# montyhall/bot7

Hardware: AMD Instinct MI355X
Metric: EI candidates scored/sec at N=2048,d=32 (higher is better)
Workload: dtype f64

## Files before the change

bot7_amd/build.py:

```python
import concurrent.futures
import os
import subprocess
import sys

HERE = os.path.dirname(os.path.abspath(__file__))
ROOT = os.path.dirname(HERE)
CSRC = os.path.join(HERE, "csrc")
BUILD = os.path.join(HERE, "_build")
OUT = os.path.join(HERE, "libbot7hip.so")
SOURCES = ["context.hip", "grid_api.hip", "gp_api.hip", "nominate.hip", "blr_api.hip", "sobol.hip", "covar.hip", "potrf.hip", "potrf_persist.hip", "posterior.hip", "score.hip", "extras.hip", "comm.hip", "group.hip", "blr_small.hip", "gp_small.hip", "kpost_small.hip", "batch.hip", "mes.hip", "rff.hip", "slice.hip", "refine.hip", "kg.hip", "ehvi.hip", "trust_region.hip"]
DIAG_ONLY_SOURCES = ["nll_small.hip"]
DIAG_OUT = os.path.join(ROOT, "tools", "_build", "libbot7hip_diag.so")
HEADERS = [os.path.join(CSRC, "b7_internal.h"), os.path.join(CSRC, "gemm_f64.h"), os.path.join(CSRC, "potrf_diag.h"), os.path.join(CSRC, "comm_rccl.h"), os.path.join(CSRC, "ksx_exp.h"), os.path.join(CSRC, "ksx_walk.h"), os.path.join(CSRC, "exp_table.h"), os.path.join(CSRC, "mes_math.h"), os.path.join(CSRC, "counter_rng.h"), os.path.join(CSRC, "gp_small_body.h"), os.path.join(CSRC, "post_ring_layout.h"),
           os.path.join(ROOT, "include", "bot7hip.h")]
HIPCC = os.environ.get("HIPCC", "/opt/rocm/bin/hipcc")
FLAGS = ["-O3", "-std=c++17", "-fPIC", "--offload-arch=gfx950", "-fno-fast-math", "-Wall",
         "-I" + os.path.join(ROOT, "include"), "-I" + CSRC, "-I/opt/rocm/include"]


def _stale(target, deps):
    if not os.path.exists(target):
        return True
    t = os.path.getmtime(target)
    return any(os.path.getmtime(d) > t for d in deps)


EXTRA_FLAGS = {"covar.hip": ["-mllvm", "-amdgpu-mfma-vgpr-form"], "batch.hip": ["-mllvm", "-amdgpu-mfma-vgpr-form"],
               "rff.hip": ["-mllvm", "-amdgpu-mfma-vgpr-form"],
               "kg.hip": ["-mllvm", "-amdgpu-mfma-vgpr-form"],
               "slice.hip": ["-mllvm", "-disable-machine-licm"]}


def _compile(src, diag=False):
    obj = os.path.join(BUILD, ("diag_" if diag else "") + src.replace(".hip", ".o"))
    path = os.path.join(CSRC, src)
    if _stale(obj, [path] + HEADERS + [os.path.abspath(__file__)]):
        subprocess.check_call([HIPCC] + FLAGS + EXTRA_FLAGS.get(src, []) + (["-DB7_DIAG"] if diag else []) + ["-c", path, "-o", obj])
        return obj, True
    return obj, False


def _mentions_diag(src):
    return "B7_DIAG" in open(os.path.join(CSRC, src)).read()


def build_diag(verbose=False):
    build()
    os.makedirs(os.path.dirname(DIAG_OUT), exist_ok=True)
    todo = [s for s in SOURCES if _mentions_diag(s)] + DIAG_ONLY_SOURCES
    with concurrent.futures.ThreadPoolExecutor(max_workers=min(8, len(todo))) as ex:
        res = dict(zip(todo, ex.map(lambda s: _compile(s, True), todo)))
    objs = [res[s][0] if s in res else os.path.join(BUILD, s.replace(".hip", ".o")) for s in SOURCES + DIAG_ONLY_SOURCES]
    if any(ch for _, ch in res.values()) or _stale(DIAG_OUT, objs):
        subprocess.check_call([HIPCC, "-shared", "-fPIC", "--offload-arch=gfx950", "-o", DIAG_OUT] + objs +
                              ["-ldl", "-Wl,-rpath,/opt/rocm/lib", "-Wl,--no-undefined", "-Wl,-Bsymbolic"])
        if verbose:
            print("built", DIAG_OUT)
    return DIAG_OUT


def posterior_isa():
    out = os.path.join(BUILD, "posterior.s")
    path = os.path.join(CSRC, "posterior.hip")
    if _stale(out, [path] + HEADERS + [os.path.abspath(__file__)]):
        subprocess.check_call([HIPCC] + [f for f in FLAGS if f != "-fPIC"] + ["-S", "--cuda-device-only", "-Wno-unused-command-line-argument",
                                                                            path, "-o", out])
    return out


def check_agpr_discipline():
    import re
    text = open(posterior_isa()).read()
    found = {}
    for m in re.finditer(r"^(_ZN\S*post_kernel_w4(?:ILi(\d)E|tILi\d+ELi\d+E)\S*):[^\n]*\n(.*?)\n\s*s_endpgm", text, flags=re.S | re.M):
        nj = int(m.group(2)) if m.group(2) else 16
        ntiles = 32 if nj == 16 else 8 * nj
        in_asm, stats, bad = False, {"mfma": 0, "mfma_from_zero": 0, "acc_reads": 0, "scratch": 0}, []
        for line in m.group(3).split("\n"):
            code = line.split(";")[0]
            if "ASMSTART" in line:
                in_asm = True
                continue
            if "ASMEND" in line:
                in_asm = False
                continue
            if in_asm:
                stats["mfma"] += "v_mfma_f64_16x16x4_f64" in code
                stats["mfma_from_zero"] += bool(re.search(r"v_mfma_f64_16x16x4_f64 a\[[^\]]*\], v\[[^\]]*\], v\[[^\]]*\], 0\s*$", code))
                stats["acc_reads"] += "v_accvgpr_read_b32" in code
            else:
                if re.search(r"(?<![A-Za-z0-9_.])a(\[|\d)", code):
                    bad.append(line.strip())
                if nj == 16 and re.search(r"\bm0\b", code):
                    bad.append(line.strip())
                stats["scratch"] += "scratch_" in code
        if bad or stats["scratch"] or stats["mfma_from_zero"] != ntiles or stats["acc_reads"] != 8 * ntiles:
            raise RuntimeError("post_kernel_w4<%d>: AGPR discipline broken: %r, compiler-generated AGPR uses: %r"
                               % (nj, stats, bad[:5]))
        found[nj] = stats
    if not {2, 4} <= set(found):
        raise RuntimeError("post_kernel_w4<2> and <4> expected in the ISA of posterior.hip, found %r" % sorted(found))
    return found


def build_post_probe():
    src = os.path.join(ROOT, "tools", "post_probe.hip")
    out = os.path.join(ROOT, "tools", "_build", "post_probe")
    os.makedirs(os.path.dirname(out), exist_ok=True)
    if _stale(out, [src, os.path.join(ROOT, "tools", "post_kernel_w8.h"), os.path.join(CSRC, "posterior.hip")] + HEADERS):
        subprocess.check_call([HIPCC, "--offload-arch=gfx950", "-O3", "-std=c++17", "-fno-fast-math", "-Wno-unused-value",
                               "-DB7_POST_NO_LAUNCHERS", "-I" + os.path.join(ROOT, "include"), "-I" + CSRC,
                               "-I/opt/rocm/include", "-o", out, src, "-Wl,-rpath,/opt/rocm/lib"])
    return out


def build(force=False, verbose=False):
    os.makedirs(BUILD, exist_ok=True)
    if force:
        for f in os.listdir(BUILD):
            os.remove(os.path.join(BUILD, f))
    with concurrent.futures.ThreadPoolExecutor(max_workers=min(8, len(SOURCES) + 2)) as ex:
        isa = ex.submit(check_agpr_discipline)
        probe = ex.submit(build_post_probe)
        results = list(ex.map(_compile, SOURCES))
        isa.result()
        probe.result()
    objs = [o for o, _ in results]
    if any(changed for _, changed in results) or _stale(OUT, objs):
        subprocess.check_call([HIPCC, "-shared", "-fPIC", "--offload-arch=gfx950", "-o", OUT] + objs +
                              ["-ldl", "-Wl,-rpath,/opt/rocm/lib", "-Wl,--no-undefined", "-Wl,-Bsymbolic"])
        if verbose:
            print("built", OUT)
    return OUT


if __name__ == "__main__":
    build(force="--force" in sys.argv, verbose=True)
    if "--diag" in sys.argv:
        build_diag(verbose=True)
```

bot7_amd/csrc/b7_internal.h:

```cpp
#pragma once
#include <hip/hip_runtime.h>
#include <stddef.h>
#include <stdint.h>

#include <map>
#include <string>
#include <vector>

#include "bot7hip.h"

constexpr int B7_NPAD = 128;
constexpr int B7_PANEL = 64;
constexpr int B7_PERSIST_NMAX = 4096;
constexpr int B7_MROWS = 256;
constexpr int B7_MAX_D = 96;

constexpr int B7_TAB_VAL = 0;
constexpr int B7_TAB_IDX = 1;
constexpr int B7_TAB_STATUS = 2;
constexpr int B7_TAB_ROWS = 3;
constexpr int B7_TAB_ROW0 = 4;
constexpr int B7_TAB_W = B7_TAB_ROW0 + B7_MAX_D;
constexpr int B7_MAX_WORLD = 64;

// ... 160 lines not shown
  DevBuf part;
  DevBuf ystar, mes_ticket;
  DevBuf mes_user;
  int mes_levels = 8;
  int mes_S = 0, mes_K = 0, mes_nb = 0;
  int64_t mes_M = 0;
  int mes_slot = 0;
  bool mes_valid = false;
  DevBuf ticket;
  DevBuf feas;
  DevBuf feas_stage;
  bool feas_valid = false;
  hipEvent_t ev_feas[2] = {nullptr, nullptr};
  DevBuf scratch;
  DevBuf tmpgrid;
  DevBuf tmpmu, tmpvar;
  DevBuf fant;
  DevBuf bel;
  DevBuf belvec;
  PinBuf pin_bel;
  DevBuf ts_paths;
  DevBuf ts_draw;
  DevBuf ts_work, ts_user;
  bool ts_valid = false;
  int64_t ts_M = 0;
  int ts_q = 0, ts_S = 0, ts_F = 0, ts_N = 0, ts_d = 0;
  DevBuf refine_ws, refine_trace;
  DevBuf refine_user;
  bool refine_trace_on = false, refine_valid = false;
  int refine_P = 0, refine_d = 0, refine_iters = 0, refine_trace_P = 0, refine_trace_iters = 0;
  RefState refine_last;
  DevBuf kg;
  DevBuf kgvec;
  DevBuf kg_slopes;
  DevBuf kg_user;
  PinBuf pin_kg;
  bool kg_trace_on = false, kg_valid = false, kg_traced = false;
  int kg_S = 0, kg_n = 0;
  int64_t kg_M = 0;
  size_t kg_al_off = 0;
  DevBuf post;
  bool post_valid = false;
  int post_S = 0;
  int64_t post_M = 0;
  DevBuf ehvi_front;
  DevBuf ehvi_user;
  hipEvent_t ev_ehvi[2] = {nullptr, nullptr};
  DevBuf feat;
  size_t feat_zeroed_bytes = 0;
  int feat_z = -1;
  int64_t Mfeat = 0;
  int zdim = 0;
  uint64_t feat_version = 0, grid_version = 0;
  DevBuf netbuf;

  void *comm = nullptr;
  int comm_rank = 0, comm_world = 1;
  DevBuf slots;
  uint64_t *tab_host = nullptr;
  uint64_t *tab_host_dev = nullptr;
  struct b7_group *group = nullptr;
  bool group_busy = false;
  bool win_valid = false;
  int64_t win_idx1 = 0;
  int win_rank = -1, win_d = 0;
  double win_row[B7_MAX_D];
  int64_t shard_rows[B7_MAX_WORLD];
  int shard_world = 0;

  hipEvent_t tev[B7_MAX_TIMERS][2];
  bool tev_init = false;
  bool profile = false;
  std::map<std::string, PhaseStat> phases;
  struct PendingPhase { const char *name; hipEvent_t e0, e1; };
  std::vector<PendingPhase> pending;
  std::vector<hipEvent_t> free_events;
  hipEvent_t phase_e0 = nullptr;
};

int b7_fail(b7_ctx *c, int code, const char *fmt, ...);
#define B7_HIP(c, expr)                                                                          \
  do {                                                                                           \
    hipError_t e__ = (expr);                                                                     \
    if (e__ != hipSuccess)                                                                       \
      return b7_fail((c), e__ == hipErrorOutOfMemory ? B7_ERR_NOMEM : B7_ERR_HIP, "%s:%d: %s", \
                     __FILE_NAME__, __LINE__, hipGetErrorString(e__));                           \
  } while (0)
#define B7_TRY(expr)          \
  do {                        \
    int rc__ = (expr);        \
    if (rc__ != B7_OK) return rc__; \
  } while (0)

int b7_ensure(b7_ctx *c, DevBuf &b, size_t bytes);
void b7_release(DevBuf &b);
int b7_pin_ensure(b7_ctx *c, PinBuf &b, size_t bytes, bool mapped);
static inline ScratchBlock *b7_scratch(const b7_ctx *c) { return static_cast<ScratchBlock *>(c->scratch.p); }

struct PhaseScope {
  b7_ctx *c;
  const char *name;
  PhaseScope(b7_ctx *c, const char *name);
  ~PhaseScope();
};

static inline int64_t round_up(int64_t x, int64_t m) { return (x + m - 1) / m * m; }
int npad_of(const b7_ctx *c, int64_t n);

struct FitSet {
  const double *w = nullptr, *zsc = nullptr, *zss = nullptr, *Linv = nullptr, *alpha = nullptr;
  int S = 1, Npad = 0, dpad = 0;
  double amp = 0.0, noise = 0.0, mean = 0.0;
  const double *amp_dev = nullptr, *noise_dev = nullptr, *mean_dev = nullptr;
  static int64_t s_w(int, int dpad) { return dpad; }
  static int64_t s_zsc(int Npad, int dpad) { return (int64_t)Npad * dpad; }
  static int64_t s_zss(int Npad, int) { return Npad; }
  static int64_t s_Linv(int Npad, int) { return (int64_t)Npad * Npad; }
  static int64_t s_alpha(int Npad, int) { return Npad; }
};
static inline FitSet ctx_fit(const b7_ctx *c) {
  FitSet f;
  f.w = (const double *)c->w.p, f.zsc = (const double *)c->zsc.p, f.zss = (const double *)c->zss.p;
  f.Linv = (const double *)c->Linv.p, f.alpha = (const double *)c->alpha.p;
  f.Npad = c->Npad, f.dpad = c->dpad;
  f.amp = c->amp, f.noise = c->noise, f.mean = c->mean;
  return f;
}

int launch_sobol(b7_ctx *c, double *out, int64_t size, int dims, int64_t skip, const double *mins,
                 const double *maxes);
int launch_random_grid(b7_ctx *c, double *out, int64_t size, int dims, uint64_t seed, int64_t row_offset,
                       const double *mins, const double *maxes);
int launch_remove_row(b7_ctx *c, const double *src, double *dst, int64_t M, int d, int64_t idx0);
int launch_remove_rows(b7_ctx *c, const double *src, double *dst, int64_t M, int d, const int64_t *cuts_dev, int ncut);
int launch_colrange(b7_ctx *c, const double *grid, int64_t M, int d, double *out_dev);
int launch_col_affine(b7_ctx *c, double *grid, int64_t M, int d, const double *v_dev, bool mul);
int launch_gather_rows(b7_ctx *c, const double *src, double *out, const int64_t *idx0_dev, int64_t n, int d);
int launch_trust_region(b7_ctx *c, double *grid, int64_t M, int d, const double *vec_dev, bool rotate, double prob, uint64_t seed,
                        int64_t row_offset);

struct KBatchDesc {
  int64_t s_w = 0, s_zsc = 0, s_zsh = 0, s_out = 0;
  const double *amp = nullptr;
  int64_t s_alpha = 0, s_mu = 0;
  const double *mean = nullptr;
};
struct ObsSet {
  const double *zsc;
  const double *zsh;
  int npad;
  const double *w = nullptr;
  KBatchDesc batch;
};
int launch_prep_obs_aux(b7_ctx *c, const double *xobs, const double *ls_dev, int N, int npad, double *zsc,
                        double *zsh);
int launch_k_generic(b7_ctx *c, const double *xq, int64_t rows, int64_t Mtotal, const ObsSet &o, double *out);
int launch_prep_obs(b7_ctx *c, const double *xobs, const double *lenscale_sq_dev, int N, int d);
int launch_kxx(b7_ctx *c, double diag_add);
int launch_ksx_batch(b7_ctx *c, const FitSet &f, const double *xq, int64_t rows, int64_t Mtotal, double *ks, int64_t s_out,
                     double *mu, int64_t s_mu);
int launch_kxx_batch(b7_ctx *c, int B, const double *ls_dev, const double *amp_dev, const double *noise_dev, double *w,
                     double *zsc, double *zss, double *K);
int launch_ksx(b7_ctx *c, const FitSet &f, const double *xq, int64_t row0, int64_t rows, int64_t Mtotal, int d, double *ks,
               double *mu, int ycols);

struct FactorNote {
  bool alpha_done = false;
  int *report_written = nullptr;
};
int launch_potrf(b7_ctx *c, double extra, bool with_inverse, int *report_hint = nullptr, FactorNote *note = nullptr);
int launch_trtri(b7_ctx *c);
int launch_potrf_persist(b7_ctx *c, double extra, bool with_inverse);
int launch_nll_batch(b7_ctx *c, int B, const double *K, double *L, double *dinv, unsigned *flags, int *info,
                     const double *resid, double *terms);
int launch_nll_one(b7_ctx *c, const double *K, double *L, double *dinv, unsigned *flags, int *info, const double *resid,
                   double *terms, double extra);
size_t persist_flag_words_host(int nb);
int launch_potrf_small(b7_ctx *c, int B, const double *K, double *L, double *Linv, double *dinv, const double *resid, double *alpha,
                       double extra, int *info, int *report_dev, int64_t sK, int64_t sL, int64_t sdinv, int64_t svec, int sinfo);
int launch_blr_head_small(b7_ctx *c, const double *Z, int N, int z, int ldz, const double *yv, double alpha_prec, double beta,
                          int *report_dev);
int launch_blr_heads_small(b7_ctx *c, int S, const double *Z, int N, int z, int ldz, const double *yraw_dev, const double *hyp3_dev,
                           double *L, double *Linv, double *m, double *b, int *info, int *report_dev, double *terms);
int launch_post_heads(b7_ctx *c, int S, const double *Linv, const double *feat, int64_t rows, int64_t Mtotal, double *var, int64_t svar,
                      const double *zero_dev, const double *invbeta_dev);
int launch_gemv_rows_batch(b7_ctx *c, int S, const double *A, int lda, const double *x, int64_t sx, int n, const double *base_dev,
                           int64_t rows, double *y, int64_t sy);
int launch_nll_small(b7_ctx *c, int B, const double *hyp_dev, const double *hyp_host, double *terms_dev, int *info_dev,
                     unsigned *done_dev);
bool kpost_small_applies(const b7_ctx *c);
int launch_kpost_small(b7_ctx *c, const FitSet &f, const double *xq, int64_t M, double *mu, double *var, int64_t sout);
bool gp_small_applies(const b7_ctx *c);
static inline bool fit_small_applies(const b7_ctx *c) {
  return c->fit_small && c->potrf_sched == 3 && c->inverse_inline && gp_small_applies(c);
}
int launch_nll_small8(b7_ctx *c, int B, const double *hyp_dev, const double *hyp_host, double *terms_dev, int *info_dev,
                      unsigned *done_dev);
int launch_fit_small(b7_ctx *c, int B, const double *hyp_dev, const double *hyp_host, double *hyp_out, double *w, double *zsc,
                     double *zss, double *L, double *Linv, double *dinv, double *alpha, double *resid, int *info_dev,
                     int *report_dev);
int launch_alpha(b7_ctx *c, int *report_dev = nullptr, int report_words = 0, const FactorNote &note = FactorNote());
int launch_alpha_batch(b7_ctx *c, int B, const double *Linv, const double *resid, double *alpha, const int *report_src = nullptr,
                       int *report_dev = nullptr, int report_words = 0);
int launch_fit_batch(b7_ctx *c, int B, const double *K, double *L, double *Linv, double *dinv, unsigned *flags, int *info);
int launch_nll_terms(b7_ctx *c, double *out_dev);
int launch_fro_norm_sq(b7_ctx *c, const double *A, int n, int ld, double *out_dev);
int launch_set_identity(b7_ctx *c);

int launch_post(b7_ctx *c, const FitSet &f, const double *ks, int64_t row0, int64_t rows, int64_t Mtotal, double *var);
int launch_post_batch(b7_ctx *c, const FitSet &f, const double *ks, int64_t sks, int64_t rows, int64_t Mtotal, double *var,
                      int64_t svar);

int launch_mean_multi(b7_ctx *c, const FitSet &f, const double *ks, int64_t row0, int64_t rows, int64_t Mtotal, double *mu);
int launch_gemm_nt(b7_ctx *c, const double *A, int lda, const double *B, int ldb, double *C, int ldc, int m, int n,
                   int k);
int launch_fantasy_cov(b7_ctx *c, const double *kpp, const double *g, double *S, int P, double diag_add);
int launch_fantasy_factor(b7_ctx *c, double *S, double *dinv_tmp, int *info_dev);
int launch_fantasy_sample(b7_ctx *c, const double *Lp, const double *mu, int P, int n, uint64_t seed, double *out);
int launch_add_diag(b7_ctx *c, double *S, int ld, int n, double v);

int launch_append_finalize(b7_ctx *c, const double *krow, const double *lvec, const double *uvec, const double *evec,
                           int *status_dev);
int launch_append_vectors(b7_ctx *c, const double *krow, double *lvec, double *uvec, double *part, double *evec);
int launch_mlp_forward(b7_ctx *c, const double *X, int64_t M, int d, const double *net_dev, const int *dims,
                       int n_layers, int activation, double *out, int ld_out);
int launch_mlp_forward_mean(b7_ctx *c, const double *X, int64_t M, int d, const double *net_dev, const int *dims,
                            int n_layers, int activation, double *out, int ld_out, const double *mvec, double mean0,
                            double *mu, bool *mean_done);
int launch_gemv_rows(b7_ctx *c, const double *A, int lda, const double *x, int n, double base, int64_t row0,
                     int64_t rows, int64_t Mtotal, double *y);
int launch_transpose_pad(b7_ctx *c, const double *Z, int n, int ldz, int z, double *Zt, int zpad, int nk);
int launch_blr_assemble(b7_ctx *c, const double *G, double *K, int z, int zpad, double alpha_prec, double beta);

int launch_score(b7_ctx *c, ScoreParams p, const double *mu, const double *var, int64_t M, int ycols, double *out, bool accumulate);
int launch_score_batch(b7_ctx *c, const ScoreParams &p, double *acc, int64_t M);
int launch_finish(b7_ctx *c, double *acc, int64_t M, double divisor, double *best_val, int64_t *best_idx1, bool logacc = false);
int launch_fill(b7_ctx *c, double *p, int64_t n, double v);
int launch_finish_slot(b7_ctx *c, double *acc, int64_t M, double divisor, uint64_t *tab_dev, int rank, int world,
                       int64_t offset, const double *grid, int d, bool all_slots, uint64_t *host_rec = nullptr,
                       unsigned *host_done = nullptr, bool logacc = false, const double *feas = nullptr);

struct ExclRows {
  int n = 0;
  long long row[B7_BATCH_MAX];
};
int launch_score_finish_slot(b7_ctx *c, const ScoreParams &p, double *acc, int64_t M, double divisor, uint64_t *tab_dev,
                             int rank, int world, int64_t offset, const double *grid, int d, bool all_slots, uint64_t *host_rec = nullptr,
                             unsigned *host_done = nullptr, const ExclRows *excl = nullptr, const double *feas = nullptr);
void acc_declare_zeros(b7_ctx *c, int score_kind);
int acc_write_zeros(b7_ctx *c);
void acc_forget(b7_ctx *c);
int acc_materialize(b7_ctx *c);
void feas_forget(b7_ctx *c);
static inline void post_forget(b7_ctx *c) { c->post_valid = false; }
int feas_write_zeros(b7_ctx *c);
int launch_feas_add(b7_ctx *c, const double *src);
int launch_feas_best(b7_ctx *c, double *best_val, int64_t *best_idx1);
int launch_keep_record(b7_ctx *c, uint64_t *tab_dev, int rank, int world);
int launch_score_grad(b7_ctx *c, const ScoreParams &p, const double *mu, const double *var, const double *dmu, const double *dvar,
                      int64_t M1, int d, double *value, double *grad);
struct RefStep {
  const double *mu, *var, *dmu, *dvar;
  const double *xq;
  double *xq_next;
  RefState *st;
  double *trace;
  const double *lo, *hi;
  int d, P, iter, iters;
  double eta0;
};
int launch_refine_step(b7_ctx *c, const ScoreParams &p, const RefStep &r);
int launch_row_slot(b7_ctx *c, uint64_t *tab_dev, int rank, int world, int64_t idx1_global, int64_t local0, const double *grid,
                    int d);

int exch_table_ensure(b7_ctx *c, int world);
int exch_local(b7_ctx *c, double divisor, int64_t offset, int rank, int world, bool all_slots, bool mirror = false,
               const ScoreParams *pend = nullptr, const ExclRows *excl = nullptr, const double *feas = nullptr);
int exch_wait_mirror(b7_ctx *c);
int exch_fail_record(b7_ctx *c, int rank, int world, int code);
int exch_allreduce(b7_ctx *c);
int exch_collective(b7_ctx *c, int rc, int rank, int world, double *best_val, int64_t *best_idx1);
int exch_rewrite_record(b7_ctx *c, int rank, int world);
int exch_fetch(b7_ctx *c, int first_rank, int nranks);
bool exch_pick(const uint64_t *tab, int world, int stride, double *val, int64_t *idx1, int *rank);
int exch_conclude(b7_ctx *c, const uint64_t *tab, int world, double *best_val, int64_t *best_idx1);
void exch_forget(b7_ctx *c);

void persist_gave_up(b7_ctx *c);
int chol_with_jitter(b7_ctx *c, double *jitter_out, int *info_first_out, bool with_inverse, FactorNote *note = nullptr);
int check_hyp(b7_ctx *c, const b7_hyp *hyp, int d);
void launch_resid_batch(b7_ctx *c, int B, const double *mean_dev);
int fit_front(b7_ctx *c, const b7_hyp *hyp, const double *ls_dev);
int fit_hyp_core(b7_ctx *c, const b7_hyp *hyp, double *nll_out, double *jitter_used, int *info_out, bool then_predict);
int64_t predict_chunk(const b7_ctx *c, int64_t M);
int predict_into(b7_ctx *c, const FitSet &fit, const double *xq, int64_t M, double *mu, double *var);
int copy_out_mu_var(b7_ctx *c, const void *mu, const void *var, int64_t M, int cols, double *mean_host, double *var_host,
                    bool wait = false);

struct HypPack { double *ls, *amp, *noise, *mean; };
static inline HypPack hyp_pack(void *base, int B, int d) {
  double *amp = static_cast<double *>(base) + (size_t)B * d;
  return {static_cast<double *>(base), amp, amp + B, amp + 2 * (size_t)B};
}
constexpr int B7_SLOTS_OPERANDS = 1;
constexpr int B7_SLOTS_LINV = 2;
constexpr int B7_SLOTS_ALPHA = 4;
constexpr int B7_SLOTS_FACTOR = 8;
int batch_slots_ensure(b7_ctx *c, int B, int groups);
static inline FitSet batch_fits(const b7_ctx *c, int S) {
  const HypPack hd = hyp_pack(c->bhyp.p, S, c->dfit);
  FitSet f;
  f.w = (const double *)c->bw.p, f.zsc = (const double *)c->bzsc.p, f.zss = (const double *)c->bzss.p;
  f.Linv = (const double *)c->bLinv.p, f.alpha = (const double *)c->balpha.p;
  f.S = S, f.Npad = c->Npad, f.dpad = c->dpad;
  f.amp_dev = hd.amp, f.noise_dev = hd.noise, f.mean_dev = hd.mean;
  return f;
}
static inline FitSet fit_at(const FitSet &set, int s, const b7_hyp &hyp) {
  const int Npad = set.Npad, dpad = set.dpad;
  FitSet f;
  f.Npad = Npad, f.dpad = dpad;
  f.w = set.w + s * FitSet::s_w(Npad, dpad), f.zsc = set.zsc + s * FitSet::s_zsc(Npad, dpad), f.zss = set.zss + s * FitSet::s_zss(Npad, dpad);
  f.Linv = set.Linv + s * FitSet::s_Linv(Npad, dpad), f.alpha = set.alpha + s * FitSet::s_alpha(Npad, dpad);
  f.amp = hyp.amp, f.noise = hyp.noise, f.mean = hyp.mean;
  return f;
}

int nominate_args(b7_ctx *c, const char *who, const b7_score_spec *spec, int64_t offset);
int stage_fmin(b7_ctx *c, const double *fmin, double **fd_out);
static inline bool score_needs_fmin(int kind) { return kind == B7_SCORE_EI || kind == B7_SCORE_LOGEI || kind == B7_SCORE_LOGPI; }
constexpr int score_acc_kind(int kind) { return (kind == B7_SCORE_LOGEI || kind == B7_SCORE_LOGPI) ? B7_ACC_LOG : B7_ACC_LINEAR; }
static inline const char *score_kind_name(int kind) {
  return kind == B7_SCORE_EI ? "ei" : kind == B7_SCORE_LOGEI ? "logei" : kind == B7_SCORE_LOGPI ? "logpi" : kind == B7_SCORE_MES ? "mes" : "cb";
}
int mes_begin(b7_ctx *c, int S, int64_t M, int K);
int launch_mes_search(b7_ctx *c, const double *mu, const double *var, int64_t stride, int nS, int slot0);
const double *mes_ystar_dev(const b7_ctx *c, int slot);
int mes_refuse(b7_ctx *c, const char *who, const b7_score_spec *spec);
ScoreParams score_params(const b7_ctx *c, const b7_score_spec *spec, const double *fd);
int score_add(b7_ctx *c, const b7_score_spec *sp, const double *fd, bool accumulate = true);
int pending_score(b7_ctx *c, int S, const b7_score_spec *spec, const double *fd, ScoreParams *out);
int eval_validate(b7_ctx *c, int S, const b7_hyp *hyps, const b7_score_spec *spec, int64_t offset);
struct BelKeep {
  double *mu = nullptr, *var = nullptr;
  FitSet fits;
  bool want_alpha = false;
};
int eval_enqueue(b7_ctx *c, int S, const b7_hyp *hyps, const b7_score_spec *spec, ScoreParams *pend, BelKeep *keep = nullptr);
bool reports_clean(b7_ctx *c, const int *reports, int S, bool persist);
int eval_redo(b7_ctx *c, int S, const b7_hyp *hyps, const b7_score_spec *spec, double *jitter_out, int *info_out,
              BelKeep *keep = nullptr);
struct BelPass {
  const double *xq; int64_t rows;
  const double *xj;
  const double *w, *zsc, *zss;
  const double *wj;
  const double *par;
  double *scal;
  double *kcol;
  double *var, *u; int64_t sgrid;
  int64_t idx; int j;
};
int launch_believer(b7_ctx *c, int S, const BelPass &p, bool column);
// ... 31 lines not shown
```

bot7_amd/csrc/blr_api.hip:

```cpp
#include <math.h>
#include <string.h>

#include "b7_internal.h"

static int upload_net(b7_ctx *c, const b7_mlp *net, int *z_out) {
  if (!net || !net->dims || !net->W || !net->b || net->n_layers < 1 || net->n_layers > 4)
    return b7_fail(c, B7_ERR_INVALID, "mlp: 1..4 layers with dims, W and b required");
  size_t total = 0;
  for (int l = 0; l < net->n_layers; ++l) total += (size_t)net->dims[l + 1] * net->dims[l] + net->dims[l + 1];
  std::vector<double> pack(total);
  size_t off = 0;
  for (int l = 0; l < net->n_layers; ++l) {
    const size_t nw = (size_t)net->dims[l + 1] * net->dims[l];
    memcpy(&pack[off], net->W[l], nw * sizeof(double));
    off += nw;
    memcpy(&pack[off], net->b[l], (size_t)net->dims[l + 1] * sizeof(double));
    off += net->dims[l + 1];
  }
  *z_out = net->dims[net->n_layers];
  if (c->net_host.size() == total && c->netbuf.cap >= total * sizeof(double) &&
      memcmp(c->net_host.data(), pack.data(), total * sizeof(double)) == 0)
    return B7_OK;
  B7_TRY(b7_ensure(c, c->netbuf, total * sizeof(double)));
  B7_HIP(c, hipStreamSynchronize(c->stream));
  B7_HIP(c, hipMemcpy(c->netbuf.p, pack.data(), total * sizeof(double), hipMemcpyHostToDevice));
  c->net_host.swap(pack);
  return B7_OK;
}

static int feat_alloc(b7_ctx *c, int64_t M, int z) {
  const int zpad = npad_of(c, z);
  const size_t bytes = sizeof(double) * (size_t)round_up(M, B7_MROWS) * zpad;
  const bool grown = c->feat.cap < bytes;
  B7_TRY(b7_ensure(c, c->feat, bytes));
  if (grown || c->feat_z != z || c->feat_zeroed_bytes < bytes) {
    B7_HIP(c, hipMemsetAsync(c->feat.p, 0, c->feat.cap, c->stream));
    c->feat_zeroed_bytes = c->feat.cap;
    c->feat_z = z;
  }
  c->Mfeat = M;
  c->zdim = z;
  c->predicted = false;
  return B7_OK;
}

static int blr_head_setup(b7_ctx *c, int z, int nk, double mean, double noise, bool general = true) {
  const size_t np = (size_t)npad_of(c, z), nn = np * np * sizeof(double);
  if (general) {
    for (DevBuf *b : {&c->K, &c->L, &c->Linv, &c->W}) B7_TRY(b7_ensure(c, *b, nn));
    B7_TRY(b7_ensure(c, c->dinv, sizeof(double) * (np + B7_PANEL) * B7_PANEL));
    B7_TRY(b7_ensure(c, c->alpha, sizeof(double) * np));
    B7_TRY(b7_ensure(c, c->resid, sizeof(double) * np));
    B7_TRY(b7_ensure(c, c->tmpvar, sizeof(double) * (size_t)nk));
  }
  B7_TRY(b7_ensure(c, c->info, B7_INFO_BYTES));
  c->have_data = false, c->fitted = false, c->predicted = false;
  post_forget(c);
  c->N = z, c->Npad = (int)np, c->ycols = 1, c->yld = 1, c->model_kind = 1;
  c->mean = mean, c->noise = noise, c->amp = 0.0;
  return B7_OK;
}

static int blr_predict_enqueue(b7_ctx *c, int64_t M, bool mean_done = false) {
  B7_TRY(b7_ensure(c, c->mu, sizeof(double) * (size_t)M));
  B7_TRY(b7_ensure(c, c->var, sizeof(double) * (size_t)M));
  if (!mean_done)
    B7_TRY(launch_gemv_rows(c, (const double *)c->feat.p, c->Npad, (const double *)c->alpha.p, c->Npad, c->mean, 0, M, M,
                            (double *)c->mu.p));
  B7_TRY(launch_post(c, ctx_fit(c), (const double *)c->feat.p, 0, round_up(M, B7_MROWS), M, (double *)c->var.p));
  c->predicted = true;
  c->Mpred = M;
  return B7_OK;
}

static int blr_fit_core(b7_ctx *c, const double *Y0, int N, int z, double alpha_prec, double beta, double mean,
                        double *nll_out) {
  const int zpad = npad_of(c, z), nk = (int)round_up(N, 16);
  const size_t np = (size_t)zpad;
  B7_TRY(blr_head_setup(c, z, nk, mean, 1.0 / beta));
  std::vector<double> rb((size_t)nk, 0.0);
  for (int i = 0; i < N; ++i) rb[i] = beta * (Y0[i] - mean);
  B7_HIP(c, hipMemcpyAsync(c->tmpvar.p, rb.data(), sizeof(double) * nk, hipMemcpyHostToDevice, c->stream));
  B7_TRY(launch_gemm_nt(c, (const double *)c->tmpgrid.p, nk, (const double *)c->tmpgrid.p, nk, (double *)c->W.p, zpad,
                        zpad, zpad, nk));
  B7_TRY(launch_blr_assemble(c, (const double *)c->W.p, (double *)c->K.p, z, zpad, alpha_prec, beta));
  B7_TRY(launch_gemv_rows(c, (const double *)c->tmpgrid.p, nk, (const double *)c->tmpvar.p, nk, 0.0, 0, zpad, zpad,
                          (double *)c->resid.p));
  int info_first = 0;
  double jitter = 0.0;
  FactorNote note;
  B7_TRY(chol_with_jitter(c, &jitter, &info_first, true, &note));
  B7_TRY(launch_trtri(c));
  B7_TRY(launch_alpha(c, nullptr, 0, note));
  B7_HIP(c, hipStreamSynchronize(c->stream));
  if (nll_out) {
    std::vector<double> diag(z), m(z), bq(z);
    B7_HIP(c, hipMemcpy2D(diag.data(), sizeof(double), c->L.p, sizeof(double) * (np + 1), sizeof(double), z,
                          hipMemcpyDeviceToHost));
    B7_HIP(c, hipMemcpy(m.data(), c->alpha.p, sizeof(double) * z, hipMemcpyDeviceToHost));
    B7_HIP(c, hipMemcpy(bq.data(), c->resid.p, sizeof(double) * z, hipMemcpyDeviceToHost));
    double logdet = 0.0, rr = 0.0, qm = 0.0;
    for (int k = 0; k < z; ++k) {
      logdet += 2.0 * log(diag[k]);
      qm += bq[k] * m[k];
    }
    for (int i = 0; i < N; ++i) rr += (Y0[i] - mean) * (Y0[i] - mean);
    const double Em = 0.5 * beta * rr - 0.5 * qm;
    *nll_out = -(0.5 * z * log(alpha_prec) + 0.5 * N * log(beta) - Em - 0.5 * logdet - 0.5 * N * log(2.0 * M_PI));
  }
  c->fitted = true;
  return B7_OK;
}

static int blr_enqueue_fit(b7_ctx *c, const b7_mlp *net, const double *X0, const double *Y0, int N, int z, double alpha_prec,
                           double beta, double mean) {
  const int d = net->dims[0], zpad = npad_of(c, z), nk = (int)round_up(N, 16);
  B7_TRY(b7_ensure(c, c->tmpgrid, sizeof(double) * (size_t)zpad * nk));
  B7_TRY(blr_head_setup(c, z, nk, mean, 1.0 / beta));
  const size_t up_doubles = (size_t)N * d + (size_t)nk;
  B7_TRY(b7_ensure(c, c->tmpmu, sizeof(double) * (up_doubles + (size_t)N * z)));
  B7_TRY(b7_pin_ensure(c, c->pin_blr, sizeof(double) * up_doubles, false));
  double *stage = static_cast<double *>(c->pin_blr.host);
  memcpy(stage, X0, sizeof(double) * (size_t)N * d);
  for (int i = 0; i < nk; ++i) stage[(size_t)N * d + i] = i < N ? beta * (Y0[i] - mean) : 0.0;
  double *xdev = (double *)c->tmpmu.p, *yvdev = xdev + (size_t)N * d, *zdev = yvdev + nk;
  B7_HIP(c, hipMemcpyAsync(xdev, stage, sizeof(double) * up_doubles, hipMemcpyHostToDevice, c->stream));
  B7_TRY(launch_mlp_forward(c, xdev, N, d, (const double *)c->netbuf.p, net->dims, net->n_layers, net->activation, zdev, z));
  if (zpad == 64 && c->blr_small) {
    B7_TRY(launch_blr_head_small(c, zdev, N, z, z, yvdev, alpha_prec, beta, nullptr));
    B7_HIP(c, hipMemcpyAsync(c->pinned->fit.info, c->info.p, 16, hipMemcpyDeviceToHost, c->stream));
    c->fitted = true;
    return B7_OK;
  }
  B7_TRY(launch_transpose_pad(c, zdev, N, z, z, (double *)c->tmpgrid.p, zpad, nk));
  B7_TRY(launch_gemm_nt(c, (const double *)c->tmpgrid.p, nk, (const double *)c->tmpgrid.p, nk, (double *)c->W.p, zpad, zpad,
                        zpad, nk));
  B7_TRY(launch_blr_assemble(c, (const double *)c->W.p, (double *)c->K.p, z, zpad, alpha_prec, beta));
  B7_TRY(launch_gemv_rows(c, (const double *)c->tmpgrid.p, nk, (const double *)yvdev, nk, 0.0, 0, zpad, zpad,
                          (double *)c->resid.p));
  FactorNote note;
  B7_TRY(launch_potrf(c, 0.0, true, nullptr, &note));
  if (!c->linv_done) B7_TRY(launch_trtri(c));
  B7_TRY(launch_alpha(c, nullptr, 0, note));
  B7_HIP(c, hipMemcpyAsync(c->pinned->fit.info, c->info.p, 16, hipMemcpyDeviceToHost, c->stream));
  c->fitted = true;
  return B7_OK;
}

static int blr_enqueue_score(b7_ctx *c, const b7_mlp *net, int z, const b7_score_spec *spec, bool fused_mean = true) {
  const int zpad = npad_of(c, z);
  B7_TRY(feat_alloc(c, c->M, z));
  B7_TRY(b7_ensure(c, c->mu, sizeof(double) * (size_t)c->M));
  B7_TRY(b7_ensure(c, c->var, sizeof(double) * (size_t)c->M));
  B7_TRY(b7_ensure(c, c->acc, sizeof(double) * (size_t)c->M));
  bool mean_done = false;
  B7_TRY(launch_mlp_forward_mean(c, (const double *)c->grid[c->grid_cur].p, c->M, c->d, (const double *)c->netbuf.p, net->dims,
                                 net->n_layers, net->activation, (double *)c->feat.p, zpad,
                                 fused_mean ? (const double *)c->alpha.p : nullptr, c->mean, (double *)c->mu.p, &mean_done));
  B7_TRY(blr_predict_enqueue(c, c->M, mean_done));
  double *fd = nullptr;
  if (score_needs_fmin(spec->kind)) B7_TRY(stage_fmin(c, spec->fmin, &fd));
  return score_add(c, spec, fd, false);
}

static int blr_marg_slow(b7_ctx *c, const b7_mlp *net, const double *X0, const double *Y0, int N, int S, const double *ap,
                         const double *bt, const double *mn, int z, const b7_score_spec *spec, double *nll_out) {
  const int zpad = npad_of(c, z);
  B7_TRY(b7_ensure(c, c->acc, sizeof(double) * (size_t)c->M));
  B7_TRY(acc_write_zeros(c));
  for (int s = 0; s < S; ++s) {
    B7_TRY(b7_blr_fit_x(c, net, X0, Y0, N, ap[s], bt[s], mn[s], nll_out ? nll_out + s : nullptr));
    if (s == 0) {
      B7_TRY(feat_alloc(c, c->M, z));
      B7_TRY(launch_mlp_forward(c, (const double *)c->grid[c->grid_cur].p, c->M, c->d, (const double *)c->netbuf.p, net->dims,
                                net->n_layers, net->activation, (double *)c->feat.p, zpad));
    }
    c->Mfeat = c->M;
    B7_TRY(blr_predict_enqueue(c, c->M));
    double *fd = nullptr;
    if (score_needs_fmin(spec->kind)) B7_TRY(stage_fmin(c, spec->fmin, &fd));
    B7_TRY(score_add(c, spec, fd));
  }
  return B7_OK;
}

static int blr_marg_fast(b7_ctx *c, const b7_mlp *net, const double *X0, const double *Y0, int N, int S, const double *ap,
                         const double *bt, const double *mn, int z, const b7_score_spec *spec, bool want_terms, ScoreParams *pend) {
  const int d = net->dims[0];
  const size_t up_doubles = (size_t)N * d + (size_t)N + 5 * (size_t)S;
  B7_TRY(b7_ensure(c, c->tmpmu, sizeof(double) * (up_doubles + (size_t)N * z)));
  B7_TRY(b7_ensure(c, c->bL, sizeof(double) * (size_t)S * 64 * 64));
  B7_TRY(b7_ensure(c, c->bLinv, sizeof(double) * (size_t)S * 64 * 64));
  B7_TRY(b7_ensure(c, c->balpha, sizeof(double) * (size_t)S * 64));
  B7_TRY(b7_ensure(c, c->bresid, sizeof(double) * (size_t)S * 64));
  B7_TRY(b7_ensure(c, c->binfo, sizeof(int) * 4 * (size_t)S));
  B7_TRY(b7_ensure(c, c->bterms, sizeof(double) * 3 * (size_t)S + 64));
  B7_TRY(b7_ensure(c, c->bmu, sizeof(double) * (size_t)S * c->M));
  B7_TRY(b7_ensure(c, c->bvar, sizeof(double) * (size_t)S * c->M));
  B7_TRY(b7_ensure(c, c->acc, sizeof(double) * (size_t)c->M));
  const size_t rep_bytes = 16 * (size_t)S, term_bytes = sizeof(double) * 3 * (size_t)S;
  B7_TRY(b7_pin_ensure(c, c->pin_eval, rep_bytes + term_bytes, true));
  B7_TRY(b7_pin_ensure(c, c->pin_blr, sizeof(double) * up_doubles, false));
  B7_TRY(blr_head_setup(c, z, 0, c->mean, c->noise, false));
  double *stage = static_cast<double *>(c->pin_blr.host);
  memcpy(stage, X0, sizeof(double) * (size_t)N * d);
  memcpy(stage + (size_t)N * d, Y0, sizeof(double) * N);
  double *hs = stage + (size_t)N * d + N;
  for (int s = 0; s < S; ++s) hs[s] = ap[s], hs[S + s] = bt[s], hs[2 * S + s] = mn[s], hs[3 * S + s] = 0.0, hs[4 * S + s] = 1.0 / bt[s];
  double *xdev = (double *)c->tmpmu.p, *ydev = xdev + (size_t)N * d, *hdev = ydev + N, *zdev = hdev + 5 * (size_t)S;
  B7_HIP(c, hipMemcpyAsync(xdev, stage, sizeof(double) * up_doubles, hipMemcpyHostToDevice, c->stream));
  B7_TRY(launch_mlp_forward(c, xdev, N, d, (const double *)c->netbuf.p, net->dims, net->n_layers, net->activation, zdev, z));
  int *reports = static_cast<int *>(c->pin_eval.host);
  memset(reports, 0xff, rep_bytes);
  B7_TRY(launch_blr_heads_small(c, S, zdev, N, z, z, ydev, hdev, (double *)c->bL.p, (double *)c->bLinv.p, (double *)c->balpha.p,
                                (double *)c->bresid.p, (int *)c->binfo.p, static_cast<int *>(c->pin_eval.dev), (double *)c->bterms.p));
  if (want_terms)
    B7_HIP(c, hipMemcpyAsync(static_cast<char *>(c->pin_eval.host) + rep_bytes, c->bterms.p, term_bytes, hipMemcpyDeviceToHost, c->stream));
  B7_TRY(feat_alloc(c, c->M, z));
  B7_TRY(launch_mlp_forward(c, (const double *)c->grid[c->grid_cur].p, c->M, c->d, (const double *)c->netbuf.p, net->dims,
                            net->n_layers, net->activation, (double *)c->feat.p, 64));
  B7_TRY(launch_gemv_rows_batch(c, S, (const double *)c->feat.p, 64, (const double *)c->balpha.p, 64, 64, hdev + 2 * (size_t)S, c->M,
                                (double *)c->bmu.p, c->M));
// ... 194 lines not shown
```

bot7_amd/csrc/covar.hip:

```cpp
#include "b7_internal.h"
#include "gemm_f64.h"
#include "ksx_exp.h"
#include "ksx_walk.h"

namespace {

__global__ void __launch_bounds__(64) prep_obs_kernel(const double *__restrict__ xobs, const double *ls, double *w,
                                                      double *zsc, double *zsh, int N, int Npad, int d, int dpad) {
  extern __shared__ __align__(16) double psm[];
  {
    const int64_t b = blockIdx.y;
    ls += b * d;
    w += b * dpad;
    zsc += b * (int64_t)Npad * dpad;
    zsh += b * Npad;
  }
  const int tld = dpad + 1, lane = threadIdx.x, row0 = blockIdx.x * 64;
  double *tile = psm, *wl = psm + 64 * tld;
  for (int k = lane; k < dpad; k += 64) {
    const double wk = (k < d) ? 1.0 / ls[k] : 0.0;
    wl[k] = wk;
    if (blockIdx.x == 0) w[k] = wk;
  }
  int nrows = N - row0;
  nrows = nrows < 0 ? 0 : (nrows > 64 ? 64 : nrows);
  const double *src = xobs + (int64_t)row0 * d;
#pragma unroll 8
  for (int e = lane; e < nrows * d; e += 64) {
    const int r = e / d, k = e - r * d;
    tile[r * tld + k] = src[e];
  }
  __syncthreads();
  double s = 0.0;
#pragma unroll 8
  for (int k = 0; k < dpad; ++k) {
    const double z = (lane < nrows && k < d) ? tile[lane * tld + k] : 0.0;
    const double wk = wl[k];
    tile[lane * tld + k] = z * wk;
    s += (z * z) * wk;
  }
  if (row0 + lane < Npad) zsh[row0 + lane] = (lane < nrows) ? 0.5 * s : 1e300;
  __syncthreads();
  double *dst = zsc + (int64_t)row0 * dpad;
#pragma unroll 8
  for (int e = lane; e < 64 * dpad; e += 64) {
    const int r = e / dpad, k = e - r * dpad;
    if (row0 + r < Npad) dst[e] = tile[r * tld + k];
  }
}

__device__ __forceinline__ void pair_pack(double a, double b, d2_t &out) {
  const int alo = __double2loint(a), ahi = __double2hiint(a), blo = __double2loint(b), bhi = __double2hiint(b);
  int o0l, o0h, o1l, o1h;
  asm volatile(
      "s_mov_b32 vcc_lo, 0x55555555\n\t"
      "s_mov_b32 vcc_hi, 0x55555555\n\t"
      "s_nop 0\n\t"
      "v_cndmask_b32_dpp %0, %6, %4, vcc quad_perm:[1,0,3,2] row_mask:0xf bank_mask:0xf\n\t"
      "v_cndmask_b32_dpp %1, %7, %5, vcc quad_perm:[1,0,3,2] row_mask:0xf bank_mask:0xf\n\t"
      "s_not_b64 vcc, vcc\n\t"
      "v_cndmask_b32_dpp %2, %4, %6, vcc quad_perm:[1,0,3,2] row_mask:0xf bank_mask:0xf\n\t"
      "v_cndmask_b32_dpp %3, %5, %7, vcc quad_perm:[1,0,3,2] row_mask:0xf bank_mask:0xf"
      : "=&v"(o0l), "=&v"(o0h), "=&v"(o1l), "=&v"(o1h)
      : "v"(alo), "v"(ahi), "v"(blo), "v"(bhi)
      : "vcc", "scc");
  out[0] = __hiloint2double(o0h, o0l);
  out[1] = __hiloint2double(o1h, o1l);
}

using KBatch = KBatchDesc;
template <int DPAD, int KERN>
__global__ void __launch_bounds__(256)
    ksx_kernel(const double *__restrict__ xq, int64_t row0, int64_t Mtotal, int d, int dpad_rt, const double *w,
               const double *zsc, const double *zsh, const double *__restrict__ alpha, double amp, double meanc, int Npad,
               double *out, double *__restrict__ mu, KBatch kb) {
  extern __shared__ __align__(16) double sm[];
  if (kb.amp) {
    const int64_t bz = blockIdx.z;
    w += bz * kb.s_w;
    zsc += bz * kb.s_zsc;
    zsh += bz * kb.s_zsh;
    out += bz * kb.s_out;
    amp = kb.amp[bz];
    if (kb.mean) {
      alpha += bz * kb.s_alpha;
      mu += bz * kb.s_mu;
      meanc = kb.mean[bz];
    }
  }
  (void)dpad_rt;
  using T = KsxTile<DPAD, 1>;
  constexpr int KO = T::KO;
  KsxWalk<DPAD, 1> wk(sm, zsc, zsh);
  const int tid = wk.tid, lane = wk.lane, wave = wk.wave, lr = wk.lr, lq = wk.lq;
  const int64_t qbase = row0 + (int64_t)blockIdx.x * KSX_Q;
  const int nslab_total = Npad / KO;
  const int nslab = nslab_total / gridDim.y;
  const int slab0 = blockIdx.y * nslab;
  __builtin_assume(nslab > 0);

  const double *sh = wk.zs();
  double *sal = wk.rider();
  double pre_a = 0.0;
  auto rider_load = [&](int s) { pre_a = alpha ? alpha[s * KO + tid] : 0.0; };
  auto rider_store = [&](int buf) { sal[buf * KO + tid] = pre_a; };
  wk.begin(xq, qbase, Mtotal, d, w, amp, slab0, nslab, [] {}, rider_load, rider_store);

  double hq[4], macc[4] = {0.0, 0.0, 0.0, 0.0};
#pragma unroll
  for (int r = 0; r < 4; ++r) hq[r] = wk.xs()[wave * 16 + lq + 4 * r];
  const bool odd = lane & 1;
  double *orow = out + ((int64_t)blockIdx.x * KSX_Q + wave * 16 + lq + (odd ? 4 : 0)) * Npad + (lr & ~1);

  wk.run(slab0, nslab, rider_load, rider_store, [&](int s, int cur, int t, const double (&bf)[T::KSTEPS]) {
    const int o0 = s * KO;
#if B7_KSX_ABLATE & 8
    const d4_t c = mfma_f64(wk.qf[0], bf[0], d4_t{0.0, 0.0, 0.0, 0.0});
#else
    const d4_t c = wk.dist(bf);
#endif
    const double hk = sh[cur * KO + t * 16 + lr];
    const double al = sal[cur * KO + t * 16 + lr];
    double kv[4];
#if B7_KSX_ABLATE & 4
    wk.arg4(c, hq, hk, kv);
#else
    wk.template cov<KERN>(c, hq, hk, kv);
#endif
#pragma unroll
    for (int r = 0; r < 4; ++r) macc[r] = __builtin_fma(kv[r], al, macc[r]);
    d2_t v01, v23;
    pair_pack(kv[0], kv[1], v01);
    pair_pack(kv[2], kv[3], v23);
    {
      double *p = orow + o0 + t * 16;
#if B7_KSX_ABLATE & 1
      if (v01[0] == 1.2345e-300) {
#endif
#if B7_KSX_ABLATE & 16
      double *pi = out + ((int64_t)blockIdx.x * KSX_Q + wave * 16 + 4 * t + (lane >> 5)) * Npad + o0 + (lane & 31) * 2;
      *reinterpret_cast<d2_t *>(pi) = v01;
      *reinterpret_cast<d2_t *>(pi + (int64_t)2 * Npad) = v23;
#elif B7_KSX_ABLATE & 32
      __builtin_nontemporal_store(v01, reinterpret_cast<d2_t *>(p));
      __builtin_nontemporal_store(v23, reinterpret_cast<d2_t *>(p + (int64_t)8 * Npad));
#else
      *reinterpret_cast<d2_t *>(p) = v01;
      *reinterpret_cast<d2_t *>(p + (int64_t)8 * Npad) = v23;
#endif
#if B7_KSX_ABLATE & 1
      }
#endif
    }
  });

  if (mu) {
#pragma unroll
    for (int r = 0; r < 4; ++r) {
      double v = macc[r];
      v += __shfl_xor(v, 1);
      v += __shfl_xor(v, 2);
      v += __shfl_xor(v, 4);
      v += __shfl_xor(v, 8);
      const int64_t g = qbase + wave * 16 + lq + 4 * r;
      if (lr == 0 && g < Mtotal) mu[g] = meanc + v;
    }
  }
}

__global__ void __launch_bounds__(256)
    kxx_fix_kernel(double *K, int N, int Npad, double diag_add, const double *diag_arr, int64_t sK) {
  if (diag_arr) {
    K += (int64_t)blockIdx.y * sK;
    diag_add = diag_arr[blockIdx.y];
  }
  int64_t e = (int64_t)blockIdx.x * blockDim.x + threadIdx.x;
  if (e >= (int64_t)Npad * Npad) return;
  int i = (int)(e / Npad), j = (int)(e - (int64_t)i * Npad);
  if (i >= N || j >= N)
    K[e] = (i == j) ? 1.0 : 0.0;
  else if (i == j)
    K[e] += diag_add;
}

template <int DPAD>
size_t ksx_lds_bytes() {
  size_t bytes = KsxTile<DPAD, 1>::lds_bytes(0);
#if B7_KSX_ABLATE & 128
  const size_t per_cu = 160 * 1024, fit = per_cu / bytes;
  if (fit > 1) bytes = per_cu / (fit - 1) - 512;
#endif
  return bytes;
}

int ksx_launch(b7_ctx *c, dim3 grid, const double *xq, int64_t row0, int64_t Mtotal, int d, const ObsSet &o,
               const double *alpha, double amp, double meanc, double *out, double *mu) {
  return ksx_for_class(c, "covariance kernel", [&](auto cls) {
    using C = decltype(cls);
    const size_t lds = ksx_lds_bytes<C::DPAD>();
    auto kern = ksx_kernel<C::DPAD, C::KERN>;
    B7_HIP(c, hipFuncSetAttribute(reinterpret_cast<const void *>(kern), hipFuncAttributeMaxDynamicSharedMemorySize,
                                  (int)lds));
    hipLaunchKernelGGL(kern, grid, dim3(256), lds, c->stream, xq, row0, Mtotal, d, c->dpad, o.w ? o.w : (const double *)c->w.p,
                       o.zsc, o.zsh, alpha, amp, meanc, o.npad, out, mu, o.batch);
    B7_HIP(c, hipGetLastError());
    return B7_OK;
  });
}

}

int launch_prep_obs(b7_ctx *c, const double *xobs, const double *ls_dev, int N, int d) {
  PhaseScope ps(c, "prep");
  const size_t lds = sizeof(double) * (64 * (size_t)(c->dpad + 1) + c->dpad);
  hipLaunchKernelGGL(prep_obs_kernel, dim3((c->Npad + 63) / 64), dim3(64), lds, c->stream, xobs, ls_dev,
                     (double *)c->w.p, (double *)c->zsc.p, (double *)c->zss.p, N, c->Npad, d, c->dpad);
  B7_HIP(c, hipGetLastError());
  return B7_OK;
}

int launch_prep_obs_aux(b7_ctx *c, const double *xobs, const double *ls_dev, int N, int npad, double *zsc,
                        double *zsh) {
  const size_t lds = sizeof(double) * (64 * (size_t)(c->dpad + 1) + c->dpad);
  hipLaunchKernelGGL(prep_obs_kernel, dim3((npad + 63) / 64), dim3(64), lds, c->stream, xobs, ls_dev, (double *)c->w.p,
                     zsc, zsh, N, npad, c->dfit, c->dpad);
  B7_HIP(c, hipGetLastError());
  return B7_OK;
}

int launch_k_generic(b7_ctx *c, const double *xq, int64_t rows, int64_t Mtotal, const ObsSet &o, double *out) {
  if (rows % KSX_Q || o.npad % 64) return b7_fail(c, B7_ERR_INVALID, "k_generic: extents not multiples of 64");
  return ksx_launch(c, dim3((unsigned)(rows / KSX_Q), 1), xq, 0, Mtotal, c->dfit, o, nullptr, c->amp, 0.0, out, nullptr);
}

int launch_ksx(b7_ctx *c, const FitSet &f, const double *xq, int64_t row0, int64_t rows, int64_t Mtotal, int d, double *ks,
               double *mu, int ycols) {
  PhaseScope ps(c, "ksx");
  if (rows % KSX_Q) return b7_fail(c, B7_ERR_INVALID, "ksx: rows %lld not a multiple of %d", (long long)rows, KSX_Q);
  if (ycols != 1) mu = nullptr;
  ObsSet o{f.zsc, f.zss, c->Npad};
  o.w = f.w;
  return ksx_launch(c, dim3((unsigned)(rows / KSX_Q), 1), xq, row0, Mtotal, d, o, mu ? f.alpha : nullptr, f.amp, f.mean, ks, mu);
}

int launch_kxx(b7_ctx *c, double diag_add) {
  PhaseScope ps(c, "kxx");
  const int Npad = c->Npad;
  int ny = 1;
  while (ny < 16 && (Npad / 64) % (ny * 2) == 0 && (Npad / KSX_Q) * ny < 2 * c->cus) ny *= 2;
  const ObsSet o{(const double *)c->zsc.p, (const double *)c->zss.p, Npad};
  B7_TRY(ksx_launch(c, dim3(Npad / KSX_Q, ny), (const double *)c->xobs.p, 0, c->N, c->dfit, o, nullptr, c->amp, 0.0,
                      (double *)c->K.p, nullptr));
  int64_t total = (int64_t)Npad * Npad;
  hipLaunchKernelGGL(kxx_fix_kernel, dim3((unsigned)((total + 255) / 256)), dim3(256), 0, c->stream, (double *)c->K.p,
                     c->N, Npad, diag_add, (const double *)nullptr, (int64_t)0);
  B7_HIP(c, hipGetLastError());
  return B7_OK;
}

int launch_ksx_batch(b7_ctx *c, const FitSet &f, const double *xq, int64_t rows, int64_t Mtotal, double *ks, int64_t s_out,
                     double *mu, int64_t s_mu) {
  PhaseScope ps(c, "ksx");
  if (rows % KSX_Q) return b7_fail(c, B7_ERR_INVALID, "ksx: rows %lld not a multiple of %d", (long long)rows, KSX_Q);
  ObsSet o{f.zsc, f.zss, c->Npad};
  o.w = f.w;
  o.batch.s_w = FitSet::s_w(c->Npad, c->dpad);
  o.batch.s_zsc = FitSet::s_zsc(c->Npad, c->dpad);
  o.batch.s_zsh = FitSet::s_zss(c->Npad, c->dpad);
  o.batch.s_out = s_out;
  o.batch.amp = f.amp_dev;
  o.batch.s_alpha = FitSet::s_alpha(c->Npad, c->dpad);
  o.batch.s_mu = s_mu;
  o.batch.mean = f.mean_dev;
  return ksx_launch(c, dim3((unsigned)(rows / KSX_Q), 1, f.S), xq, 0, Mtotal, c->dfit, o, f.alpha, f.amp, 0.0, ks, mu);
}

int launch_kxx_batch(b7_ctx *c, int B, const double *ls_dev, const double *amp_dev, const double *noise_dev, double *w,
                     double *zsc, double *zss, double *K) {
  PhaseScope ps(c, "kxx");
  const int Npad = c->Npad, d = c->dfit, dpad = c->dpad;
  const size_t lds = sizeof(double) * (64 * (size_t)(dpad + 1) + dpad);
  hipLaunchKernelGGL(prep_obs_kernel, dim3((Npad + 63) / 64, B), dim3(64), lds, c->stream, (const double *)c->xobs.p, ls_dev,
                     w, zsc, zss, c->N, Npad, d, dpad);
  ObsSet o{zsc, zss, Npad};
  o.w = w;
  o.batch.s_w = FitSet::s_w(Npad, dpad);
  o.batch.s_zsc = FitSet::s_zsc(Npad, dpad);
  o.batch.s_zsh = FitSet::s_zss(Npad, dpad);
  o.batch.s_out = (int64_t)Npad * Npad;
  o.batch.amp = amp_dev;
  int ny = 1;
  while (ny < 16 && (Npad / 64) % (ny * 2) == 0 && (Npad / KSX_Q) * ny * B < 2 * c->cus) ny *= 2;
  B7_TRY(ksx_launch(c, dim3(Npad / KSX_Q, ny, B), (const double *)c->xobs.p, 0, c->N, d, o, nullptr, c->amp, 0.0, K, nullptr));
  const int64_t total = (int64_t)Npad * Npad;
  hipLaunchKernelGGL(kxx_fix_kernel, dim3((unsigned)((total + 255) / 256), B), dim3(256), 0, c->stream, K, c->N, Npad, 0.0,
                     noise_dev, total);
  B7_HIP(c, hipGetLastError());
  return B7_OK;
}
```

bot7_amd/csrc/gp_api.hip:

```cpp
#include <math.h>
#include <string.h>

#include <chrono>

#include "b7_internal.h"

extern "C" __global__ void __launch_bounds__(256) resid_kernel(const double *__restrict__ y, double *__restrict__ r, int64_t nreal,
                                                               int64_t ntotal, double mean) {
  const int64_t e = (int64_t)blockIdx.x * blockDim.x + threadIdx.x;
  if (e < ntotal) r[e] = e < nreal ? y[e] - mean : 0.0;
}

extern "C" __global__ void __launch_bounds__(256) resid_batch_kernel(const double *__restrict__ y, double *__restrict__ r, int N,
                                                                     int Npad, const double *__restrict__ mean) {
  const int i = blockIdx.x * blockDim.x + threadIdx.x, b = blockIdx.y;
  if (i < Npad) r[(int64_t)b * Npad + i] = i < N ? y[i] - mean[b] : 0.0;
}

void launch_resid_batch(b7_ctx *c, int B, const double *mean_dev) {
  hipLaunchKernelGGL(resid_batch_kernel, dim3((c->Npad + 255) / 256, B), dim3(256), 0, c->stream, (const double *)c->ybuf.p,
                     (double *)c->bresid.p, c->N, c->Npad, mean_dev);
}

void persist_gave_up(b7_ctx *c) {
  c->persist_aborts += 1;
  if (c->potrf_sched == 3) c->potrf_sched_saved = 3;
  c->potrf_sched = 1;
}
static void persist_restore(b7_ctx *c) {
  if (c->potrf_sched_saved == 3 && c->persist_aborts < 3) c->potrf_sched = 3;
}

static int try_factor(b7_ctx *c, double extra, int *info, bool with_inverse, FactorNote *note) {
  int two[2] = {0, 0};
  for (int attempt = 0; attempt < 2; ++attempt) {
    B7_TRY(launch_potrf(c, extra, with_inverse, nullptr, note));
    B7_HIP(c, hipMemcpyAsync(two, c->info.p, 2 * sizeof(int), hipMemcpyDeviceToHost, c->stream));
    B7_HIP(c, hipStreamSynchronize(c->stream));
    if (two[1] == 0) break;
    if (attempt == 1) return b7_fail(c, B7_ERR_HIP, "Cholesky: hand-off time-out (code %d) outside the persistent schedule", two[1]);
    persist_gave_up(c);
  }
  persist_restore(c);
  *info = two[0];
  return B7_OK;
}

static int jitter_retries(b7_ctx *c, double *jitter_out, bool with_inverse, FactorNote *note) {
  const int N = c->N;
  int info = 1;
  double jitter = 0.0;
  {
    double *fro_dev = reinterpret_cast<double *>(reinterpret_cast<char *>(c->info.p) + 16);
    B7_TRY(launch_fro_norm_sq(c, (const double *)c->K.p, N, c->Npad, fro_dev));
    double fro = 0.0;
    B7_HIP(c, hipMemcpyAsync(&fro, fro_dev, sizeof(double), hipMemcpyDeviceToHost, c->stream));
    B7_HIP(c, hipStreamSynchronize(c->stream));
    const double max_eps = sqrt(fro);
    if (max_eps != max_eps)
      return b7_fail(c, B7_ERR_INVALID, "chol: the matrix contains NaN (check X_obs and the hyper-parameters)");
    double eps = c->opts.jitter_eps;
    for (;;) {
      if (eps > max_eps) {
        jitter = -1.0;
        B7_TRY(launch_set_identity(c));
        c->linv_done = false;
        if (note) *note = FactorNote();
        break;
      }
      eps = eps * c->opts.jitter_growth;
      B7_TRY(try_factor(c, eps, &info, with_inverse, note));
      if (info == 0) {
        jitter = eps;
        break;
      }
    }
  }
  *jitter_out = jitter;
  return B7_OK;
}

int chol_with_jitter(b7_ctx *c, double *jitter_out, int *info_first_out, bool with_inverse, FactorNote *note) {
  int info = 0;
  B7_TRY(try_factor(c, 0.0, &info, with_inverse, note));
  *info_first_out = info;
  *jitter_out = 0.0;
  if (info != 0) B7_TRY(jitter_retries(c, jitter_out, with_inverse, note));
  return B7_OK;
}

int64_t predict_chunk(const b7_ctx *c, int64_t M) {
  int64_t chunk = (int64_t)(c->ks_bytes / (sizeof(double) * (size_t)c->Npad)) / B7_MROWS * B7_MROWS;
  if (chunk < B7_MROWS) chunk = B7_MROWS;
  const int64_t Mpad = round_up(M, B7_MROWS);
  return chunk > Mpad ? Mpad : chunk;
}

int predict_into(b7_ctx *c, const FitSet &fit, const double *xq, int64_t M, double *mu, double *var) {
  if (M == 0) return B7_OK;
  if (c->kpost_small && c->model_kind == 0 && kpost_small_applies(c))
    return launch_kpost_small(c, fit, xq, M, mu, var, M);
  const int64_t chunk = predict_chunk(c, M), Mpad = round_up(M, B7_MROWS);
  B7_TRY(b7_ensure(c, c->ks, sizeof(double) * (size_t)chunk * c->Npad));
  for (int64_t row0 = 0; row0 < M; row0 += chunk) {
    int64_t rows = Mpad - row0 < chunk ? Mpad - row0 : chunk;
    B7_TRY(launch_ksx(c, fit, xq, row0, rows, M, c->dfit, (double *)c->ks.p, mu, c->ycols));
    if (c->ycols > 1) B7_TRY(launch_mean_multi(c, fit, (const double *)c->ks.p, row0, rows, M, mu));
    B7_TRY(launch_post(c, fit, (const double *)c->ks.p, row0, rows, M, var));
  }
  return B7_OK;
}

int batch_slots_ensure(b7_ctx *c, int B, int groups) {
  const size_t n = (size_t)c->Npad, one = sizeof(double) * (size_t)B;
  if (groups & B7_SLOTS_OPERANDS) {
    B7_TRY(b7_ensure(c, c->bw, one * FitSet::s_w(c->Npad, c->dpad)));
    B7_TRY(b7_ensure(c, c->bzsc, one * FitSet::s_zsc(c->Npad, c->dpad)));
    B7_TRY(b7_ensure(c, c->bzss, one * FitSet::s_zss(c->Npad, c->dpad)));
  }
  if (groups & B7_SLOTS_LINV) B7_TRY(b7_ensure(c, c->bLinv, one * FitSet::s_Linv(c->Npad, c->dpad)));
  if (groups & B7_SLOTS_ALPHA) B7_TRY(b7_ensure(c, c->balpha, one * FitSet::s_alpha(c->Npad, c->dpad)));
  if (groups & B7_SLOTS_FACTOR) {
    B7_TRY(b7_ensure(c, c->bK, one * n * n));
    B7_TRY(b7_ensure(c, c->bL, one * n * n));
    B7_TRY(b7_ensure(c, c->bdinv, one * n * B7_PANEL));
    B7_TRY(b7_ensure(c, c->bresid, one * n));
  }
  return B7_OK;
}

int check_hyp(b7_ctx *c, const b7_hyp *hyp, int d) {
  if (!hyp || !hyp->lenscale_sq) return b7_fail(c, B7_ERR_INVALID, "gp_fit_hyp: NULL argument");
  for (int k = 0; k < d; ++k)
    if (!(hyp->lenscale_sq[k] > 0.0)) return b7_fail(c, B7_ERR_INVALID, "gp_fit: lenscale_sq[%d] must be > 0", k);
  if (!(hyp->amp > 0.0) || !(hyp->noise >= 0.0)) return b7_fail(c, B7_ERR_INVALID, "gp_fit: amp > 0, noise >= 0");
  return B7_OK;
}

int fit_front(b7_ctx *c, const b7_hyp *hyp, const double *ls_dev) {
  const int N = c->N, d = c->dfit, ycols = c->ycols;
  c->fitted = false;
  c->model_kind = 0;
  c->predicted = false;
  c->amp = hyp->amp;
  c->noise = hyp->noise;
  c->mean = hyp->mean;
  const int64_t ntotal = (int64_t)c->Npad * ycols;
  hipLaunchKernelGGL(resid_kernel, dim3((unsigned)((ntotal + 255) / 256)), dim3(256), 0, c->stream,
                     (const double *)c->ybuf.p, (double *)c->resid.p, (int64_t)N * ycols, ntotal, hyp->mean);
  B7_TRY(launch_prep_obs(c, (const double *)c->xobs.p, ls_dev, N, d));
  return launch_kxx(c, hyp->noise);
}

int fit_hyp_core(b7_ctx *c, const b7_hyp *hyp, double *nll_out, double *jitter_used, int *info_out,
                        bool then_predict) {
  if (!c) return B7_ERR_INVALID;
  if (!c->have_data) return b7_fail(c, B7_ERR_STATE, "gp_fit_hyp: call b7_gp_set_data first");
  const int N = c->N, d = c->dfit, ycols = c->ycols;
  B7_TRY(check_hyp(c, hyp, d));
  B7_HIP(c, hipSetDevice(c->device));

  double *ls_stage = c->pinned->vec, *ls_dev = b7_scratch(c)->lenscale;
  memcpy(ls_stage, hyp->lenscale_sq, sizeof(double) * d);
  const bool small = fit_small_applies(c);
  if (small) {
    ls_stage[d] = hyp->amp, ls_stage[d + 1] = hyp->noise, ls_stage[d + 2] = hyp->mean;
    c->fitted = false;
    c->model_kind = 0;
    c->predicted = false;
    c->amp = hyp->amp;
    c->noise = hyp->noise;
    c->mean = hyp->mean;
  } else {
    B7_HIP(c, hipMemcpyAsync(ls_dev, ls_stage, sizeof(double) * d, hipMemcpyHostToDevice, c->stream));
    B7_TRY(fit_front(c, hyp, ls_dev));
  }

  FitBlock &blk = c->pinned->fit;
  double *terms_dev = reinterpret_cast<double *>(reinterpret_cast<char *>(c->info.p) + 16);
  const size_t blk_bytes = 16 + sizeof(double) * (nll_out ? 1 + ycols : 0);
  bool tail_done = false;
  FactorNote note;
  for (int attempt = 0; attempt < 2; ++attempt) {
    if (small && attempt == 0) {
      B7_TRY(launch_fit_small(c, 1, nullptr, ls_stage, ls_dev, (double *)c->w.p, (double *)c->zsc.p, (double *)c->zss.p, (double *)c->L.p,
                              (double *)c->Linv.p, (double *)c->dinv.p, (double *)c->alpha.p, (double *)c->resid.p, (int *)c->info.p,
                              nullptr));
      c->linv_done = true;
      tail_done = true;
      if (nll_out) B7_TRY(launch_nll_terms(c, terms_dev));
    } else {
      B7_TRY(launch_potrf(c, 0.0, true, nullptr, &note));
      tail_done = c->linv_done;
      if (tail_done) {
        B7_TRY(launch_alpha(c, nullptr, 0, note));
        if (nll_out) B7_TRY(launch_nll_terms(c, terms_dev));
      }
    }
    B7_HIP(c, hipMemcpyAsync(&blk, c->info.p, tail_done ? blk_bytes : 16, hipMemcpyDeviceToHost, c->stream));
    if (then_predict && tail_done) {
      B7_HIP(c, hipEventRecord(c->ev_fit, c->stream));
      c->fitted = true;
      B7_TRY(predict_into(c, ctx_fit(c), (const double *)c->grid[c->grid_cur].p, c->M, (double *)c->mu.p, (double *)c->var.p));
      B7_HIP(c, hipEventSynchronize(c->ev_fit));
    } else {
      B7_HIP(c, hipStreamSynchronize(c->stream));
    }
    if (blk.info[1] == 0) break;
    c->fitted = false;
    if (attempt == 1) return b7_fail(c, B7_ERR_HIP, "Cholesky: hand-off time-out (code %d) outside the persistent schedule", blk.info[1]);
    persist_gave_up(c);
  }
  const int info_first = blk.info[0];
  double jitter = 0.0;
  bool predicted = then_predict && tail_done;
  if (info_first != 0) {
    c->fitted = false;
    if (small) B7_TRY(fit_front(c, hyp, ls_dev));
    B7_TRY(jitter_retries(c, &jitter, true, &note));
    tail_done = false;
    predicted = false;
  }
  if (!tail_done) {
    B7_TRY(launch_trtri(c));
    B7_TRY(launch_alpha(c, nullptr, 0, note));
    if (nll_out) B7_TRY(launch_nll_terms(c, terms_dev));
    B7_HIP(c, hipMemcpyAsync(&blk, c->info.p, blk_bytes, hipMemcpyDeviceToHost, c->stream));
    B7_HIP(c, hipStreamSynchronize(c->stream));
  }
  if (then_predict && !predicted) {
    c->fitted = true;
    B7_TRY(predict_into(c, ctx_fit(c), (const double *)c->grid[c->grid_cur].p, c->M, (double *)c->mu.p, (double *)c->var.p));
  }
  if (nll_out)
    for (int k = 0; k < ycols; ++k) nll_out[k] = 0.5 * blk.terms[1 + k] + blk.terms[0] + 0.5 * N * log(2.0 * M_PI);
  if (jitter_used) *jitter_used = jitter;
  if (info_out) *info_out = info_first;
  persist_restore(c);
  c->fitted = true;
  return B7_OK;
}

int copy_out_mu_var(b7_ctx *c, const void *mu, const void *var, int64_t M, int cols, double *mean_host, double *var_host, bool wait) {
  if (mean_host) B7_HIP(c, hipMemcpyAsync(mean_host, mu, sizeof(double) * (size_t)M * cols, hipMemcpyDeviceToHost, c->stream));
  if (var_host) B7_HIP(c, hipMemcpyAsync(var_host, var, sizeof(double) * (size_t)M, hipMemcpyDeviceToHost, c->stream));
  if (mean_host || var_host || wait) B7_HIP(c, hipStreamSynchronize(c->stream));
  return B7_OK;
}

extern "C" {

int b7_gp_default_opts(b7_gp_opts *o) {
  if (!o) return B7_ERR_INVALID;
  o->jitter_eps = 1e-8;
  o->jitter_growth = 1.1;
  o->var_with_noise = 0;
  o->var_clamp = 0;
  o->var_min = 0.0;
  return B7_OK;
}

// ... 146 lines not shown
      B7_HIP(c, hipMemcpyAsync(&terms[(size_t)b * 2], tb, 2 * sizeof(double), hipMemcpyDeviceToHost, c->stream));
      B7_HIP(c, hipStreamSynchronize(c->stream));
      bad = two[0];
      aborted = two[1];
      return B7_OK;
    };
    if (aborted) {
      c->persist_aborts += 1;
      B7_TRY(redo(0.0));
    }
    if (aborted) {
      b7_hyp h{lenscale_sq + (size_t)b * d, amp[b], noise[b], mean[b]};
      persist_gave_up(c);
      double nll1 = 0.0, jit1 = 0.0;
      int info1 = 0;
      const int rc1 = fit_hyp_core(c, &h, &nll1, &jit1, &info1, false);
      c->fitted = false;
      c->predicted = false;
      B7_TRY(rc1);
      nll_out[b] = nll1;
      if (jitter_out) jitter_out[b] = jit1;
      if (info_out) info_out[b] = info1;
      continue;
    }
    if (bad != 0) {
      double *fro_dev = (double *)c->bterms.p;
      B7_TRY(launch_fro_norm_sq(c, Kb, N, n, fro_dev));
      double fro = 0.0;
      B7_HIP(c, hipMemcpyAsync(&fro, fro_dev, sizeof(double), hipMemcpyDeviceToHost, c->stream));
      B7_HIP(c, hipStreamSynchronize(c->stream));
      const double max_eps = sqrt(fro);
      if (max_eps != max_eps) return b7_fail(c, B7_ERR_INVALID, "gp_nll_batch: K of fit %d contains NaN", b);
      double eps = c->opts.jitter_eps;
      while (bad != 0) {
        if (eps > max_eps) return b7_fail(c, B7_ERR_INVALID, "gp_nll_batch: fit %d cannot be factored", b);
        eps = eps * c->opts.jitter_growth;
        B7_TRY(redo(eps));
        if (aborted) return b7_fail(c, B7_ERR_HIP, "gp_nll_batch: hand-off time-out (code %d) in fit %d", aborted, b);
        jitter = eps;
      }
    }
    nll_out[b] = 0.5 * terms[(size_t)b * 2] + terms[(size_t)b * 2 + 1] + c0;
    if (jitter_out) jitter_out[b] = jitter;
    if (info_out) info_out[b] = info_first;
  }
  return B7_OK;
}

int b7_gp_fit_hyp(b7_ctx *c, const b7_hyp *hyp, double *nll_out, double *jitter_used, int *info_out) {
  return fit_hyp_core(c, hyp, nll_out, jitter_used, info_out, false);
}

int b7_gp_fit(b7_ctx *c, const double *X, const double *Y, int N, int d, int ycols, const b7_hyp *hyp,
              double *nll_out, double *jitter_used, int *info_out) {
  if (!c) return B7_ERR_INVALID;
  if (!hyp || !hyp->lenscale_sq) return b7_fail(c, B7_ERR_INVALID, "gp_fit: NULL argument");
  B7_TRY(b7_gp_set_data(c, X, Y, N, d, ycols));
  return b7_gp_fit_hyp(c, hyp, nll_out, jitter_used, info_out);
}

int b7_gp_predict_hyp(b7_ctx *c, const b7_hyp *hyp, double *mean_host, double *var_host, double *nll_out,
                      double *jitter_used, int *info_out) {
  if (!c) return B7_ERR_INVALID;
  if (!c->have_data) return b7_fail(c, B7_ERR_STATE, "gp_predict_hyp: call b7_gp_set_data first");
  if (c->M <= 0) return b7_fail(c, B7_ERR_STATE, "gp_predict_hyp: no candidate grid on this context");
  if (c->d != c->dfit) return b7_fail(c, B7_ERR_INVALID, "gp_predict_hyp: grid dims %d != data dims %d", c->d, c->dfit);
  B7_HIP(c, hipSetDevice(c->device));
  B7_TRY(b7_ensure(c, c->mu, sizeof(double) * (size_t)c->M * c->ycols));
  B7_TRY(b7_ensure(c, c->var, sizeof(double) * (size_t)c->M));
  B7_TRY(fit_hyp_core(c, hyp, nll_out, jitter_used, info_out, true));
  c->predicted = true;
  c->Mpred = c->M;
  return copy_out_mu_var(c, c->mu.p, c->var.p, c->M, c->ycols, mean_host, var_host);
}

int b7_chol(b7_ctx *c, const double *src, int n, double *res, double *jitter_used, int *info_out) {
  if (!c) return B7_ERR_INVALID;
  if (!src || !res || n < 1) return b7_fail(c, B7_ERR_INVALID, "chol: bad arguments");
  B7_HIP(c, hipSetDevice(c->device));
  c->fitted = false;
  c->have_data = false;
  c->predicted = false;
  post_forget(c);
  c->N = n;
  c->Npad = npad_of(c, n);
  const size_t np = (size_t)c->Npad, nn = np * np * sizeof(double);
  B7_TRY(b7_ensure(c, c->K, nn));
  B7_TRY(b7_ensure(c, c->L, nn));
  B7_TRY(b7_ensure(c, c->dinv, sizeof(double) * (np + B7_PANEL) * B7_PANEL));
  B7_TRY(b7_ensure(c, c->info, B7_INFO_BYTES));
  std::vector<double> Kp(np * np, 0.0);
  for (size_t i = 0; i < np; ++i) {
    if (i < (size_t)n)
      memcpy(&Kp[i * np], src + i * (size_t)n, sizeof(double) * n);
    else
      Kp[i * np + i] = 1.0;
  }
  B7_HIP(c, hipMemcpy(c->K.p, Kp.data(), nn, hipMemcpyHostToDevice));
  int info_first = 0;
  double jitter = 0.0;
  B7_TRY(chol_with_jitter(c, &jitter, &info_first, false));
  B7_HIP(c, hipStreamSynchronize(c->stream));
  B7_HIP(c, hipMemcpy2D(res, sizeof(double) * n, c->L.p, sizeof(double) * np, sizeof(double) * n, n,
                        hipMemcpyDeviceToHost));
  if (jitter_used) *jitter_used = jitter;
  if (info_out) *info_out = info_first;
  return B7_OK;
}

int b7_gp_predict(b7_ctx *c, double *mean_host, double *var_host) {
  if (!c) return B7_ERR_INVALID;
  if (!c->fitted || c->model_kind != 0) return b7_fail(c, B7_ERR_STATE, "gp_predict: no GP fit on this context");
  if (c->M <= 0) return b7_fail(c, B7_ERR_STATE, "gp_predict: no candidate grid on this context");
  if (c->d != c->dfit) return b7_fail(c, B7_ERR_INVALID, "gp_predict: grid dims %d != fit dims %d", c->d, c->dfit);
  B7_HIP(c, hipSetDevice(c->device));
  B7_TRY(b7_ensure(c, c->mu, sizeof(double) * (size_t)c->M * c->ycols));
  B7_TRY(b7_ensure(c, c->var, sizeof(double) * (size_t)c->M));
  B7_TRY(predict_into(c, ctx_fit(c), (const double *)c->grid[c->grid_cur].p, c->M, (double *)c->mu.p, (double *)c->var.p));
  c->predicted = true;
  c->Mpred = c->M;
  return copy_out_mu_var(c, c->mu.p, c->var.p, c->M, c->ycols, mean_host, var_host);
}

int b7_gp_predict_at(b7_ctx *c, const double *X1, int64_t M1, double *mean_host, double *var_host) {
  if (!c) return B7_ERR_INVALID;
  if (!c->fitted || c->model_kind != 0) return b7_fail(c, B7_ERR_STATE, "gp_predict_at: no GP fit on this context");
  if (M1 < 0 || (!X1 && M1 > 0)) return b7_fail(c, B7_ERR_INVALID, "gp_predict_at: bad X1/M1");
  if (M1 == 0) return B7_OK;
  B7_HIP(c, hipSetDevice(c->device));
  B7_TRY(b7_ensure(c, c->tmpgrid, sizeof(double) * (size_t)M1 * c->dfit));
  B7_TRY(b7_ensure(c, c->tmpmu, sizeof(double) * (size_t)M1 * c->ycols));
  B7_TRY(b7_ensure(c, c->tmpvar, sizeof(double) * (size_t)M1));
  B7_HIP(c, hipMemcpyAsync(c->tmpgrid.p, X1, sizeof(double) * (size_t)M1 * c->dfit, hipMemcpyHostToDevice, c->stream));
  B7_TRY(predict_into(c, ctx_fit(c), (const double *)c->tmpgrid.p, M1, (double *)c->tmpmu.p, (double *)c->tmpvar.p));
  return copy_out_mu_var(c, c->tmpmu.p, c->tmpvar.p, M1, c->ycols, mean_host, var_host, true);
}

int b7_gp_fantasize(b7_ctx *c, const double *X_pend, int P, int n, uint64_t seed, double *Y_out, double *mean_out,
                    double *cov_out) {
  if (!c) return B7_ERR_INVALID;
  if (!c->fitted || c->model_kind != 0) return b7_fail(c, B7_ERR_STATE, "gp_fantasize: no GP fit on this context");
  if (c->ycols != 1) return b7_fail(c, B7_ERR_UNSUPPORTED, "gp_fantasize: the fit must have one response column");
  if (!X_pend || P < 1 || n < 1 || !Y_out) return b7_fail(c, B7_ERR_INVALID, "gp_fantasize: bad arguments");
  if (P > 64) return b7_fail(c, B7_ERR_UNSUPPORTED, "gp_fantasize: %d pending points > 64", P);
  B7_HIP(c, hipSetDevice(c->device));
  const int np = c->Npad, d = c->dfit, dp = c->dpad;
  size_t need = (size_t)64 * d + (size_t)64 * dp + 64 + (size_t)2 * 64 * np + 4 * 4096 + 64 + (size_t)P * n + 16;
  B7_TRY(b7_ensure(c, c->fant, need * sizeof(double)));
  double *xp = (double *)c->fant.p, *zscp = xp + (size_t)64 * d, *zshp = zscp + (size_t)64 * dp, *kp = zshp + 64;
  double *vt = kp + (size_t)64 * np, *g = vt + (size_t)64 * np, *kpp = g + 4096, *S = kpp + 4096, *dv = S + 4096;
  double *mu = dv + 4096, *out = mu + 64;
  int *info_dev = (int *)(out + (size_t)P * n + 2);
  B7_HIP(c, hipMemcpyAsync(xp, X_pend, sizeof(double) * (size_t)P * d, hipMemcpyHostToDevice, c->stream));
  B7_TRY(launch_ksx(c, ctx_fit(c), xp, 0, 64, P, d, kp, mu, 1));
  B7_TRY(launch_gemm_nt(c, kp, np, (const double *)c->Linv.p, np, vt, np, 64, np, np));
  B7_TRY(launch_gemm_nt(c, vt, np, vt, np, g, 64, 64, 64, np));
  double *ls_dev = b7_scratch(c)->lenscale;
  B7_TRY(launch_prep_obs_aux(c, xp, ls_dev, P, 64, zscp, zshp));
  const ObsSet op{zscp, zshp, 64};
  B7_TRY(launch_k_generic(c, xp, 64, P, op, kpp));
  B7_TRY(launch_fantasy_cov(c, kpp, g, S, P, c->opts.var_with_noise ? c->noise : 0.0));
  if (cov_out) {
    B7_HIP(c, hipStreamSynchronize(c->stream));
    B7_HIP(c, hipMemcpy2D(cov_out, sizeof(double) * P, S, sizeof(double) * 64, sizeof(double) * P, P,
                          hipMemcpyDeviceToHost));
  }
  B7_HIP(c, hipMemcpyAsync(kpp, S, sizeof(double) * 4096, hipMemcpyDeviceToDevice, c->stream));
  double eps = c->opts.jitter_eps;
  int info = 0;
  for (int attempt = 0;; ++attempt) {
    B7_TRY(launch_fantasy_factor(c, S, dv, info_dev));
    B7_HIP(c, hipMemcpyAsync(&info, info_dev, sizeof(int), hipMemcpyDeviceToHost, c->stream));
    B7_HIP(c, hipStreamSynchronize(c->stream));
    if (info == 0) break;
    if (attempt > 4000) return b7_fail(c, B7_ERR_INVALID, "gp_fantasize: posterior covariance cannot be factored");
    eps = eps * c->opts.jitter_growth;
    B7_HIP(c, hipMemcpyAsync(S, kpp, sizeof(double) * 4096, hipMemcpyDeviceToDevice, c->stream));
    B7_TRY(launch_add_diag(c, S, 64, P, eps));
  }
  B7_TRY(launch_fantasy_sample(c, S, mu, P, n, seed, out));
  B7_HIP(c, hipMemcpyAsync(Y_out, out, sizeof(double) * (size_t)P * n, hipMemcpyDeviceToHost, c->stream));
  if (mean_out) B7_HIP(c, hipMemcpyAsync(mean_out, mu, sizeof(double) * P, hipMemcpyDeviceToHost, c->stream));
  B7_HIP(c, hipStreamSynchronize(c->stream));
  return B7_OK;
}

int b7_gp_append(b7_ctx *c, const double *x_new, const double *y_new) {
  if (!c) return B7_ERR_INVALID;
  if (!c->fitted || c->model_kind != 0) return b7_fail(c, B7_ERR_STATE, "gp_append: no GP fit on this context");
  if (!x_new || !y_new) return b7_fail(c, B7_ERR_INVALID, "gp_append: NULL argument");
  if (c->N + 1 > c->Npad)
    return b7_fail(c, B7_ERR_STATE, "gp_append: the padded factor is full (N = %d); refit with b7_gp_fit", c->N);
  B7_HIP(c, hipSetDevice(c->device));
  const int N = c->N, np = c->Npad, d = c->dfit, yc = c->ycols;
  c->predicted = false;
  post_forget(c);
  B7_HIP(c, hipMemcpyAsync((double *)c->xobs.p + (size_t)N * d, x_new, sizeof(double) * d, hipMemcpyHostToDevice,
                           c->stream));
  std::vector<double> r(yc);
  for (int k = 0; k < yc; ++k) r[k] = y_new[k] - c->mean;
  B7_HIP(c, hipMemcpyAsync((double *)c->resid.p + (size_t)N * yc, r.data(), sizeof(double) * yc, hipMemcpyHostToDevice,
                           c->stream));
  if (c->have_data)
    B7_HIP(c, hipMemcpyAsync((double *)c->ybuf.p + (size_t)N * yc, y_new, sizeof(double) * yc, hipMemcpyHostToDevice,
                             c->stream));
  double *ls_dev = b7_scratch(c)->lenscale;
  B7_TRY(launch_prep_obs(c, (const double *)c->xobs.p, ls_dev, N + 1, d));
  const size_t nslices = ((size_t)np + 255) / 256;
  B7_TRY(b7_ensure(c, c->fant, sizeof(double) * ((size_t)64 * np + 4 * (size_t)np + (size_t)np * nslices + 64)));
  double *krows = (double *)c->fant.p, *lvec = krows + (size_t)64 * np, *uvec = lvec + np, *evec = uvec + np;
  double *part = evec + np;
  int *status_dev = (int *)(part + (size_t)np * nslices);
  B7_TRY(launch_ksx(c, ctx_fit(c), (const double *)c->xobs.p + (size_t)N * d, 0, 64, 1, d, krows, nullptr, 1));
  B7_TRY(launch_append_vectors(c, krows, lvec, uvec, part, evec));
  B7_TRY(launch_append_finalize(c, krows, lvec, uvec, evec, status_dev));
  int status = 0;
  B7_HIP(c, hipMemcpyAsync(&status, status_dev, sizeof(int), hipMemcpyDeviceToHost, c->stream));
  B7_HIP(c, hipStreamSynchronize(c->stream));
  if (status != 0) {
    B7_TRY(launch_prep_obs(c, (const double *)c->xobs.p, ls_dev, N, d));
    B7_HIP(c, hipStreamSynchronize(c->stream));
    return b7_fail(c, B7_ERR_STATE, "gp_append: the extended matrix is not positive definite; refit with b7_gp_fit");
  }
  c->N = N + 1;
  B7_TRY(launch_alpha(c));
  B7_HIP(c, hipStreamSynchronize(c->stream));
  return B7_OK;
}

int b7_gp_download(b7_ctx *c, double *L_host, double *alpha_host, double *Linv_host) {
  if (!c) return B7_ERR_INVALID;
  if (!c->fitted) return b7_fail(c, B7_ERR_STATE, "gp_download: no fit on this context");
  const size_t N = c->N, np = c->Npad;
  B7_HIP(c, hipStreamSynchronize(c->stream));
  if (L_host)
    B7_HIP(c, hipMemcpy2D(L_host, sizeof(double) * N, c->L.p, sizeof(double) * np, sizeof(double) * N, N,
                          hipMemcpyDeviceToHost));
  if (Linv_host)
    B7_HIP(c, hipMemcpy2D(Linv_host, sizeof(double) * N, c->Linv.p, sizeof(double) * np, sizeof(double) * N, N,
                          hipMemcpyDeviceToHost));
  if (alpha_host)
    B7_HIP(c, hipMemcpy2D(alpha_host, sizeof(double) * c->ycols, c->alpha.p, sizeof(double) * c->yld,
                          sizeof(double) * c->ycols, N, hipMemcpyDeviceToHost));
  return B7_OK;
}

}
```

bot7_amd/csrc/nominate.hip:

```cpp
#include <string.h>

#include <algorithm>

#include "b7_internal.h"

int stage_fmin(b7_ctx *c, const double *fmin, double **fd_out) {
  if (c->ycols == 1) {
    c->fmin_scalar = fmin[0];
    *fd_out = nullptr;
    return B7_OK;
  }
  double *fh = c->pinned->fmin, *fd = b7_scratch(c)->fmin;
  if (!c->fmin_staged || memcmp(fh, fmin, sizeof(double) * c->ycols) != 0) {
    B7_HIP(c, hipStreamSynchronize(c->stream));
    memcpy(fh, fmin, sizeof(double) * c->ycols);
    c->fmin_staged = true;
  }
  B7_HIP(c, hipMemcpyAsync(fd, fh, sizeof(double) * c->ycols, hipMemcpyHostToDevice, c->stream));
  *fd_out = fd;
  return B7_OK;
}

ScoreParams score_params(const b7_ctx *c, const b7_score_spec *spec, const double *fd) {
  ScoreParams p;
// ... 11 lines not shown

int mes_refuse(b7_ctx *c, const char *who, const b7_score_spec *spec) {
  if (spec->kind != B7_SCORE_MES) return B7_OK;
  if (c->comm && c->comm_world > 1)
    return b7_fail(c, B7_ERR_UNSUPPORTED, "%s: max-value entropy search over a communicator of %d ranks is not built (y* over a sharded grid needs an all-reduce per round)", who, c->comm_world);
  if (c->ycols != 1)
    return b7_fail(c, B7_ERR_UNSUPPORTED, "%s: max-value entropy search over %d response columns (fantasies) is not built", who, c->ycols);
  return B7_OK;
}

int score_add(b7_ctx *c, const b7_score_spec *sp, const double *fd, bool accumulate) {
  ScoreParams p = score_params(c, sp, fd);
  if (sp->kind == B7_SCORE_MES)
    B7_TRY(mes_search_for(c, &p, (const double *)c->mu.p, (const double *)c->var.p, 0, 1, c->mes_slot));
  return launch_score(c, p, (const double *)c->mu.p, (const double *)c->var.p, c->M, c->ycols, (double *)c->acc.p, accumulate);
}

int nominate_args(b7_ctx *c, const char *who, const b7_score_spec *spec, int64_t offset) {
  if (spec->kind != B7_SCORE_EI && spec->kind != B7_SCORE_CB && spec->kind != B7_SCORE_LOGEI && spec->kind != B7_SCORE_MES &&
      spec->kind != B7_SCORE_LOGPI)
    return b7_fail(c, B7_ERR_INVALID, "%s: unknown score kind %d", who, spec->kind);
  if (score_needs_fmin(spec->kind) && !spec->fmin)
    return b7_fail(c, B7_ERR_INVALID, "%s: %s needs fmin", who, spec->kind == B7_SCORE_LOGPI ? "LogPI" : "EI");
  if (offset < 0) return b7_fail(c, B7_ERR_INVALID, "%s: negative row offset", who);
  if (c->M == 0 && !(c->comm && c->comm_world > 1) && !c->group)
    return b7_fail(c, B7_ERR_STATE, "%s: no candidate grid on this context", who);
  return B7_OK;
}

int eval_validate(b7_ctx *c, int S, const b7_hyp *hyps, const b7_score_spec *spec, int64_t offset) {
  if (S < 1 || !hyps || !spec) return b7_fail(c, B7_ERR_INVALID, "eval_nominate: S >= 1, hyps and spec required");
  B7_TRY(nominate_args(c, "eval_nominate", spec, offset));
  if (!c->have_data) return b7_fail(c, B7_ERR_STATE, "eval_nominate: call b7_gp_set_data first");
  if (c->M > 0 && c->d != c->dfit)
    return b7_fail(c, B7_ERR_INVALID, "eval_nominate: grid dims %d != data dims %d", c->d, c->dfit);
  for (int s = 0; s < S; ++s) B7_TRY(check_hyp(c, &hyps[s], c->dfit));
  return mes_refuse(c, "eval_nominate", spec);
}

int pending_score(b7_ctx *c, int S, const b7_score_spec *spec, const double *fd, ScoreParams *out) {
  ScoreParams p = score_params(c, spec, fd);
  p.S = S, p.mu = (const double *)c->bmu.p, p.var = (const double *)c->bvar.p, p.stride = c->M;
  if (spec->kind == B7_SCORE_MES) B7_TRY(mes_search_for(c, &p, p.mu, p.var, p.stride, S, 0));
  *out = p;
  return B7_OK;
}

static int keep_slots_ensure(b7_ctx *c, const BelKeep *keep, int S) {
  if (!keep || S == 1) return B7_OK;
  return batch_slots_ensure(c, S, B7_SLOTS_OPERANDS | B7_SLOTS_LINV | (keep->want_alpha ? B7_SLOTS_ALPHA : 0));
}
static int keep_sample(b7_ctx *c, BelKeep *keep, int S, int s, bool in_slot) {
  if (!keep) return B7_OK;
  const size_t mb = sizeof(double) * (size_t)c->M;
  if (keep->mu) {
    B7_HIP(c, hipMemcpyAsync(keep->mu + (size_t)s * c->M, c->mu.p, mb, hipMemcpyDeviceToDevice, c->stream));
    B7_HIP(c, hipMemcpyAsync(keep->var + (size_t)s * c->M, c->var.p, mb, hipMemcpyDeviceToDevice, c->stream));
  }
  if (S == 1 && !in_slot) {
    keep->fits = ctx_fit(c);
    return B7_OK;
  }
  keep->fits = batch_fits(c, S);
  if (in_slot) return B7_OK;
  const FitSet src = ctx_fit(c), dst = fit_at(keep->fits, s, b7_hyp{nullptr, c->amp, c->noise, c->mean});
  const int n = c->Npad, dp = c->dpad;
  auto put = [&](const double *to, const double *from, int64_t doubles) {
    return hipMemcpyAsync(const_cast<double *>(to), from, sizeof(double) * (size_t)doubles, hipMemcpyDeviceToDevice, c->stream);
  };
  if (keep->want_alpha) B7_HIP(c, put(dst.alpha, src.alpha, FitSet::s_alpha(n, dp)));
  B7_HIP(c, put(dst.w, src.w, FitSet::s_w(n, dp)));
  B7_HIP(c, put(dst.zsc, src.zsc, FitSet::s_zsc(n, dp)));
  B7_HIP(c, put(dst.zss, src.zss, FitSet::s_zss(n, dp)));
  B7_HIP(c, put(dst.Linv, src.Linv, FitSet::s_Linv(n, dp)));
  return B7_OK;
}
static int keep_batch(b7_ctx *c, BelKeep *keep, int S) {
  if (!keep) return B7_OK;
  const size_t bytes = sizeof(double) * (size_t)S * c->M;
  if (keep->mu) {
    B7_HIP(c, hipMemcpyAsync(keep->mu, c->bmu.p, bytes, hipMemcpyDeviceToDevice, c->stream));
    B7_HIP(c, hipMemcpyAsync(keep->var, c->bvar.p, bytes, hipMemcpyDeviceToDevice, c->stream));
  }
  keep->fits = batch_fits(c, S);
  return B7_OK;
}

struct EvalStage {
  int *reports, *reports_dev;
  double *hyp_host;
  const double *hyp_map;
  size_t hyp_bytes, rep_bytes;
};
static int eval_stage(b7_ctx *c, int S, const b7_hyp *hyps, EvalStage *st) {
  const int d = c->dfit;
  st->hyp_bytes = sizeof(double) * (size_t)S * (d + 3), st->rep_bytes = 16 * (size_t)S;
  B7_TRY(b7_pin_ensure(c, c->pin_eval, st->hyp_bytes + st->rep_bytes, true));
  B7_TRY(b7_ensure(c, c->bhyp, st->hyp_bytes));
  st->reports = static_cast<int *>(c->pin_eval.host), st->reports_dev = static_cast<int *>(c->pin_eval.dev);
  st->hyp_host = reinterpret_cast<double *>(static_cast<char *>(c->pin_eval.host) + st->rep_bytes);
  st->hyp_map = reinterpret_cast<const double *>(static_cast<const char *>(c->pin_eval.dev) + st->rep_bytes);
  const HypPack hp = hyp_pack(st->hyp_host, S, d);
  for (int s = 0; s < S; ++s) {
    memcpy(hp.ls + (size_t)s * d, hyps[s].lenscale_sq, sizeof(double) * d);
    hp.amp[s] = hyps[s].amp;
    hp.noise[s] = hyps[s].noise;
    hp.mean[s] = hyps[s].mean;
  }
  memset(st->reports, 0xff, st->rep_bytes);
  return B7_OK;
}

static int fits_side_by_side(b7_ctx *c, int S, bool small, const EvalStage &st) {
  double *bw = (double *)c->bw.p, *bzsc = (double *)c->bzsc.p, *bzss = (double *)c->bzss.p, *bLinv = (double *)c->bLinv.p;
  double *balpha = (double *)c->balpha.p;
  int *binfo = (int *)c->binfo.p;
  if (small)
    return launch_fit_small(c, S, st.hyp_map, st.hyp_host, (double *)c->bhyp.p, bw, bzsc, bzss, nullptr, bLinv, nullptr, balpha, nullptr,
                            binfo, st.reports_dev);
  const int n = c->Npad;
  const int64_t sq = FitSet::s_Linv(n, c->dpad);
  const HypPack hd = hyp_pack(c->bhyp.p, S, c->dfit);
  const double *bK = (const double *)c->bK.p, *bresid = (const double *)c->bresid.p;
  double *bL = (double *)c->bL.p, *bdinv = (double *)c->bdinv.p;
  launch_resid_batch(c, S, hd.mean);
  B7_TRY(launch_kxx_batch(c, S, hd.ls, hd.amp, hd.noise, bw, bzsc, bzss, (double *)c->bK.p));
  if (n == 64 && c->potrf_small)
    return launch_potrf_small(c, S, bK, bL, bLinv, bdinv, bresid, balpha, 0.0, binfo, st.reports_dev, sq, sq, (int64_t)n * B7_PANEL,
                              FitSet::s_alpha(n, c->dpad), 4);
  B7_TRY(launch_fit_batch(c, S, bK, bL, bLinv, bdinv, (unsigned *)c->bflags.p, binfo));
  if (4 * S <= 256)
    return launch_alpha_batch(c, S, bLinv, bresid, balpha, binfo, st.reports_dev, 4 * S);
  B7_TRY(launch_alpha_batch(c, S, bLinv, bresid, balpha));
  B7_HIP(c, hipMemcpyAsync(st.reports, binfo, st.rep_bytes, hipMemcpyDeviceToHost, c->stream));
  return B7_OK;
}

static int post_side_by_side_small(b7_ctx *c, int S, const b7_score_spec *spec, const double *fd, ScoreParams *pend, BelKeep *keep) {
  B7_TRY(b7_ensure(c, c->bmu, sizeof(double) * (size_t)S * c->M));
  B7_TRY(b7_ensure(c, c->bvar, sizeof(double) * (size_t)S * c->M));
  B7_TRY(launch_kpost_small(c, batch_fits(c, S), (const double *)c->grid[c->grid_cur].p, c->M, (double *)c->bmu.p, (double *)c->bvar.p, c->M));
  B7_TRY(keep_batch(c, keep, S));
  B7_TRY(pending_score(c, S, spec, fd, pend));
  c->fitted = false;
  c->predicted = false;
  return B7_OK;
}
static int post_side_by_side(b7_ctx *c, int S, const b7_score_spec *spec, const double *fd, BelKeep *keep) {
  const int64_t Mpad = round_up(c->M, B7_MROWS), sks = Mpad * c->Npad;
  const FitSet fits = batch_fits(c, S);
  B7_TRY(b7_ensure(c, c->ks, sizeof(double) * (size_t)sks * S));
  B7_TRY(b7_ensure(c, c->bmu, sizeof(double) * (size_t)S * c->M));
  B7_TRY(b7_ensure(c, c->bvar, sizeof(double) * (size_t)S * c->M));
  B7_TRY(launch_ksx_batch(c, fits, (const double *)c->grid[c->grid_cur].p, Mpad, c->M, (double *)c->ks.p, sks, (double *)c->bmu.p, c->M));
  B7_TRY(launch_post_batch(c, fits, (const double *)c->ks.p, sks, Mpad, c->M, (double *)c->bvar.p, c->M));
  B7_TRY(keep_batch(c, keep, S));
  ScoreParams all;
  B7_TRY(pending_score(c, S, spec, fd, &all));
  B7_TRY(launch_score_batch(c, all, (double *)c->acc.p, c->M));
  c->fitted = false;
  c->predicted = false;
  return B7_OK;
}
static int post_in_turn(b7_ctx *c, int S, const b7_hyp *hyps, const b7_score_spec *spec, const double *fd, BelKeep *keep) {
  const FitSet fits = batch_fits(c, S);
  c->model_kind = 0;
  int rc = B7_OK;
  for (int s = 0; s < S && rc == B7_OK; ++s) {
    c->amp = hyps[s].amp, c->noise = hyps[s].noise, c->mean = hyps[s].mean;
    rc = predict_into(c, fit_at(fits, s, hyps[s]), (const double *)c->grid[c->grid_cur].p, c->M, (double *)c->mu.p, (double *)c->var.p);
    c->mes_slot = s;
    if (rc == B7_OK) rc = score_add(c, spec, fd);
    if (rc == B7_OK) rc = keep_sample(c, keep, S, s, true);
  }
  c->fitted = false;
  c->predicted = true;
  c->Mpred = c->M;
  return rc;
}

static int fits_in_turn(b7_ctx *c, int S, const b7_hyp *hyps, const b7_score_spec *spec, const double *fd, BelKeep *keep) {
  B7_TRY(keep_slots_ensure(c, keep, S));
  for (int s = 0; s < S; ++s) {
    B7_TRY(fit_front(c, &hyps[s], (const double *)c->bhyp.p + (size_t)s * c->dfit));
    int *report = static_cast<int *>(c->pin_eval.dev) + 4 * s;
    FactorNote note;
    B7_TRY(launch_potrf(c, 0.0, true, report, &note));
    if (!c->linv_done) B7_TRY(launch_trtri(c));
    B7_TRY(launch_alpha(c, report, 4, note));
    c->fitted = true;
    B7_TRY(predict_into(c, ctx_fit(c), (const double *)c->grid[c->grid_cur].p, c->M, (double *)c->mu.p, (double *)c->var.p));
    c->predicted = true;
    c->Mpred = c->M;
    c->mes_slot = s;
    B7_TRY(score_add(c, spec, fd));
    B7_TRY(keep_sample(c, keep, S, s, false));
  }
  c->fitted = false;
  return B7_OK;
}

int eval_enqueue(b7_ctx *c, int S, const b7_hyp *hyps, const b7_score_spec *spec, ScoreParams *pend, BelKeep *keep) {
  B7_HIP(c, hipSetDevice(c->device));
  B7_TRY(b7_ensure(c, c->mu, sizeof(double) * (size_t)c->M * c->ycols));
  B7_TRY(b7_ensure(c, c->var, sizeof(double) * (size_t)c->M));
  B7_TRY(b7_ensure(c, c->acc, sizeof(double) * (size_t)c->M));
  B7_TRY(b7_ensure(c, c->ks, sizeof(double) * (size_t)predict_chunk(c, c->M) * c->Npad));
  if (spec->kind == B7_SCORE_MES) B7_TRY(mes_begin(c, S, c->M, c->mes_levels));
  EvalStage st;
  B7_TRY(eval_stage(c, S, hyps, &st));
  const bool small = fit_small_applies(c);
  const bool batch = small || (S > 1 && c->ycols == 1 && c->potrf_sched == 3 && c->Npad <= B7_PERSIST_NMAX && c->inverse_inline);
  if (batch) {
    B7_TRY(batch_slots_ensure(c, S, B7_SLOTS_OPERANDS | B7_SLOTS_LINV | B7_SLOTS_ALPHA | (small ? 0 : B7_SLOTS_FACTOR)));
    B7_TRY(b7_ensure(c, c->binfo, sizeof(int) * 4 * (size_t)S));
    if (!small) B7_TRY(b7_ensure(c, c->bflags, sizeof(unsigned) * S * persist_flag_words_host(c->Npad / B7_PANEL)));
  }
  if (!small) B7_HIP(c, hipMemcpyAsync(c->bhyp.p, st.hyp_host, st.hyp_bytes, hipMemcpyHostToDevice, c->stream));
  double *fd = nullptr;
  if (score_needs_fmin(spec->kind)) B7_TRY(stage_fmin(c, spec->fmin, &fd));
  acc_declare_zeros(c, spec->kind);
  if (!batch) return fits_in_turn(c, S, hyps, spec, fd, keep);
  B7_TRY(fits_side_by_side(c, S, small, st));
  if (c->kpost_small && kpost_small_applies(c)) return post_side_by_side_small(c, S, spec, fd, pend, keep);
  if ((size_t)round_up(c->M, B7_MROWS) * S * sizeof(double) * (size_t)c->Npad <= c->ks_bytes) return post_side_by_side(c, S, spec, fd, keep);
  return post_in_turn(c, S, hyps, spec, fd, keep);
}

bool reports_clean(b7_ctx *c, const int *reports, int S, bool persist) {
  bool clean = true, aborted = false;
  for (int s = 0; s < S; ++s) {
    clean = clean && reports[4 * s] == 0 && reports[4 * s + 1] == 0;
    aborted = aborted || reports[4 * s + 1] != 0;
  }
  if (aborted && persist) persist_gave_up(c);
  return clean;
}

int eval_redo(b7_ctx *c, int S, const b7_hyp *hyps, const b7_score_spec *spec, double *jitter_out, int *info_out, BelKeep *keep) {
  B7_HIP(c, hipSetDevice(c->device));
  B7_TRY(keep_slots_ensure(c, keep, S));
  B7_TRY(acc_write_zeros(c));
  if (spec->kind == B7_SCORE_MES) B7_TRY(mes_begin(c, S, c->M, c->mes_levels));
  double *fd = nullptr;
  for (int s = 0; s < S; ++s) {
    B7_TRY(fit_hyp_core(c, &hyps[s], nullptr, jitter_out ? jitter_out + s : nullptr, info_out ? info_out + s : nullptr, true));
    c->predicted = true;
    c->Mpred = c->M;
    if (score_needs_fmin(spec->kind)) B7_TRY(stage_fmin(c, spec->fmin, &fd));
    c->mes_slot = s;
    B7_TRY(score_add(c, spec, fd));
    B7_TRY(keep_sample(c, keep, S, s, false));
  }
  return B7_OK;
}

static int score_ready(b7_ctx *c, const char *who) {
  if (!c->predicted || c->Mpred != c->M) return b7_fail(c, B7_ERR_STATE, "%s: call b7_gp_predict first", who);
  if (!c->acc_valid) return b7_fail(c, B7_ERR_STATE, "%s: call b7_score_reset first", who);
  return B7_OK;
}

static int upload_mv(b7_ctx *c, const double *mean, const double *var, int64_t M, int cc) {
  B7_TRY(b7_ensure(c, c->tmpmu, sizeof(double) * (size_t)M * cc));
  B7_TRY(b7_ensure(c, c->tmpvar, sizeof(double) * (size_t)M));
  B7_TRY(b7_ensure(c, c->tmpgrid, sizeof(double) * (size_t)M));
  B7_HIP(c, hipMemcpyAsync(c->tmpmu.p, mean, sizeof(double) * (size_t)M * cc, hipMemcpyHostToDevice, c->stream));
  B7_HIP(c, hipMemcpyAsync(c->tmpvar.p, var, sizeof(double) * (size_t)M, hipMemcpyHostToDevice, c->stream));
  return B7_OK;
}

static int score_compute(b7_ctx *c, const b7_score_spec &spec, const double *mean, const double *var, int64_t M, int cc, double *out) {
  if (M == 0) return B7_OK;
  B7_HIP(c, hipSetDevice(c->device));
  B7_TRY(upload_mv(c, mean, var, M, cc));
  double *fd = nullptr;
  if (score_needs_fmin(spec.kind)) {
    fd = b7_scratch(c)->fmin;
    B7_HIP(c, hipMemcpyAsync(fd, spec.fmin, sizeof(double) * cc, hipMemcpyHostToDevice, c->stream));
  }
  B7_TRY(launch_score(c, score_params(c, &spec, fd), (const double *)c->tmpmu.p, (const double *)c->tmpvar.p, M, cc,
                      (double *)c->tmpgrid.p, false));
  B7_HIP(c, hipMemcpyAsync(out, c->tmpgrid.p, sizeof(double) * (size_t)M, hipMemcpyDeviceToHost, c->stream));
  B7_HIP(c, hipStreamSynchronize(c->stream));
  return B7_OK;
}

extern "C" {

int b7_eval_nominate(b7_ctx *c, int S, const b7_hyp *hyps, const b7_score_spec *spec, int64_t global_row_offset,
                     double *best_val, int64_t *best_idx1, double *jitter_out, int *info_out) {
  if (!c) return B7_ERR_INVALID;
  if (c->group) return b7_fail(c, B7_ERR_STATE, "eval_nominate: this context belongs to a group (b7_group_eval_nominate)");
  if (jitter_out && S > 0) std::fill(jitter_out, jitter_out + S, 0.0);
  if (info_out && S > 0) std::fill(info_out, info_out + S, 0);
  if (spec && spec->kind == B7_SCORE_MES && c->comm && c->comm_world > 1) return mes_refuse(c, "eval_nominate", spec);
  return nominate_run(
      c, "eval_nominate", eval_validate(c, S, hyps, spec, global_row_offset), global_row_offset, (double)S,
      [&](ScoreParams *pend) { return eval_enqueue(c, S, hyps, spec, pend); },
      [&]() { return reports_clean(c, static_cast<const int *>(c->pin_eval.host), S, true); },
      [&]() { return eval_redo(c, S, hyps, spec, jitter_out, info_out); }, best_val, best_idx1);
}

int b7_eval_nominate_feasible(b7_ctx *c, int S, const b7_hyp *hyps, const b7_score_spec *spec, double *best_val, int64_t *best_idx1,
                              double *jitter_out, int *info_out) {
  if (!c) return B7_ERR_INVALID;
  if (c->group) return b7_fail(c, B7_ERR_STATE, "eval_nominate_feasible: this context belongs to a group (constrained nomination over a sharded grid is not built)");
  if (jitter_out && S > 0) std::fill(jitter_out, jitter_out + S, 0.0);
// ... 182 lines not shown
```

bot7_amd/csrc/posterior.hip:

```cpp
#include "b7_internal.h"
#include "post_ring_layout.h"
#include <utility>

#ifdef B7_POST_STAMPS
__device__ unsigned long long b7_post_stamps[4 * 4096];
extern "C" int b7dbg_post_stamps(unsigned long long *out, int nblocks) {
  return (int)hipMemcpyFromSymbol(out, HIP_SYMBOL(b7_post_stamps), sizeof(unsigned long long) * 4 * nblocks);
}
#endif

typedef double d2_t __attribute__((ext_vector_type(2)));

struct PostBatch {
  int64_t sLinv = 0, sks = 0, svar = 0;
  const double *base = nullptr, *var_add = nullptr;
};

namespace w4 {
constexpr int BM = 128, BK = 16, LD = BK + 1, A_DBL = BM * LD;

#define B7_W4_ACC_REGS \
  "a0", "a1", "a2", "a3", "a4", "a5", "a6", "a7", "a8", "a9", "a10", "a11", "a12", "a13", "a14", "a15", \
  "a16", "a17", "a18", "a19", "a20", "a21", "a22", "a23", "a24", "a25", "a26", "a27", "a28", "a29", "a30", \
  "a31", "a32", "a33", "a34", "a35", "a36", "a37", "a38", "a39", "a40", "a41", "a42", "a43", "a44", "a45", \
  "a46", "a47", "a48", "a49", "a50", "a51", "a52", "a53", "a54", "a55", "a56", "a57", "a58", "a59", "a60", \
  "a61", "a62", "a63", "a64", "a65", "a66", "a67", "a68", "a69", "a70", "a71", "a72", "a73", "a74", "a75", \
  "a76", "a77", "a78", "a79", "a80", "a81", "a82", "a83", "a84", "a85", "a86", "a87", "a88", "a89", "a90", \
  "a91", "a92", "a93", "a94", "a95", "a96", "a97", "a98", "a99", "a100", "a101", "a102", "a103", "a104", \
  "a105", "a106", "a107", "a108", "a109", "a110", "a111", "a112", "a113", "a114", "a115", "a116", "a117", \
  "a118", "a119", "a120", "a121", "a122", "a123", "a124", "a125", "a126", "a127", "a128", "a129", "a130", \
  "a131", "a132", "a133", "a134", "a135", "a136", "a137", "a138", "a139", "a140", "a141", "a142", "a143", \
  "a144", "a145", "a146", "a147", "a148", "a149", "a150", "a151", "a152", "a153", "a154", "a155", "a156", \
  "a157", "a158", "a159", "a160", "a161", "a162", "a163", "a164", "a165", "a166", "a167", "a168", "a169", \
  "a170", "a171", "a172", "a173", "a174", "a175", "a176", "a177", "a178", "a179", "a180", "a181", "a182", \
  "a183", "a184", "a185", "a186", "a187", "a188", "a189", "a190", "a191", "a192", "a193", "a194", "a195", \
  "a196", "a197", "a198", "a199", "a200", "a201", "a202", "a203", "a204", "a205", "a206", "a207", "a208", \
  "a209", "a210", "a211", "a212", "a213", "a214", "a215", "a216", "a217", "a218", "a219", "a220", "a221", \
  "a222", "a223", "a224", "a225", "a226", "a227", "a228", "a229", "a230", "a231", "a232", "a233", "a234", \
  "a235", "a236", "a237", "a238", "a239", "a240", "a241", "a242", "a243", "a244", "a245", "a246", "a247", \
  "a248", "a249", "a250", "a251", "a252", "a253", "a254", "a255"

template <int NJ, int I, int J, bool ZERO>
__device__ __forceinline__ void mfma_tile(double a, double b) {
  constexpr int lo = 8 * (NJ * I + J);
  if constexpr (ZERO)
    asm volatile("v_mfma_f64_16x16x4_f64 a[%2:%3], %0, %1, 0" ::"v"(a), "v"(b), "n"(lo), "n"(lo + 7) : B7_W4_ACC_REGS);
  else
    asm volatile("v_mfma_f64_16x16x4_f64 a[%2:%3], %0, %1, a[%2:%3]" ::"v"(a), "v"(b), "n"(lo), "n"(lo + 7)
                 : B7_W4_ACC_REGS);
}

template <int NJ, int I, int J>
__device__ __forceinline__ void read_tile(double (&v)[4]) {
  constexpr int lo = 8 * (NJ * I + J);
  unsigned w[8];
  asm volatile(
      "v_accvgpr_read_b32 %0, a[%8]\n\tv_accvgpr_read_b32 %1, a[%9]\n\tv_accvgpr_read_b32 %2, a[%10]\n\t"
      "v_accvgpr_read_b32 %3, a[%11]\n\tv_accvgpr_read_b32 %4, a[%12]\n\tv_accvgpr_read_b32 %5, a[%13]\n\t"
      "v_accvgpr_read_b32 %6, a[%14]\n\tv_accvgpr_read_b32 %7, a[%15]"
      : "=v"(w[0]), "=v"(w[1]), "=v"(w[2]), "=v"(w[3]), "=v"(w[4]), "=v"(w[5]), "=v"(w[6]), "=v"(w[7])
      : "n"(lo), "n"(lo + 1), "n"(lo + 2), "n"(lo + 3), "n"(lo + 4), "n"(lo + 5), "n"(lo + 6), "n"(lo + 7));
#pragma unroll
  for (int r = 0; r < 4; ++r) v[r] = __hiloint2double((int)w[2 * r + 1], (int)w[2 * r]);
}

template <int NJ>
struct Frags {
  double a[2][8], b[2][NJ];
};
template <int NJ>
struct Stage {
  d2_t c[4 + 2 * NJ];
};
struct Cursor {
  int t, kb, ntiles;
  __device__ __forceinline__ void advance() {
    if (kb + 1 < (t + 1) * (BM / BK)) {
      ++kb;
    } else if (t + 1 < ntiles) {
      ++t;
      kb = 0;
    }
  }
};

template <int N, class F, int... Is>
__device__ __forceinline__ void static_for_impl(F &&f, std::integer_sequence<int, Is...>) {
  (f(std::integral_constant<int, Is>{}), ...);
}
template <int N, class F>
__device__ __forceinline__ void static_for(F &&f) {
  static_for_impl<N>(f, std::make_integer_sequence<int, N>{});
}

template <int NJ, int P, int S0>
__device__ __forceinline__ void read_pair(Frags<NJ> &f, const double *__restrict__ sa, const double *__restrict__ sb) {
  if constexpr (P < NJ) {
    f.b[0][P] = sb[P * 16 * LD + 4 * S0];
    f.b[1][P] = sb[P * 16 * LD + 4 * S0 + 4];
  } else {
    f.a[0][P - NJ] = sa[(P - NJ) * 16 * LD + 4 * S0];
    f.a[1][P - NJ] = sa[(P - NJ) * 16 * LD + 4 * S0 + 4];
  }
}

template <int NJ, int C>
__device__ __forceinline__ void load_chunk(Stage<NJ> &g, const double *__restrict__ qa, const double *__restrict__ qb,
                                           int64_t lda) {
  if constexpr (C < 4)
    g.c[C] = *reinterpret_cast<const d2_t *>(qa + (int64_t)(32 * C) * lda);
  else
    g.c[C] = *reinterpret_cast<const d2_t *>(qb + (int64_t)(32 * (C - 4)) * lda);
}
template <int NJ, int C>
__device__ __forceinline__ void store_chunk(const Stage<NJ> &g, double *__restrict__ w) {
  constexpr int o = C < 4 ? 32 * C * LD : A_DBL + 32 * (C - 4) * LD;
  w[o] = g.c[C][0];
  w[o + 1] = g.c[C][1];
}

template <int NJ, int FIRST, bool ZERO>
__device__ __forceinline__ void stage(Frags<NJ> &f0, Frags<NJ> &f1, Stage<NJ> &g, double *__restrict__ cur,
                                      double *__restrict__ nxt, int fa, int fb, int wofs, const double *__restrict__ pa,
                                      const double *__restrict__ pb, int64_t lda, Cursor &ld) {
  constexpr int NI = 8 - FIRST, NM = 2 * NJ * NI, NP = 8 + NJ, NC = 4 + 2 * NJ, NS = NP + 2 * NC;
  const double *qa = pa + ((int64_t)ld.t * BM) * lda + ld.kb * BK, *qb = pb + ld.kb * BK;
  ld.advance();
  constexpr int K1 = (NS + NM - 1) / NM + 1, K2 = (NP + NM - 1) / NM + 1;
  static_for<NM>([&](auto m_) {
    constexpr int m = decltype(m_)::value, ks = m / (NJ * NI), i = FIRST + (m % (NJ * NI)) / NJ, j = m % NJ;
    mfma_tile<NJ, i, j, ZERO && ks == 0>(f0.a[ks][i], f0.b[ks][j]);
    static_for<K1>([&](auto k_) {
      constexpr int sidx = m * NS / NM + decltype(k_)::value;
      if constexpr (sidx < (m + 1) * NS / NM) {
        if constexpr (sidx < NP) {
          if constexpr (sidx < NJ || sidx - NJ >= FIRST) read_pair<NJ, sidx, 2>(f1, cur + fa, cur + fb);
        } else if constexpr (sidx < NP + NC) {
          store_chunk<NJ, sidx - NP>(g, nxt + wofs);
        } else {
          load_chunk<NJ, sidx - NP - NC>(g, qa, qb, lda);
        }
      }
    });
  });
  __builtin_amdgcn_s_waitcnt(0xC07F);
  __builtin_amdgcn_s_barrier();
  static_for<NM>([&](auto m_) {
    constexpr int m = decltype(m_)::value, ks = m / (NJ * NI), i = FIRST + (m % (NJ * NI)) / NJ, j = m % NJ;
    mfma_tile<NJ, i, j, false>(f1.a[ks][i], f1.b[ks][j]);
    static_for<K2>([&](auto k_) {
      constexpr int sidx = m * NP / NM + decltype(k_)::value;
      if constexpr (sidx < (m + 1) * NP / NM) read_pair<NJ, sidx, 0>(f0, nxt + fa, nxt + fb);
    });
  });
}

template <int NJ>
__global__ void __launch_bounds__(256)
    post_kernel_w4(const double *__restrict__ Linv, const double *__restrict__ ks, int Npad, int64_t row0, int64_t Mtotal,
                   double base, double sgn, double var_add, int clamp, double var_min, double *__restrict__ var,
                   PostBatch bat) {
  constexpr int BN = 64 * NJ, STAGE_DBL = (BM + BN) * LD, NC = 4 + 2 * NJ, NP = 8 + NJ;
  extern __shared__ __align__(16) double sm[];
  if (bat.base) {
    const int64_t y = blockIdx.y;
    Linv += y * bat.sLinv;
    ks += y * bat.sks;
    var += y * bat.svar;
    base = bat.base[y];
    if (bat.var_add) var_add = bat.var_add[y];
  }
  const int lane = threadIdx.x & 63, wave = __builtin_amdgcn_readfirstlane(threadIdx.x >> 6);
#ifdef B7_POST_STAMPS
  const unsigned long long st0 = __builtin_amdgcn_s_memtime(), sr0 = __builtin_amdgcn_s_memrealtime();
  __builtin_amdgcn_s_waitcnt(0xC07F);
#endif
  const int64_t lda = Npad;
  const int r0 = threadIdx.x >> 3, kc = threadIdx.x & 7;
  const double *pa = Linv + (int64_t)r0 * lda + 2 * kc;
  const double *pb = ks + ((int64_t)blockIdx.x * BN + r0) * lda + 2 * kc;
  const int wofs = r0 * LD + 2 * kc;
  const int fa = (lane & 15) * LD + (lane >> 4);
  const int fb = A_DBL + (wave * 16 * NJ + (lane & 15)) * LD + (lane >> 4);

  const int ntiles = Npad / BM;
  Cursor ld{0, 0, ntiles};
  Stage<NJ> g;
  Frags<NJ> f0, f1;
  double *const b0 = sm, *const b1 = sm + STAGE_DBL;
  static_for<NC>([&](auto c_) { load_chunk<NJ, decltype(c_)::value>(g, pa, pb, lda); });
  ld.advance();
  static_for<NC>([&](auto c_) { store_chunk<NJ, decltype(c_)::value>(g, b0 + wofs); });
  {
    const double *qa = pa + ((int64_t)ld.t * BM) * lda + ld.kb * BK, *qb = pb + ld.kb * BK;
    static_for<NC>([&](auto c_) { load_chunk<NJ, decltype(c_)::value>(g, qa, qb, lda); });
    ld.advance();
  }
  __builtin_amdgcn_s_waitcnt(0xC07F);
  __builtin_amdgcn_s_barrier();
  static_for<NP>([&](auto p_) { read_pair<NJ, decltype(p_)::value, 0>(f0, b0 + fa, b0 + fb); });

  double colss[2][NJ] = {};
#define B7_STAGE(F, Z, CUR, NXT) stage<NJ, F, Z>(f0, f1, g, CUR, NXT, fa, fb, wofs, pa, pb, lda, ld)
  for (int t = 0; t < ntiles; ++t) {
    B7_STAGE(0, true, b0, b1);
    if (t > 0) {
      for (int p = 0; p < 4 * t - 1; ++p) {
        B7_STAGE(0, false, b1, b0);
        B7_STAGE(0, false, b0, b1);
      }
      B7_STAGE(0, false, b1, b0);
      B7_STAGE(0, false, b0, b1);
    }
    B7_STAGE(1, false, b1, b0);
    B7_STAGE(2, false, b0, b1);
    B7_STAGE(3, false, b1, b0);
    B7_STAGE(4, false, b0, b1);
    B7_STAGE(5, false, b1, b0);
    B7_STAGE(6, false, b0, b1);
    B7_STAGE(7, false, b1, b0);
    asm volatile("s_nop 15\n\ts_nop 15\n\ts_nop 15" ::: "memory");
    static_for<2 * NJ>([&](auto hj_) {
      constexpr int h = decltype(hj_)::value / NJ, j = decltype(hj_)::value % NJ;
      double s = 0.0;
      static_for<4>([&](auto i_) {
        double v[4];
        read_tile<NJ, 4 * h + decltype(i_)::value, j>(v);
#pragma unroll
        for (int r = 0; r < 4; ++r) s = __builtin_fma(v[r], v[r], s);
      });
      colss[h][j] += s;
    });
  }
#undef B7_STAGE

#pragma unroll
  for (int j = 0; j < NJ; ++j) {
    double v0 = colss[0][j], v1 = colss[1][j];
    v0 += __shfl_xor(v0, 16);
    v0 += __shfl_xor(v0, 32);
    v1 += __shfl_xor(v1, 16);
    v1 += __shfl_xor(v1, 32);
    const int64_t gidx = row0 + (int64_t)blockIdx.x * BN + wave * 16 * NJ + j * 16 + lane;
    if (lane < 16 && gidx < Mtotal) {
      double ss = v0;
      ss += v1;
      double v = (base + sgn * ss) + var_add;
      if (clamp) v = (v < var_min) ? var_min : v;
      var[gidx] = v;
    }
  }
#ifdef B7_POST_STAMPS
  if (threadIdx.x == 0 && blockIdx.x < 4096) {
    const unsigned long long st1 = __builtin_amdgcn_s_memtime(), sr1 = __builtin_amdgcn_s_memrealtime();
    __builtin_amdgcn_s_waitcnt(0xC07F);
    unsigned long long *o = b7_post_stamps + 4 * blockIdx.x;
    o[0] = st0, o[1] = sr0, o[2] = st1, o[3] = sr1;
  }
#endif
}

template <int NJ>
constexpr int lds_bytes() { return 2 * (BM + 64 * NJ) * LD * 8; }

template <int NJ, int NR>
struct Tall {
  static constexpr int BMT = 16 * NR, BN = 64 * NJ, ROWS = BMT + BN;
  static constexpr int STAGE_BYTES = ROWS * post_ring::ROW_BYTES, NBUF = 3;
  static constexpr int ND = ROWS / post_ring::PIECE_ROWS / post_ring::WAVES;
  static constexpr int NDA = BMT / post_ring::PIECE_ROWS / post_ring::WAVES;
  static constexpr int NP = NR + NJ;
  static constexpr int LDS_BYTES = NBUF * STAGE_BYTES;
  static_assert(NJ * NR == 32, "32 accumulator tiles per wave");
  static_assert(ND == 12 && ND % 3 == 0, "vmcnt(12) below is ND; a third of the pieces per k-step");
  static_assert(LDS_BYTES <= 160 * 1024, "three stage images in 160 KiB");

  struct Set {
    double a[NR], b[NJ];
  };
  typedef __attribute__((address_space(3))) double lds_double;
  struct Lane {
    int fa[NBUF][4], fb[NBUF][4];
    unsigned src, dst[NBUF];
    __device__ __forceinline__ void rotate1() {
#pragma unroll
      for (int s = 0; s < 4; ++s) {
        const int a = fa[0][s], b = fb[0][s];
        fa[0][s] = fa[1][s], fa[1][s] = fa[2][s], fa[2][s] = a;
        fb[0][s] = fb[1][s], fb[1][s] = fb[2][s], fb[2][s] = b;
      }
      const unsigned d = dst[0];
      dst[0] = dst[1], dst[1] = dst[2], dst[2] = d;
    }
    __device__ __forceinline__ void rotate(int k) {
      if (k >= 1) rotate1();
      if (k >= 2) rotate1();
    }
  };
  struct Cursor {
    int t, kb, ntiles;
    __device__ __forceinline__ void advance() {
      if (kb + 1 < (t + 1) * (BMT / BK)) {
        ++kb;
      } else if (t + 1 < ntiles) {
        ++t;
        kb = 0;
      }
    }
  };

  template <int P, int S, int B>
  static __device__ __forceinline__ void read_one(Set &f, const Lane &ln) {
    constexpr int strip = (P < NJ ? P : P - NJ) * 16 * post_ring::ROW_BYTES;
    if constexpr (P < NJ)
      f.b[P] = *reinterpret_cast<const lds_double *>((uintptr_t)(unsigned)(ln.fb[B][S] + strip));
    else
      f.a[P - NJ] = *reinterpret_cast<const lds_double *>((uintptr_t)(unsigned)(ln.fa[B][S] + strip));
  }
  template <int C>
  static __device__ __forceinline__ void dma_piece(const char *__restrict__ ga, const char *__restrict__ gb, int64_t step,
                                                   unsigned src, unsigned dst) {
    const char *g = C < NDA ? ga + C * step : gb + (C - NDA) * step;
    const unsigned m0 = dst + C * post_ring::WAVES * post_ring::PIECE_BYTES;
    asm volatile("s_mov_b32 m0, %0\n\ts_nop 0\n\tglobal_load_lds_dwordx4 %1, %2" ::"s"(m0), "v"(src), "s"(g) : "memory");
  }

  template <int FIRST, bool ZERO, int NSIDE, int TAIL, class Side>
  static __device__ __forceinline__ void kstep(const Set &use, Side &&side) {
    constexpr int NI = NR - FIRST, NM = NJ * NI, NMS = NM > 2 * TAIL ? NM - TAIL : NM;
    constexpr int KMAX = (NSIDE + NMS - 1) / NMS + 1;
    static_for<NM>([&](auto m_) {
      constexpr int m = decltype(m_)::value, i = FIRST + m / NJ, j = m % NJ;
      mfma_tile<NJ, i, j, ZERO>(use.a[i], use.b[j]);
      if constexpr (m < NMS)
        static_for<KMAX>([&](auto k_) {
          constexpr int sidx = m * NSIDE / NMS + decltype(k_)::value;
          if constexpr (sidx < (m + 1) * NSIDE / NMS) side(std::integral_constant<int, sidx>{});
        });
    });
  }
  static constexpr int H = ND / 3, NS = NP + H;
  static constexpr int dma_before(int x) {
    int n = 0;
    for (int d = 0; d < H; ++d) n += (d + 1) * NS / (H + 1) < x;
    return n;
  }
  static constexpr bool is_dma(int x) { return dma_before(x + 1) > dma_before(x); }

  template <int FIRST, int NEXT_FIRST, bool ZERO, int POS>
  static __device__ __forceinline__ void stage(Set &s0, Set &s1, const Lane &ln,
                                               const char *__restrict__ pa, const char *__restrict__ pb, int64_t lda, Cursor &ld) {
    constexpr int CUR = POS % NBUF, NXT = (POS + 1) % NBUF, DST = (POS + 2) % NBUF;
    const int64_t step = 32 * lda * 8;
    const char *ga = pa + (((int64_t)ld.t * BMT) * lda + ld.kb * BK) * 8, *gb = pb + (int64_t)(ld.kb * BK) * 8;
    ld.advance();
    auto sides = [&](auto ks_, Set &into, auto x_) {
      constexpr int ks = decltype(ks_)::value, x = decltype(x_)::value, r = x - dma_before(x);
      if constexpr (is_dma(x))
        dma_piece<H * ks + dma_before(x)>(ga, gb, step, ln.src, ln.dst[DST]);
      else if constexpr (r < NJ || r - NJ >= FIRST)
        read_one<r, ks + 1, CUR>(into, ln);
    };
    kstep<FIRST, ZERO, NS, 0>(s0, [&](auto x_) { sides(std::integral_constant<int, 0>{}, s1, x_); });
    kstep<FIRST, false, NS, 0>(s1, [&](auto x_) { sides(std::integral_constant<int, 1>{}, s0, x_); });
    kstep<FIRST, false, NS, 3>(s0, [&](auto x_) { sides(std::integral_constant<int, 2>{}, s1, x_); });
    asm volatile("s_waitcnt vmcnt(12) lgkmcnt(0)" ::: "memory");
    __builtin_amdgcn_s_barrier();
    kstep<FIRST, false, NP, 0>(s1, [&](auto s_) {
      constexpr int x = decltype(s_)::value;
      if constexpr (x < NJ || x - NJ >= NEXT_FIRST) read_one<x, 0, NXT>(s0, ln);
    });
  }
};

template <int NJ, int NR>
__global__ void __launch_bounds__(256)
    post_kernel_w4t(const double *__restrict__ Linv, const double *__restrict__ ks, int Npad, int64_t row0, int64_t Mtotal,
                    double base, double sgn, double var_add, int clamp, double var_min, double *__restrict__ var,
                    PostBatch bat) {
  using T = Tall<NJ, NR>;
  constexpr int BMT = T::BMT, BN = T::BN, NP = T::NP;
  extern __shared__ __align__(16) double sm[];
  if (bat.base) {
    const int64_t y = blockIdx.y;
    Linv += y * bat.sLinv;
    ks += y * bat.sks;
    var += y * bat.svar;
    base = bat.base[y];
    if (bat.var_add) var_add = bat.var_add[y];
  }
  const int lane = threadIdx.x & 63, wave = __builtin_amdgcn_readfirstlane(threadIdx.x >> 6);
#ifdef B7_POST_STAMPS
  const unsigned long long st0 = __builtin_amdgcn_s_memtime(), sr0 = __builtin_amdgcn_s_memrealtime();
  __builtin_amdgcn_s_waitcnt(0xC07F);
#endif
  const int64_t lda = Npad;
  const char *pa = reinterpret_cast<const char *>(Linv + (int64_t)(post_ring::PIECE_ROWS * wave) * lda);
  const char *pb = reinterpret_cast<const char *>(ks + ((int64_t)blockIdx.x * BN + post_ring::PIECE_ROWS * wave) * lda);
  typename T::Lane ln;
  {
    const post_ring::Chunk c = post_ring::dma_src(wave, lane);
    ln.src = (unsigned)(((c.row - post_ring::PIECE_ROWS * wave) * Npad + 2 * c.chunk) * 8);
  }
  const unsigned lds0 = (unsigned)(uintptr_t)(__attribute__((address_space(3))) void *)sm;
#pragma unroll
  for (int b = 0; b < T::NBUF; ++b) {
#pragma unroll
    for (int s = 0; s < 4; ++s) {
      ln.fa[b][s] = lds0 + b * T::STAGE_BYTES + post_ring::frag_byte(lane & 15, 4 * s + (lane >> 4));
      ln.fb[b][s] = ln.fa[b][s] + (BMT + wave * 16 * NJ) * post_ring::ROW_BYTES;
      asm volatile("" : "+v"(ln.fa[b][s]), "+v"(ln.fb[b][s]));
    }
    ln.dst[b] = lds0 + b * T::STAGE_BYTES + wave * post_ring::PIECE_BYTES;
  }

  const int ntiles = Npad / BMT;
  typename T::Cursor ld{0, 0, ntiles};
  typename T::Set s0, s1;
  {
    const int64_t step = 32 * lda * 8;
    static_for<T::ND>([&](auto c_) { T::template dma_piece<decltype(c_)::value>(pa, pb, step, ln.src, ln.dst[0]); });
    ld.advance();
    const char *ga = pa + (((int64_t)ld.t * BMT) * lda + ld.kb * BK) * 8, *gb = pb + (int64_t)(ld.kb * BK) * 8;
    static_for<T::ND>([&](auto c_) { T::template dma_piece<decltype(c_)::value>(ga, gb, step, ln.src, ln.dst[1]); });
    ld.advance();
  }
  asm volatile("s_waitcnt vmcnt(12)" ::: "memory");
  __builtin_amdgcn_s_barrier();
  static_for<NP>([&](auto p_) { T::template read_one<decltype(p_)::value, 0, 0>(s0, ln); });

  double colss[2][NJ] = {};
#define B7_STAGE(F, NF, Z, POS) T::template stage<F, NF, Z, POS>(s0, s1, ln, pa, pb, lda, ld)
  for (int t = 0; t < ntiles; ++t) {
    B7_STAGE(0, 0, true, 0);
    if (t > 0) {
      const int n = NR * t - 1;
      for (int p = 0; p < n / 3; ++p) {
        B7_STAGE(0, 0, false, 1);
        B7_STAGE(0, 0, false, 2);
        B7_STAGE(0, 0, false, 0);
      }
      if (n % 3 >= 1) B7_STAGE(0, 0, false, 1);
      if (n % 3 == 2) B7_STAGE(0, 0, false, 2);
      ln.rotate((n + 1) % 3);
      B7_STAGE(0, 1, false, 0);
    }
    static_for<NR - 1>([&](auto q_) {
      constexpr int Q = decltype(q_)::value + 1;
      B7_STAGE(Q, (Q + 1) % NR, false, Q % 3);
    });
    ln.rotate(NR % 3);
    asm volatile("s_nop 15\n\ts_nop 15\n\ts_nop 15" ::: "memory");
    static_for<(NR / 4) * NJ>([&](auto qj_) {
      constexpr int q = decltype(qj_)::value / NJ, j = decltype(qj_)::value % NJ;
      double s = 0.0;
      static_for<4>([&](auto i_) {
        double v[4];
        read_tile<NJ, 4 * q + decltype(i_)::value, j>(v);
#pragma unroll
        for (int r = 0; r < 4; ++r) s = __builtin_fma(v[r], v[r], s);
      });
      colss[q & 1][j] += s;
    });
  }
#undef B7_STAGE
  asm volatile("s_waitcnt vmcnt(0)" ::: "memory");

#pragma unroll
  for (int j = 0; j < NJ; ++j) {
    double v0 = colss[0][j], v1 = colss[1][j];
    v0 += __shfl_xor(v0, 16);
    v0 += __shfl_xor(v0, 32);
    v1 += __shfl_xor(v1, 16);
    v1 += __shfl_xor(v1, 32);
    const int64_t gidx = row0 + (int64_t)blockIdx.x * BN + wave * 16 * NJ + j * 16 + lane;
    if (lane < 16 && gidx < Mtotal) {
      double ss = v0;
      ss += v1;
      double v = (base + sgn * ss) + var_add;
      if (clamp) v = (v < var_min) ? var_min : v;
      var[gidx] = v;
    }
  }
#ifdef B7_POST_STAMPS
  if (threadIdx.x == 0 && blockIdx.x < 4096) {
    const unsigned long long st1 = __builtin_amdgcn_s_memtime(), sr1 = __builtin_amdgcn_s_memrealtime();
    __builtin_amdgcn_s_waitcnt(0xC07F);
    unsigned long long *o = b7_post_stamps + 4 * blockIdx.x;
    o[0] = st0, o[1] = sr0, o[2] = st1, o[3] = sr1;
  }
#endif
}
}

namespace small64 {
typedef double d4_t __attribute__((ext_vector_type(4)));
constexpr int NB = 64, LLD = NB + 2, BN = 64;
constexpr int LDS_BYTES = BN * LLD * 8;

__global__ void __launch_bounds__(256)
    post_small_kernel(const double *__restrict__ Linv, const double *__restrict__ ks, int64_t row0, int64_t Mtotal, int ntiles,
                      double base, double sgn, double var_add, int clamp, double var_min, double *__restrict__ var, PostBatch bat) {
  extern __shared__ __align__(16) double sm[];
  if (bat.base) {
    const int64_t y = blockIdx.y;
    Linv += y * bat.sLinv;
    ks += y * bat.sks;
    var += y * bat.svar;
    base = bat.base[y];
    if (bat.var_add) var_add = bat.var_add[y];
  }
  double *Ks = sm;
  const int tid = threadIdx.x, lane = tid & 63, wave = tid >> 6, lr = lane & 15, lq = lane >> 4;
  d2_t pv[BN / 8];
  auto fetch = [&](int tile) {
    const double *kt = ks + ((int64_t)tile * BN) * NB;
#pragma unroll
    for (int i = 0; i < BN / 8; ++i) {
      const int e = tid + 256 * i;
      pv[i] = *reinterpret_cast<const d2_t *>(kt + (int64_t)(e >> 5) * NB + 2 * (e & 31));
    }
  };
  int tile = blockIdx.x;
  if (tile < ntiles) fetch(tile);
  double af[40];
#pragma unroll
  for (int I = 0; I < 4; ++I)
#pragma unroll
    for (int k4 = 0; k4 < 4 * (I + 1); ++k4) af[2 * I * (I + 1) + k4] = Linv[(int64_t)(I * 16 + lr) * NB + 4 * k4 + lq];
#pragma unroll
  for (int g = 0; g < 4; ++g)
    asm volatile("" : "+v"(af[10 * g]), "+v"(af[10 * g + 1]), "+v"(af[10 * g + 2]), "+v"(af[10 * g + 3]), "+v"(af[10 * g + 4]),
                      "+v"(af[10 * g + 5]), "+v"(af[10 * g + 6]), "+v"(af[10 * g + 7]), "+v"(af[10 * g + 8]), "+v"(af[10 * g + 9]));
  for (; tile < ntiles; tile += gridDim.x) {
#pragma unroll
    for (int i = 0; i < BN / 8; ++i) {
      const int e = tid + 256 * i, r = e >> 5, c2 = 2 * (e & 31);
      Ks[r * LLD + c2] = pv[i][0];
      Ks[r * LLD + c2 + 1] = pv[i][1];
    }
    __syncthreads();
    if (tile + (int)gridDim.x < ntiles) fetch(tile + gridDim.x);
    __builtin_amdgcn_sched_barrier(0);
    constexpr int NJ = BN / 64;
    double ss[NJ];
#pragma unroll
    for (int j = 0; j < NJ; ++j) {
      const double *bp = Ks + (wave * 16 * NJ + j * 16 + lr) * LLD + lq;
      double bf[16];
#pragma unroll
      for (int k4 = 0; k4 < 16; ++k4) bf[k4] = bp[4 * k4];
      double s = 0.0;
#pragma unroll
      for (int I = 0; I < 4; ++I) {
        d4_t c = {0.0, 0.0, 0.0, 0.0};
#ifdef B7_PS_ABLATE
        c = __builtin_amdgcn_mfma_f64_16x16x4f64(af[2 * I * (I + 1)], bf[I], c, 0, 0, 0);
#else
#pragma unroll
        for (int k4 = 0; k4 < 4 * (I + 1); ++k4) c = __builtin_amdgcn_mfma_f64_16x16x4f64(af[2 * I * (I + 1) + k4], bf[k4], c, 0, 0, 0);
#endif
#pragma unroll
        for (int r = 0; r < 4; ++r) s = __builtin_fma(c[r], c[r], s);
      }
      ss[j] = s;
    }
#pragma unroll
    for (int j = 0; j < NJ; ++j) {
      double v = ss[j];
      v += __shfl_xor(v, 16);
      v += __shfl_xor(v, 32);
      const int64_t gidx = row0 + (int64_t)tile * BN + wave * 16 * NJ + j * 16 + lr;
      if (lane < 16 && gidx < Mtotal) {
        double o = (base + sgn * v) + var_add;
        if (clamp) o = (o < var_min) ? var_min : o;
        var[gidx] = o;
      }
    }
    __syncthreads();
  }
}
}

#ifndef B7_POST_NO_LAUNCHERS
namespace {
struct PostArgs {
  const double *Linv, *ks;
  double *var;
  double base, sgn, var_add;
  int S;
  PostBatch pb;
};

template <int NJ>
int launch_post_w4(b7_ctx *c, const PostArgs &a, int64_t row0, int64_t rows, int64_t Mtotal) {
  constexpr int lds = w4::lds_bytes<NJ>();
  B7_HIP(c, hipFuncSetAttribute(reinterpret_cast<const void *>(w4::post_kernel_w4<NJ>),
                                hipFuncAttributeMaxDynamicSharedMemorySize, lds));
  hipLaunchKernelGGL(w4::post_kernel_w4<NJ>, dim3((unsigned)(rows / (64 * NJ)), a.S), dim3(256), lds, c->stream, a.Linv, a.ks,
                     c->Npad, row0, Mtotal, a.base, a.sgn, a.var_add, c->opts.var_clamp, c->opts.var_min, a.var, a.pb);
  B7_HIP(c, hipGetLastError());
  return B7_OK;
}

template <int NJ, int NR>
int launch_post_tall(b7_ctx *c, const PostArgs &a, int64_t row0, int64_t rows, int64_t Mtotal) {
  using T = w4::Tall<NJ, NR>;
  auto kern = w4::post_kernel_w4t<NJ, NR>;
  B7_HIP(c, hipFuncSetAttribute(reinterpret_cast<const void *>(kern), hipFuncAttributeMaxDynamicSharedMemorySize,
                                T::LDS_BYTES));
  hipLaunchKernelGGL(kern, dim3((unsigned)(rows / T::BN), a.S), dim3(256), T::LDS_BYTES, c->stream, a.Linv, a.ks, c->Npad, row0,
                     Mtotal, a.base, a.sgn, a.var_add, c->opts.var_clamp, c->opts.var_min, a.var, a.pb);
  B7_HIP(c, hipGetLastError());
  return B7_OK;
}

int launch_post_small(b7_ctx *c, const PostArgs &a, int64_t row0, int64_t rows, int64_t Mtotal) {
  B7_HIP(c, hipFuncSetAttribute(reinterpret_cast<const void *>(small64::post_small_kernel), hipFuncAttributeMaxDynamicSharedMemorySize,
                                small64::LDS_BYTES));
  const int ntiles = (int)(rows / small64::BN), S = a.S > 0 ? a.S : 1;
  int gx = (2 * c->cus + S - 1) / S;
  if (gx > ntiles) gx = ntiles;
  if (gx < 1) gx = 1;
  hipLaunchKernelGGL(small64::post_small_kernel, dim3((unsigned)gx, S), dim3(256), small64::LDS_BYTES, c->stream, a.Linv, a.ks, row0,
                     Mtotal, ntiles, a.base, a.sgn, a.var_add, c->opts.var_clamp, c->opts.var_min, a.var, a.pb);
  B7_HIP(c, hipGetLastError());
  return B7_OK;
}

int dispatch_post(b7_ctx *c, const PostArgs &a, int64_t row0, int64_t rows, int64_t Mtotal) {
  if (rows % B7_MROWS) return b7_fail(c, B7_ERR_INVALID, "post: rows %lld not a multiple of %d", (long long)rows, B7_MROWS);
  if (c->Npad == 64) return launch_post_small(c, a, row0, rows, Mtotal);
  const bool large = rows / 256 * a.S >= c->cus;
  if (c->Npad % 256 == 0 && large) return launch_post_tall<2, 16>(c, a, row0, rows, Mtotal);
  if (!large) return launch_post_w4<2>(c, a, row0, rows, Mtotal);
  return launch_post_w4<4>(c, a, row0, rows, Mtotal);
}
}

int launch_post(b7_ctx *c, const FitSet &f, const double *ks, int64_t row0, int64_t rows, int64_t Mtotal, double *var) {
  PhaseScope ps(c, "post");
  const bool blr = c->model_kind == 1;
  PostArgs a{f.Linv, ks, var, blr ? 0.0 : f.amp, blr ? 1.0 : -1.0, blr ? f.noise : (c->opts.var_with_noise ? f.noise : 0.0), 1,
             PostBatch{}};
  return dispatch_post(c, a, row0, rows, Mtotal);
}

int launch_post_batch(b7_ctx *c, const FitSet &f, const double *ks, int64_t sks, int64_t rows, int64_t Mtotal, double *var,
                      int64_t svar) {
  PhaseScope ps(c, "post");
  PostArgs a{f.Linv, ks, var, 0.0, -1.0, 0.0, f.S, PostBatch{}};
  a.pb.sLinv = FitSet::s_Linv(c->Npad, c->dpad);
  a.pb.sks = sks;
  a.pb.svar = svar;
  a.pb.base = f.amp_dev;
  a.pb.var_add = c->opts.var_with_noise ? f.noise_dev : nullptr;
  return dispatch_post(c, a, 0, rows, Mtotal);
}

int launch_post_heads(b7_ctx *c, int S, const double *Linv, const double *feat, int64_t rows, int64_t Mtotal, double *var, int64_t svar,
                      const double *zero_dev, const double *invbeta_dev) {
  PhaseScope ps(c, "post");
  PostArgs a{Linv, feat, var, 0.0, 1.0, 0.0, S, PostBatch{}};
  a.pb.sLinv = FitSet::s_Linv(c->Npad, c->dpad);
  a.pb.sks = 0;
  a.pb.svar = svar;
  a.pb.base = zero_dev;
  a.pb.var_add = invbeta_dev;
  return dispatch_post(c, a, 0, rows, Mtotal);
}
#endif
```

bot7_amd/csrc/rff.hip:

```cpp
#include <math.h>
#include <string.h>

#include <vector>

#include "b7_internal.h"
#include "counter_rng.h"
#include "gemm_f64.h"

namespace {

constexpr int RT = 2;
constexpr int RROWS = 4 * 16 * RT;

__host__ __device__ constexpr int rff_dpad(int d) { return d <= 8 ? 8 : d <= 16 ? 16 : d <= 32 ? 32 : d <= 64 ? 64 : 96; }

__device__ __forceinline__ double rff_cos(double x) {
  const double n = __builtin_rint(x * 6.36619772367581382433e-01);
  double r = __builtin_fma(-n, 1.57079632679489655800e+00, x);
  r = __builtin_fma(-n, 6.12323399573676603587e-17, r);
  const double z = r * r;
  double ps = 1.58969099521155010221e-10;
  ps = __builtin_fma(ps, z, -2.50507602534068634195e-08);
  ps = __builtin_fma(ps, z, 2.75573137070700676789e-06);
  ps = __builtin_fma(ps, z, -1.98412698298579493134e-04);
// ... 92 lines not shown
    }
  }
#pragma unroll
  for (int t = 0; t < RT; ++t) {
    const int64_t g = row0 + 16 * t + lr;
    if (g >= M) continue;
#pragma unroll
    for (int r = 0; r < 4; ++r) {
      const int p = lq + 4 * r;
      if (p < qn) out[g * ldo + ocol0 + (int64_t)p * ostride] = (base ? base[g * ldb + p] : 0.0) + acc[t][r];
    }
  }
}

__global__ void __launch_bounds__(256) ts_basis_kernel(uint64_t key, int F, int d, int matern, const double *__restrict__ inv_ls,
                                                       double *__restrict__ omega, double *__restrict__ phase) {
  const int64_t e = (int64_t)blockIdx.x * blockDim.x + threadIdx.x;
  if (e >= (int64_t)F * d) return;
  const int f = (int)(e / d), k = (int)(e - (int64_t)f * d);
  double v = counter_normal(key, (uint64_t)f * 128 + (uint64_t)k);
  if (matern) {
    double u = 0.0;
    for (int i = 0; i < 5; ++i) {
      const double g = counter_normal(key, (uint64_t)f * 128 + 96 + (uint64_t)i);
      u += g * g;
    }
    v = v * sqrt(5.0 / u);
  }
  omega[e] = v * inv_ls[k];
  if (phase && k == 0) phase[f] = 6.283185307179586476925 * counter_uniform(key, (uint64_t)f * 128 + 101);
}

__global__ void __launch_bounds__(256) ts_path_draws_kernel(uint64_t seed, int q, int F, int N, double *__restrict__ weight,
                                                            double *__restrict__ zeps) {
  const int64_t e = (int64_t)blockIdx.x * blockDim.x + threadIdx.x;
  const int64_t per = (int64_t)F + N;
  if (e >= per * q) return;
  const int j = (int)(e / per);
  const int64_t i = e - (int64_t)j * per;
  const uint64_t key = counter_key(seed, 1 + (uint64_t)j);
  if (i < F)
    weight[(int64_t)j * F + i] = counter_normal(key, (uint64_t)i);
  else
    zeps[(int64_t)j * N + (i - F)] = counter_normal(key, 4096 + (uint64_t)(i - F));
}

__global__ void __launch_bounds__(256) ts_pseudo_kernel(const double *__restrict__ y, const double *__restrict__ phiw, double *__restrict__ eps,
                                                        int N, int qs, int s, int S, double sd_noise, double *__restrict__ ycols) {
  const int e = blockIdx.x * blockDim.x + threadIdx.x;
  if (e >= N * qs) return;
  const int i = e / qs, p = e - i * qs;
  double *ej = eps + (int64_t)(s + S * p) * N + i;
  const double ev = sd_noise * *ej;
  *ej = ev;
  ycols[e] = (y[i] - phiw[e]) - ev;
}

struct TsBest { double v; long long i; };
__device__ __forceinline__ bool ts_better(double av, long long ai, double bv, long long bi) {
  if (ai < 0) return false;
  if (bi < 0) return true;
  const bool an = av != av, bn = bv != bv;
  if (an != bn) return bn;
  if (!an && av != bv) return av < bv;
  return ai < bi;
}
__device__ __forceinline__ void ts_block_reduce(double &v, long long &i, TsBest *sm) {
  const int t = threadIdx.x;
  sm[t].v = v, sm[t].i = i;
  __syncthreads();
  for (int s = 128; s > 0; s >>= 1) {
    if (t < s && ts_better(sm[t + s].v, sm[t + s].i, sm[t].v, sm[t].i)) sm[t] = sm[t + s];
    __syncthreads();
  }
  v = sm[0].v, i = sm[0].i;
}
__global__ void __launch_bounds__(256) ts_argmin_part_kernel(const double *__restrict__ paths, int64_t M, int q, int j,
                                                             const long long *__restrict__ taken, TsBest *__restrict__ part) {
  __shared__ TsBest sm[256];
  long long tk[B7_BATCH_MAX];
  for (int i = 0; i < j; ++i) tk[i] = taken[i];
  double bv = 0.0;
  long long bi = -1;
  for (int64_t g = (int64_t)blockIdx.x * 256 + threadIdx.x; g < M; g += (int64_t)gridDim.x * 256) {
    bool skip = false;
    for (int i = 0; i < j; ++i) skip = skip || tk[i] == g;
    if (skip) continue;
    const double v = paths[g * q + j];
    if (ts_better(v, g, bv, bi)) bv = v, bi = g;
  }
  ts_block_reduce(bv, bi, sm);
  if (threadIdx.x == 0) part[blockIdx.x].v = bv, part[blockIdx.x].i = bi;
}
__global__ void __launch_bounds__(256) ts_argmin_final_kernel(const TsBest *__restrict__ part, int nblk, int j, long long *__restrict__ taken,
                                                              double *__restrict__ pmin) {
  __shared__ TsBest sm[256];
  double bv = 0.0;
  long long bi = -1;
  for (int b = threadIdx.x; b < nblk; b += 256)
    if (ts_better(part[b].v, part[b].i, bv, bi)) bv = part[b].v, bi = part[b].i;
  ts_block_reduce(bv, bi, sm);
  if (threadIdx.x == 0) taken[j] = bi, pmin[j] = bv;
}

template <int DPAD>
void rff_launch_class(b7_ctx *c, const double *X, int64_t M, int d, const double *omf, const double *phase, const double *wf, int F,
                      const double *base, int ldb, double *out, int ldo, int ocol0, int ostride, int qn) {
  hipLaunchKernelGGL(rff_kernel<DPAD>, dim3((unsigned)((M + RROWS - 1) / RROWS)), dim3(256), 0, c->stream, X, M, d, omf, phase, wf, F / 16,
                     base, ldb, out, ldo, ocol0, ostride, qn);
}

int launch_rff(b7_ctx *c, const double *X, int64_t M, int d, const double *omf, const double *phase, const double *wf, int F,
               const double *base, int ldb, double *out, int ldo, int ocol0, int ostride, int qn) {
  PhaseScope ps(c, "rff");
  if (M <= 0) return B7_OK;
  switch (rff_dpad(d)) {
    case 8: rff_launch_class<8>(c, X, M, d, omf, phase, wf, F, base, ldb, out, ldo, ocol0, ostride, qn); break;
    case 16: rff_launch_class<16>(c, X, M, d, omf, phase, wf, F, base, ldb, out, ldo, ocol0, ostride, qn); break;
    case 32: rff_launch_class<32>(c, X, M, d, omf, phase, wf, F, base, ldb, out, ldo, ocol0, ostride, qn); break;
    case 64: rff_launch_class<64>(c, X, M, d, omf, phase, wf, F, base, ldb, out, ldo, ocol0, ostride, qn); break;
    default: rff_launch_class<96>(c, X, M, d, omf, phase, wf, F, base, ldb, out, ldo, ocol0, ostride, qn); break;
  }
  B7_HIP(c, hipGetLastError());
  return B7_OK;
}

int launch_rff_pack(b7_ctx *c, const double *omega, int F, int d, const double *W, int64_t ldw, int64_t col0, int64_t cstride, int qn,
                    double scale, double *omf, double *wf) {
  const int dpad = rff_dpad(d);
  const int64_t total = (int64_t)F * (dpad + 16);
  hipLaunchKernelGGL(rff_pack_kernel, dim3((unsigned)((total + 255) / 256)), dim3(256), 0, c->stream, omega, F, d, dpad, W, ldw, col0,
                     cstride, qn, scale, omf, wf);
  B7_HIP(c, hipGetLastError());
  return B7_OK;
}

struct TsDraws { double *omega, *phase, *weight, *eps; };
TsDraws ts_draws(const b7_ctx *c, int ns, int q, int F, int d, int N) {
  TsDraws t;
  t.omega = (double *)c->ts_draw.p;
  t.phase = t.omega + (size_t)ns * F * d;
  t.weight = t.phase + F;
  t.eps = t.weight + (size_t)q * F;
  (void)N;
  return t;
}

int ts_mean_over_grid(b7_ctx *c) {
  const int64_t M = c->M, chunk = predict_chunk(c, M), Mpad = round_up(M, B7_MROWS);
  B7_TRY(b7_ensure(c, c->ks, sizeof(double) * (size_t)chunk * c->Npad));
  const double *grid = (const double *)c->grid[c->grid_cur].p;
  for (int64_t row0 = 0; row0 < M; row0 += chunk) {
    const int64_t rows = Mpad - row0 < chunk ? Mpad - row0 : chunk;
    B7_TRY(launch_ksx(c, ctx_fit(c), grid, row0, rows, M, c->dfit, (double *)c->ks.p, (double *)c->mu.p, c->ycols));
    if (c->ycols > 1) B7_TRY(launch_mean_multi(c, ctx_fit(c), (const double *)c->ks.p, row0, rows, M, (double *)c->mu.p));
  }
  return B7_OK;
}

struct YSwap {
  b7_ctx *c;
  DevBuf ybuf, alpha, resid;
  int ycols, yld;
  explicit YSwap(b7_ctx *c) : c(c), ybuf(c->ybuf), alpha(c->alpha), resid(c->resid), ycols(c->ycols), yld(c->yld) {}
  ~YSwap() {
    c->ybuf = ybuf, c->alpha = alpha, c->resid = resid, c->ycols = ycols, c->yld = yld;
    c->fitted = false;
    c->predicted = false;
  }
};

}

extern "C" {

int b7_ts_nominate(b7_ctx *c, int S, const b7_hyp *hyps, int q, int F, uint64_t seed, double *path_min, int64_t *best_idx1,
                   double *jitter_out, int *info_out) {
  if (!c) return B7_ERR_INVALID;
  if (c->group) return b7_fail(c, B7_ERR_STATE, "ts_nominate: this context belongs to a group (sharded Thompson sampling is not built)");
  if (q < 1 || q > B7_BATCH_MAX) return b7_fail(c, B7_ERR_INVALID, "ts_nominate: q = %d not in [1, %d]", q, B7_BATCH_MAX);
  if (F < 16 || F > B7_TS_MAX_FEATURES || F % 16)
    return b7_fail(c, B7_ERR_INVALID, "ts_nominate: F = %d features: a multiple of 16 in [16, %d]", F, B7_TS_MAX_FEATURES);
  if (S < 1) return b7_fail(c, B7_ERR_INVALID, "ts_nominate: S = %d hyper samples (at least one)", S);
  if (!hyps || !path_min || !best_idx1) return b7_fail(c, B7_ERR_INVALID, "ts_nominate: NULL argument (hyps, path_min and best_idx1 are needed)");
  if (c->comm && c->comm_world > 1)
    return b7_fail(c, B7_ERR_UNSUPPORTED, "ts_nominate: a communicator of %d ranks (sharded Thompson sampling is not built)", c->comm_world);
  if (!c->have_data) return b7_fail(c, B7_ERR_STATE, "ts_nominate: no resident data (call b7_gp_set_data first)");
  if (c->M <= 0) return b7_fail(c, B7_ERR_STATE, "ts_nominate: no candidate grid on this context");
  if (c->ycols != 1) return b7_fail(c, B7_ERR_UNSUPPORTED, "ts_nominate: %d response columns (one is built)", c->ycols);
  if (c->d != c->dfit) return b7_fail(c, B7_ERR_INVALID, "ts_nominate: grid dims %d != data dims %d", c->d, c->dfit);
  if (q > c->M) return b7_fail(c, B7_ERR_INVALID, "ts_nominate: q = %d exceeds the grid's %lld rows", q, (long long)c->M);
  const int ns = S < q ? S : q, N = c->N, d = c->dfit, dpad = rff_dpad(d), np = c->Npad;
  for (int s = 0; s < ns; ++s) B7_TRY(check_hyp(c, &hyps[s], d));
  B7_HIP(c, hipSetDevice(c->device));
  const int64_t M = c->M;
  if (jitter_out) std::fill(jitter_out, jitter_out + S, 0.0);
  if (info_out) std::fill(info_out, info_out + S, 0);
  c->ts_valid = false;

  const int qmax = (q + ns - 1) / ns, yldmax = qmax == 1 ? 1 : (int)round_up(qmax, 64);
  const int nblk = (int)std::min<int64_t>(1024, (M + 255) / 256);
  B7_TRY(b7_ensure(c, c->ts_paths, sizeof(double) * (size_t)M * q));
  B7_TRY(b7_ensure(c, c->ts_draw, sizeof(double) * ((size_t)ns * F * d + F + (size_t)q * F + (size_t)q * N)));
  const size_t pieces[10] = {(size_t)F * dpad, 16 * (size_t)F, (size_t)N * qmax, (size_t)np * qmax, (size_t)np * yldmax, (size_t)np * qmax,
                             (size_t)d,        (size_t)q,      (size_t)q,        2 * (size_t)nblk};
  size_t off[11] = {0};
  for (int i = 0; i < 10; ++i) off[i + 1] = off[i] + (size_t)round_up((int64_t)pieces[i], 32);
  B7_TRY(b7_ensure(c, c->ts_work, sizeof(double) * off[10]));
  const TsDraws dr = ts_draws(c, ns, q, F, d, N);
  double *wk = (double *)c->ts_work.p;
  double *omf = wk + off[0], *wf = wk + off[1], *phiw = wk + off[2], *ycols = wk + off[3], *alpha = wk + off[4], *resid = wk + off[5];
  double *inv_ls = wk + off[6], *pmin = wk + off[7];
  long long *taken = reinterpret_cast<long long *>(wk + off[8]);
  TsBest *part = reinterpret_cast<TsBest *>(wk + off[9]);
  double *paths = (double *)c->ts_paths.p;
  const double *grid = (const double *)c->grid[c->grid_cur].p;

  {
    const int64_t total = ((int64_t)F + N) * q;
    hipLaunchKernelGGL(ts_path_draws_kernel, dim3((unsigned)((total + 255) / 256)), dim3(256), 0, c->stream, seed, q, F, N, dr.weight, dr.eps);
    B7_HIP(c, hipGetLastError());
  }
  const uint64_t key0 = counter_key(seed, 0);
  std::vector<double> ils(d);
  {
    YSwap swap(c);
    for (int s = 0; s < ns; ++s) {
      const int qs = (q - s + S - 1) / S;
      const b7_hyp &h = hyps[s];
      for (int k = 0; k < d; ++k) ils[k] = 1.0 / sqrt(h.lenscale_sq[k]);
      B7_HIP(c, hipMemcpyAsync(inv_ls, ils.data(), sizeof(double) * d, hipMemcpyHostToDevice, c->stream));
      B7_HIP(c, hipStreamSynchronize(c->stream));
      double *omega = dr.omega + (size_t)s * F * d;
      {
        PhaseScope ps(c, "ts_draws");
        hipLaunchKernelGGL(ts_basis_kernel, dim3((unsigned)(((int64_t)F * d + 255) / 256)), dim3(256), 0, c->stream, key0, F, d,
                           c->kernel == B7_KERNEL_MATERN52 ? 1 : 0, (const double *)inv_ls, omega, s == 0 ? dr.phase : (double *)nullptr);
        B7_HIP(c, hipGetLastError());
        B7_TRY(launch_rff_pack(c, omega, F, d, dr.weight + (size_t)s * F, 1, 0, (int64_t)S * F, qs, sqrt(2.0 * h.amp / F), omf, wf));
      }
      B7_TRY(launch_rff(c, (const double *)c->xobs.p, N, d, omf, dr.phase, wf, F, nullptr, 0, phiw, qs, 0, 1, qs));
      hipLaunchKernelGGL(ts_pseudo_kernel, dim3((unsigned)((N * qs + 255) / 256)), dim3(256), 0, c->stream, (const double *)swap.ybuf.p,
                         (const double *)phiw, dr.eps, N, qs, s, S, sqrt(h.noise), ycols);
      B7_HIP(c, hipGetLastError());
      c->ybuf.p = ycols, c->alpha.p = alpha, c->resid.p = resid;
      c->ycols = qs;
      c->yld = qs == 1 ? 1 : (int)round_up(qs, 64);
      double jit = 0.0;
      int info = 0;
      B7_TRY(fit_hyp_core(c, &h, nullptr, &jit, &info, false));
      if (jitter_out) jitter_out[s] = jit;
      if (info_out) info_out[s] = info;
      B7_TRY(b7_ensure(c, c->mu, sizeof(double) * (size_t)M * qs));
      B7_TRY(ts_mean_over_grid(c));
      B7_TRY(launch_rff(c, grid, M, d, omf, dr.phase, wf, F, (const double *)c->mu.p, qs, paths, q, s, S, qs));
    }
  }
  {
    PhaseScope ps(c, "ts_argmin");
    for (int j = 0; j < q; ++j) {
      hipLaunchKernelGGL(ts_argmin_part_kernel, dim3(nblk), dim3(256), 0, c->stream, (const double *)paths, M, q, j, (const long long *)taken, part);
      hipLaunchKernelGGL(ts_argmin_final_kernel, dim3(1), dim3(256), 0, c->stream, (const TsBest *)part, nblk, j, taken, pmin);
    }
    B7_HIP(c, hipGetLastError());
  }
  long long tk[B7_BATCH_MAX];
  B7_HIP(c, hipMemcpyAsync(path_min, pmin, sizeof(double) * q, hipMemcpyDeviceToHost, c->stream));
  B7_HIP(c, hipMemcpyAsync(tk, taken, sizeof(long long) * q, hipMemcpyDeviceToHost, c->stream));
  B7_HIP(c, hipStreamSynchronize(c->stream));
  for (int j = 0; j < q; ++j) best_idx1[j] = tk[j] + 1;
  c->ts_valid = true;
  c->ts_M = M, c->ts_q = q, c->ts_S = S, c->ts_F = F, c->ts_N = N, c->ts_d = d;
  return B7_OK;
}

int b7_ts_last_paths(b7_ctx *c, double *paths_host) {
  if (!c) return B7_ERR_INVALID;
  if (!paths_host) return b7_fail(c, B7_ERR_INVALID, "ts_last_paths: NULL argument");
  if (!c->ts_valid) return b7_fail(c, B7_ERR_STATE, "ts_last_paths: no successful b7_ts_nominate on this context");
  B7_HIP(c, hipSetDevice(c->device));
  B7_HIP(c, hipMemcpyAsync(paths_host, c->ts_paths.p, sizeof(double) * (size_t)c->ts_M * c->ts_q, hipMemcpyDeviceToHost, c->stream));
  B7_HIP(c, hipStreamSynchronize(c->stream));
  return B7_OK;
}

int b7_ts_last_draws(b7_ctx *c, int path, double *omega, double *phase, double *weight, double *eps) {
  if (!c) return B7_ERR_INVALID;
  if (!c->ts_valid) return b7_fail(c, B7_ERR_STATE, "ts_last_draws: no successful b7_ts_nominate on this context");
  if (path < 0 || path >= c->ts_q) return b7_fail(c, B7_ERR_INVALID, "ts_last_draws: path %d not in [0, %d)", path, c->ts_q);
  B7_HIP(c, hipSetDevice(c->device));
  const int F = c->ts_F, d = c->ts_d, N = c->ts_N, ns = c->ts_S < c->ts_q ? c->ts_S : c->ts_q;
  const TsDraws dr = ts_draws(c, ns, c->ts_q, F, d, N);
  if (omega) B7_HIP(c, hipMemcpyAsync(omega, dr.omega + (size_t)(path % c->ts_S) * F * d, sizeof(double) * (size_t)F * d, hipMemcpyDeviceToHost, c->stream));
  if (phase) B7_HIP(c, hipMemcpyAsync(phase, dr.phase, sizeof(double) * F, hipMemcpyDeviceToHost, c->stream));
  if (weight) B7_HIP(c, hipMemcpyAsync(weight, dr.weight + (size_t)path * F, sizeof(double) * F, hipMemcpyDeviceToHost, c->stream));
  if (eps) B7_HIP(c, hipMemcpyAsync(eps, dr.eps + (size_t)path * N, sizeof(double) * N, hipMemcpyDeviceToHost, c->stream));
  B7_HIP(c, hipStreamSynchronize(c->stream));
  return B7_OK;
}

int b7_rff_compute(b7_ctx *c, const double *X, int64_t M1, int d, const double *omega, const double *phase, const double *W, int F, int q,
                   double *out) {
  if (!c) return B7_ERR_INVALID;
  if (!X || !omega || !phase || !W || !out) return b7_fail(c, B7_ERR_INVALID, "rff_compute: NULL argument");
  if (M1 < 1 || d < 1 || d > B7_MAX_D) return b7_fail(c, B7_ERR_INVALID, "rff_compute: M1 = %lld rows, d = %d (1..%d)", (long long)M1, d, B7_MAX_D);
  if (q < 1 || q > B7_BATCH_MAX) return b7_fail(c, B7_ERR_INVALID, "rff_compute: q = %d not in [1, %d]", q, B7_BATCH_MAX);
  if (F < 16 || F > B7_TS_MAX_FEATURES || F % 16)
// ... 20 lines not shown
```

Before: 16.48 million.

## Store K* in tiled piece order so the tall posterior kernel DMAs contiguous tiles

Adds a tiled K* layout in which the covariance kernel writes each 16x16 tile contiguously, in the order the tall posterior kernel's DMA ring consumes it. The posterior kernel gains a TILED variant that reads pieces from tile offsets and uses a matching LDS fragment mapping. The aim is to replace strided row-major global loads with contiguous ones and to simplify the ksx store. Selection runs through ks_buf_for for single-output GP predict and batch nominate. The change adds layout coupling between two kernels plus new validity checks that can reject some shapes.

```diff
diff --git a/bot7_amd/build.py b/bot7_amd/build.py
--- a/bot7_amd/build.py
+++ b/bot7_amd/build.py
@@ -11,7 +11,7 @@
 SOURCES = ["context.hip", "grid_api.hip", "gp_api.hip", "nominate.hip", "blr_api.hip", "sobol.hip", "covar.hip", "potrf.hip", "potrf_persist.hip", "posterior.hip", "score.hip", "extras.hip", "comm.hip", "group.hip", "blr_small.hip", "gp_small.hip", "kpost_small.hip", "batch.hip", "mes.hip", "rff.hip", "slice.hip", "refine.hip", "kg.hip", "ehvi.hip", "trust_region.hip"]
 DIAG_ONLY_SOURCES = ["nll_small.hip"]
 DIAG_OUT = os.path.join(ROOT, "tools", "_build", "libbot7hip_diag.so")
-HEADERS = [os.path.join(CSRC, "b7_internal.h"), os.path.join(CSRC, "gemm_f64.h"), os.path.join(CSRC, "potrf_diag.h"), os.path.join(CSRC, "comm_rccl.h"), os.path.join(CSRC, "ksx_exp.h"), os.path.join(CSRC, "ksx_walk.h"), os.path.join(CSRC, "exp_table.h"), os.path.join(CSRC, "mes_math.h"), os.path.join(CSRC, "counter_rng.h"), os.path.join(CSRC, "gp_small_body.h"), os.path.join(CSRC, "post_ring_layout.h"),
+HEADERS = [os.path.join(CSRC, "b7_internal.h"), os.path.join(CSRC, "gemm_f64.h"), os.path.join(CSRC, "potrf_diag.h"), os.path.join(CSRC, "comm_rccl.h"), os.path.join(CSRC, "ksx_exp.h"), os.path.join(CSRC, "ksx_walk.h"), os.path.join(CSRC, "exp_table.h"), os.path.join(CSRC, "mes_math.h"), os.path.join(CSRC, "counter_rng.h"), os.path.join(CSRC, "gp_small_body.h"), os.path.join(CSRC, "post_ring_layout.h"), os.path.join(CSRC, "ks_tile_layout.h"),
            os.path.join(ROOT, "include", "bot7hip.h")]
 HIPCC = os.environ.get("HIPCC", "/opt/rocm/bin/hipcc")
 FLAGS = ["-O3", "-std=c++17", "-fPIC", "--offload-arch=gfx950", "-fno-fast-math", "-Wall",
diff --git a/bot7_amd/csrc/b7_internal.h b/bot7_amd/csrc/b7_internal.h
--- a/bot7_amd/csrc/b7_internal.h
+++ b/bot7_amd/csrc/b7_internal.h
@@ -336,16 +336,27 @@
   const double *w = nullptr;
   KBatchDesc batch;
 };
+enum class KsLayout { RowMajor, Tiles };
+struct KsBuf {
+  double *p;
+  KsLayout layout;
+};
+static inline bool post_takes_tall(const b7_ctx *c, int64_t rows, int S) { return c->Npad % 256 == 0 && rows / 256 * S >= c->cus; }
+static inline KsBuf ks_row_major(const void *p) { return KsBuf{(double *)p, KsLayout::RowMajor}; }
+static inline KsBuf ks_buf_for(const b7_ctx *c, void *p, int64_t rows, int S) {
+  const bool tiles = c->model_kind == 0 && c->ycols == 1 && post_takes_tall(c, rows, S);
+  return KsBuf{(double *)p, tiles ? KsLayout::Tiles : KsLayout::RowMajor};
+}
 int launch_prep_obs_aux(b7_ctx *c, const double *xobs, const double *ls_dev, int N, int npad, double *zsc,
                         double *zsh);
 int launch_k_generic(b7_ctx *c, const double *xq, int64_t rows, int64_t Mtotal, const ObsSet &o, double *out);
 int launch_prep_obs(b7_ctx *c, const double *xobs, const double *lenscale_sq_dev, int N, int d);
 int launch_kxx(b7_ctx *c, double diag_add);
-int launch_ksx_batch(b7_ctx *c, const FitSet &f, const double *xq, int64_t rows, int64_t Mtotal, double *ks, int64_t s_out,
+int launch_ksx_batch(b7_ctx *c, const FitSet &f, const double *xq, int64_t rows, int64_t Mtotal, const KsBuf &ks, int64_t s_out,
                      double *mu, int64_t s_mu);
 int launch_kxx_batch(b7_ctx *c, int B, const double *ls_dev, const double *amp_dev, const double *noise_dev, double *w,
                      double *zsc, double *zss, double *K);
-int launch_ksx(b7_ctx *c, const FitSet &f, const double *xq, int64_t row0, int64_t rows, int64_t Mtotal, int d, double *ks,
+int launch_ksx(b7_ctx *c, const FitSet &f, const double *xq, int64_t row0, int64_t rows, int64_t Mtotal, int d, const KsBuf &ks,
                double *mu, int ycols);
 
 struct FactorNote {
@@ -391,8 +402,8 @@
 int launch_fro_norm_sq(b7_ctx *c, const double *A, int n, int ld, double *out_dev);
 int launch_set_identity(b7_ctx *c);
 
-int launch_post(b7_ctx *c, const FitSet &f, const double *ks, int64_t row0, int64_t rows, int64_t Mtotal, double *var);
-int launch_post_batch(b7_ctx *c, const FitSet &f, const double *ks, int64_t sks, int64_t rows, int64_t Mtotal, double *var,
+int launch_post(b7_ctx *c, const FitSet &f, const KsBuf &ks, int64_t row0, int64_t rows, int64_t Mtotal, double *var);
+int launch_post_batch(b7_ctx *c, const FitSet &f, const KsBuf &ks, int64_t sks, int64_t rows, int64_t Mtotal, double *var,
                       int64_t svar);
 
 int launch_mean_multi(b7_ctx *c, const FitSet &f, const double *ks, int64_t row0, int64_t rows, int64_t Mtotal, double *mu);
diff --git a/bot7_amd/csrc/blr_api.hip b/bot7_amd/csrc/blr_api.hip
--- a/bot7_amd/csrc/blr_api.hip
+++ b/bot7_amd/csrc/blr_api.hip
@@ -67,7 +67,7 @@
   if (!mean_done)
     B7_TRY(launch_gemv_rows(c, (const double *)c->feat.p, c->Npad, (const double *)c->alpha.p, c->Npad, c->mean, 0, M, M,
                             (double *)c->mu.p));
-  B7_TRY(launch_post(c, ctx_fit(c), (const double *)c->feat.p, 0, round_up(M, B7_MROWS), M, (double *)c->var.p));
+  B7_TRY(launch_post(c, ctx_fit(c), ks_row_major(c->feat.p), 0, round_up(M, B7_MROWS), M, (double *)c->var.p));
   c->predicted = true;
   c->Mpred = M;
   return B7_OK;
diff --git a/bot7_amd/csrc/covar.hip b/bot7_amd/csrc/covar.hip
--- a/bot7_amd/csrc/covar.hip
+++ b/bot7_amd/csrc/covar.hip
@@ -2,6 +2,7 @@
 #include "gemm_f64.h"
 #include "ksx_exp.h"
 #include "ksx_walk.h"
+#include "ks_tile_layout.h"
 
 namespace {
 
@@ -69,7 +70,7 @@
 }
 
 using KBatch = KBatchDesc;
-template <int DPAD, int KERN>
+template <int DPAD, int KERN, bool TILED>
 __global__ void __launch_bounds__(256)
     ksx_kernel(const double *__restrict__ xq, int64_t row0, int64_t Mtotal, int d, int dpad_rt, const double *w,
                const double *zsc, const double *zsh, const double *__restrict__ alpha, double amp, double meanc, int Npad,
@@ -111,6 +112,8 @@
   for (int r = 0; r < 4; ++r) hq[r] = wk.xs()[wave * 16 + lq + 4 * r];
   const bool odd = lane & 1;
   double *orow = out + ((int64_t)blockIdx.x * KSX_Q + wave * 16 + lq + (odd ? 4 : 0)) * Npad + (lr & ~1);
+  double *otile = out + (ks_tile::tile_byte(ks_tile::store_panel(blockIdx.x), 0, ks_tile::store_tile(blockIdx.x, wave), Npad) +
+                         ks_tile::store_byte(0, lane)) / 8;
 
   wk.run(slab0, nslab, rider_load, rider_store, [&](int s, int cur, int t, const double (&bf)[T::KSTEPS]) {
     const int o0 = s * KO;
@@ -129,10 +132,14 @@
 #endif
 #pragma unroll
     for (int r = 0; r < 4; ++r) macc[r] = __builtin_fma(kv[r], al, macc[r]);
-    d2_t v01, v23;
-    pair_pack(kv[0], kv[1], v01);
-    pair_pack(kv[2], kv[3], v23);
-    {
+    if constexpr (TILED) {
+      double *p = otile + (int64_t)((o0 + t * 16) / ks_tile::KB) * (ks_tile::BLOCK_BYTES / 8);
+      *reinterpret_cast<d2_t *>(p) = d2_t{kv[0], kv[1]};
+      *reinterpret_cast<d2_t *>(p + ks_tile::HALF_BYTES / 8) = d2_t{kv[2], kv[3]};
+    } else {
+      d2_t v01, v23;
+      pair_pack(kv[0], kv[1], v01);
+      pair_pack(kv[2], kv[3], v23);
       double *p = orow + o0 + t * 16;
 #if B7_KSX_ABLATE & 1
       if (v01[0] == 1.2345e-300) {
@@ -193,12 +200,15 @@
   return bytes;
 }
 
+template <bool TILED>
 int ksx_launch(b7_ctx *c, dim3 grid, const double *xq, int64_t row0, int64_t Mtotal, int d, const ObsSet &o,
                const double *alpha, double amp, double meanc, double *out, double *mu) {
+  if (TILED && (grid.x % 2 || grid.y != 1 || o.npad % ks_tile::KB))
+    return b7_fail(c, B7_ERR_INVALID, "covariance kernel: piece order needs whole panels of %d rows and unsplit observations", ks_tile::PANEL);
   return ksx_for_class(c, "covariance kernel", [&](auto cls) {
     using C = decltype(cls);
     const size_t lds = ksx_lds_bytes<C::DPAD>();
-    auto kern = ksx_kernel<C::DPAD, C::KERN>;
+    auto kern = ksx_kernel<C::DPAD, C::KERN, TILED>;
     B7_HIP(c, hipFuncSetAttribute(reinterpret_cast<const void *>(kern), hipFuncAttributeMaxDynamicSharedMemorySize,
                                   (int)lds));
     hipLaunchKernelGGL(kern, grid, dim3(256), lds, c->stream, xq, row0, Mtotal, d, c->dpad, o.w ? o.w : (const double *)c->w.p,
@@ -208,6 +218,15 @@
   });
 }
 
+int ksx_launch_into(b7_ctx *c, dim3 grid, const double *xq, int64_t row0, int64_t Mtotal, int d, const ObsSet &o, const double *alpha,
+                    double amp, double meanc, const KsBuf &out, double *mu) {
+  if (out.layout == KsLayout::Tiles) {
+    if (c->profile) c->phases["ksx.tiles"].launches += 1;
+    return ksx_launch<true>(c, grid, xq, row0, Mtotal, d, o, alpha, amp, meanc, out.p, mu);
+  }
+  return ksx_launch<false>(c, grid, xq, row0, Mtotal, d, o, alpha, amp, meanc, out.p, mu);
+}
+
 }
 
 int launch_prep_obs(b7_ctx *c, const double *xobs, const double *ls_dev, int N, int d) {
@@ -230,17 +249,17 @@
 
 int launch_k_generic(b7_ctx *c, const double *xq, int64_t rows, int64_t Mtotal, const ObsSet &o, double *out) {
   if (rows % KSX_Q || o.npad % 64) return b7_fail(c, B7_ERR_INVALID, "k_generic: extents not multiples of 64");
-  return ksx_launch(c, dim3((unsigned)(rows / KSX_Q), 1), xq, 0, Mtotal, c->dfit, o, nullptr, c->amp, 0.0, out, nullptr);
-}
-
-int launch_ksx(b7_ctx *c, const FitSet &f, const double *xq, int64_t row0, int64_t rows, int64_t Mtotal, int d, double *ks,
+  return ksx_launch<false>(c, dim3((unsigned)(rows / KSX_Q), 1), xq, 0, Mtotal, c->dfit, o, nullptr, c->amp, 0.0, out, nullptr);
+}
+
+int launch_ksx(b7_ctx *c, const FitSet &f, const double *xq, int64_t row0, int64_t rows, int64_t Mtotal, int d, const KsBuf &ks,
                double *mu, int ycols) {
   PhaseScope ps(c, "ksx");
   if (rows % KSX_Q) return b7_fail(c, B7_ERR_INVALID, "ksx: rows %lld not a multiple of %d", (long long)rows, KSX_Q);
   if (ycols != 1) mu = nullptr;
   ObsSet o{f.zsc, f.zss, c->Npad};
   o.w = f.w;
-  return ksx_launch(c, dim3((unsigned)(rows / KSX_Q), 1), xq, row0, Mtotal, d, o, mu ? f.alpha : nullptr, f.amp, f.mean, ks, mu);
+  return ksx_launch_into(c, dim3((unsigned)(rows / KSX_Q), 1), xq, row0, Mtotal, d, o, mu ? f.alpha : nullptr, f.amp, f.mean, ks, mu);
 }
 
 int launch_kxx(b7_ctx *c, double diag_add) {
@@ -249,7 +268,7 @@
   int ny = 1;
   while (ny < 16 && (Npad / 64) % (ny * 2) == 0 && (Npad / KSX_Q) * ny < 2 * c->cus) ny *= 2;
   const ObsSet o{(const double *)c->zsc.p, (const double *)c->zss.p, Npad};
-  B7_TRY(ksx_launch(c, dim3(Npad / KSX_Q, ny), (const double *)c->xobs.p, 0, c->N, c->dfit, o, nullptr, c->amp, 0.0,
+  B7_TRY(ksx_launch<false>(c, dim3(Npad / KSX_Q, ny), (const double *)c->xobs.p, 0, c->N, c->dfit, o, nullptr, c->amp, 0.0,
                       (double *)c->K.p, nullptr));
   int64_t total = (int64_t)Npad * Npad;
   hipLaunchKernelGGL(kxx_fix_kernel, dim3((unsigned)((total + 255) / 256)), dim3(256), 0, c->stream, (double *)c->K.p,
@@ -258,7 +277,7 @@
   return B7_OK;
 }
 
-int launch_ksx_batch(b7_ctx *c, const FitSet &f, const double *xq, int64_t rows, int64_t Mtotal, double *ks, int64_t s_out,
+int launch_ksx_batch(b7_ctx *c, const FitSet &f, const double *xq, int64_t rows, int64_t Mtotal, const KsBuf &ks, int64_t s_out,
                      double *mu, int64_t s_mu) {
   PhaseScope ps(c, "ksx");
   if (rows % KSX_Q) return b7_fail(c, B7_ERR_INVALID, "ksx: rows %lld not a multiple of %d", (long long)rows, KSX_Q);
@@ -272,7 +291,7 @@
   o.batch.s_alpha = FitSet::s_alpha(c->Npad, c->dpad);
   o.batch.s_mu = s_mu;
   o.batch.mean = f.mean_dev;
-  return ksx_launch(c, dim3((unsigned)(rows / KSX_Q), 1, f.S), xq, 0, Mtotal, c->dfit, o, f.alpha, f.amp, 0.0, ks, mu);
+  return ksx_launch_into(c, dim3((unsigned)(rows / KSX_Q), 1, f.S), xq, 0, Mtotal, c->dfit, o, f.alpha, f.amp, 0.0, ks, mu);
 }
 
 int launch_kxx_batch(b7_ctx *c, int B, const double *ls_dev, const double *amp_dev, const double *noise_dev, double *w,
@@ -291,7 +310,7 @@
   o.batch.amp = amp_dev;
   int ny = 1;
   while (ny < 16 && (Npad / 64) % (ny * 2) == 0 && (Npad / KSX_Q) * ny * B < 2 * c->cus) ny *= 2;
-  B7_TRY(ksx_launch(c, dim3(Npad / KSX_Q, ny, B), (const double *)c->xobs.p, 0, c->N, d, o, nullptr, c->amp, 0.0, K, nullptr));
+  B7_TRY(ksx_launch<false>(c, dim3(Npad / KSX_Q, ny, B), (const double *)c->xobs.p, 0, c->N, d, o, nullptr, c->amp, 0.0, K, nullptr));
   const int64_t total = (int64_t)Npad * Npad;
   hipLaunchKernelGGL(kxx_fix_kernel, dim3((unsigned)((total + 255) / 256), B), dim3(256), 0, c->stream, K, c->N, Npad, 0.0,
                      noise_dev, total);
diff --git a/bot7_amd/csrc/gp_api.hip b/bot7_amd/csrc/gp_api.hip
--- a/bot7_amd/csrc/gp_api.hip
+++ b/bot7_amd/csrc/gp_api.hip
@@ -104,9 +104,10 @@
   B7_TRY(b7_ensure(c, c->ks, sizeof(double) * (size_t)chunk * c->Npad));
   for (int64_t row0 = 0; row0 < M; row0 += chunk) {
     int64_t rows = Mpad - row0 < chunk ? Mpad - row0 : chunk;
-    B7_TRY(launch_ksx(c, fit, xq, row0, rows, M, c->dfit, (double *)c->ks.p, mu, c->ycols));
-    if (c->ycols > 1) B7_TRY(launch_mean_multi(c, fit, (const double *)c->ks.p, row0, rows, M, mu));
-    B7_TRY(launch_post(c, fit, (const double *)c->ks.p, row0, rows, M, var));
+    const KsBuf ks = ks_buf_for(c, c->ks.p, rows, 1);
+    B7_TRY(launch_ksx(c, fit, xq, row0, rows, M, c->dfit, ks, mu, c->ycols));
+    if (c->ycols > 1) B7_TRY(launch_mean_multi(c, fit, ks.p, row0, rows, M, mu));
+    B7_TRY(launch_post(c, fit, ks, row0, rows, M, var));
   }
   return B7_OK;
 }
@@ -559,7 +560,7 @@
   double *mu = dv + 4096, *out = mu + 64;
   int *info_dev = (int *)(out + (size_t)P * n + 2);
   B7_HIP(c, hipMemcpyAsync(xp, X_pend, sizeof(double) * (size_t)P * d, hipMemcpyHostToDevice, c->stream));
-  B7_TRY(launch_ksx(c, ctx_fit(c), xp, 0, 64, P, d, kp, mu, 1));
+  B7_TRY(launch_ksx(c, ctx_fit(c), xp, 0, 64, P, d, ks_row_major(kp), mu, 1));
   B7_TRY(launch_gemm_nt(c, kp, np, (const double *)c->Linv.p, np, vt, np, 64, np, np));
   B7_TRY(launch_gemm_nt(c, vt, np, vt, np, g, 64, 64, 64, np));
   double *ls_dev = b7_scratch(c)->lenscale;
@@ -618,7 +619,7 @@
   double *krows = (double *)c->fant.p, *lvec = krows + (size_t)64 * np, *uvec = lvec + np, *evec = uvec + np;
   double *part = evec + np;
   int *status_dev = (int *)(part + (size_t)np * nslices);
-  B7_TRY(launch_ksx(c, ctx_fit(c), (const double *)c->xobs.p + (size_t)N * d, 0, 64, 1, d, krows, nullptr, 1));
+  B7_TRY(launch_ksx(c, ctx_fit(c), (const double *)c->xobs.p + (size_t)N * d, 0, 64, 1, d, ks_row_major(krows), nullptr, 1));
   B7_TRY(launch_append_vectors(c, krows, lvec, uvec, part, evec));
   B7_TRY(launch_append_finalize(c, krows, lvec, uvec, evec, status_dev));
   int status = 0;
diff --git a/bot7_amd/csrc/ks_tile_layout.h b/bot7_amd/csrc/ks_tile_layout.h
--- /dev/null
+++ b/bot7_amd/csrc/ks_tile_layout.h
@@ -0,0 +1,38 @@
+#pragma once
+#include "post_ring_layout.h"
+
+namespace ks_tile {
+constexpr int PANEL = 128, KB = 16, TILE_CAND = 16, TILES = PANEL / TILE_CAND;
+constexpr int HALF_BYTES = post_ring::PIECE_BYTES, TILE_BYTES = 2 * HALF_BYTES, BLOCK_BYTES = TILES * TILE_BYTES;
+constexpr int KS_PIECES = BLOCK_BYTES / post_ring::PIECE_BYTES;
+static_assert(TILE_BYTES == TILE_CAND * KB * 8 && BLOCK_BYTES == PANEL * KB * 8, "a tile is 16 x 16 doubles");
+static_assert(TILE_BYTES == TILE_CAND * post_ring::ROW_BYTES, "a strip of the image is one tile");
+
+struct Elem {
+  int cand, k;
+};
+
+constexpr long long tile_byte(long long panel, int kb, int tile, int Npad) {
+  return ((panel * (Npad / KB) + kb) * TILES + tile) * TILE_BYTES;
+}
+
+constexpr long long store_panel(long long bx) { return bx >> 1; }
+constexpr int store_tile(long long bx, int wave) { return (int)(bx & 1) * 4 + wave; }
+constexpr int store_byte(int r2, int lane) { return r2 * HALF_BYTES + post_ring::CHUNK_BYTES * lane; }
+constexpr Elem store_elem(int r2, int lane, int e) { return Elem{(lane >> 4) + 4 * (2 * r2 + e), lane & 15}; }
+
+constexpr int piece_of(int wave, int i) { return post_ring::WAVES * i + wave; }
+constexpr int piece_tile(int piece) { return piece >> 1; }
+constexpr int piece_half(int piece) { return piece & 1; }
+constexpr int lds_pos(int half, int b, int k) { return 16 * (k >> 2) + 8 * (((k >> 1) & 1) ^ half) + 2 * b + (k & 1); }
+constexpr int dma_src_chunk(int half, int lane) {
+  return 16 * ((lane >> 1) & 3) + 4 * (lane >> 4) + 2 * (((lane >> 3) & 1) ^ half) + (lane & 1);
+}
+constexpr int dma_src_byte(int piece, int lane) {
+  return piece * post_ring::PIECE_BYTES + post_ring::CHUNK_BYTES * dma_src_chunk(piece_half(piece), lane);
+}
+constexpr int frag_byte(int cand, int k) {
+  const int c = cand & 15, half = c >> 3;
+  return (cand >> 4) * TILE_BYTES + half * HALF_BYTES + lds_pos(half, c & 3, k) * post_ring::CHUNK_BYTES + ((c >> 2) & 1) * 8;
+}
+}
diff --git a/bot7_amd/csrc/nominate.hip b/bot7_amd/csrc/nominate.hip
--- a/bot7_amd/csrc/nominate.hip
+++ b/bot7_amd/csrc/nominate.hip
@@ -187,8 +187,9 @@
   B7_TRY(b7_ensure(c, c->ks, sizeof(double) * (size_t)sks * S));
   B7_TRY(b7_ensure(c, c->bmu, sizeof(double) * (size_t)S * c->M));
   B7_TRY(b7_ensure(c, c->bvar, sizeof(double) * (size_t)S * c->M));
-  B7_TRY(launch_ksx_batch(c, fits, (const double *)c->grid[c->grid_cur].p, Mpad, c->M, (double *)c->ks.p, sks, (double *)c->bmu.p, c->M));
-  B7_TRY(launch_post_batch(c, fits, (const double *)c->ks.p, sks, Mpad, c->M, (double *)c->bvar.p, c->M));
+  const KsBuf ks = ks_buf_for(c, c->ks.p, Mpad, S);
+  B7_TRY(launch_ksx_batch(c, fits, (const double *)c->grid[c->grid_cur].p, Mpad, c->M, ks, sks, (double *)c->bmu.p, c->M));
+  B7_TRY(launch_post_batch(c, fits, ks, sks, Mpad, c->M, (double *)c->bvar.p, c->M));
   B7_TRY(keep_batch(c, keep, S));
   ScoreParams all;
   B7_TRY(pending_score(c, S, spec, fd, &all));
diff --git a/bot7_amd/csrc/posterior.hip b/bot7_amd/csrc/posterior.hip
--- a/bot7_amd/csrc/posterior.hip
+++ b/bot7_amd/csrc/posterior.hip
@@ -1,5 +1,6 @@
 #include "b7_internal.h"
 #include "post_ring_layout.h"
+#include "ks_tile_layout.h"
 #include <utility>
 
 #ifdef B7_POST_STAMPS
@@ -263,7 +264,7 @@
 template <int NJ>
 constexpr int lds_bytes() { return 2 * (BM + 64 * NJ) * LD * 8; }
 
-template <int NJ, int NR>
+template <int NJ, int NR, bool TILED = false>
 struct Tall {
   static constexpr int BMT = 16 * NR, BN = 64 * NJ, ROWS = BMT + BN;
   static constexpr int STAGE_BYTES = ROWS * post_ring::ROW_BYTES, NBUF = 3;
@@ -274,6 +275,8 @@
   static_assert(NJ * NR == 32, "32 accumulator tiles per wave");
   static_assert(ND == 12 && ND % 3 == 0, "vmcnt(12) below is ND; a third of the pieces per k-step");
   static_assert(LDS_BYTES <= 160 * 1024, "three stage images in 160 KiB");
+  static_assert(!TILED || (BN == ks_tile::PANEL && BK == ks_tile::KB && ND - NDA == ks_tile::KS_PIECES / post_ring::WAVES),
+                "piece order: a workgroup is one panel, a stage one k block");
 
   struct Set {
     double a[NR], b[NJ];
@@ -281,7 +284,7 @@
   typedef __attribute__((address_space(3))) double lds_double;
   struct Lane {
     int fa[NBUF][4], fb[NBUF][4];
-    unsigned src, dst[NBUF];
+    unsigned src, srcb, dst[NBUF];
     __device__ __forceinline__ void rotate1() {
 #pragma unroll
       for (int s = 0; s < 4; ++s) {
@@ -319,8 +322,10 @@
   }
   template <int C>
   static __device__ __forceinline__ void dma_piece(const char *__restrict__ ga, const char *__restrict__ gb, int64_t step,
-                                                   unsigned src, unsigned dst) {
-    const char *g = C < NDA ? ga + C * step : gb + (C - NDA) * step;
+                                                   const Lane &ln, unsigned dst) {
+    const char *g = C < NDA ? ga + C * step
+                            : gb + (C - NDA) * (TILED ? (int64_t)(post_ring::WAVES * post_ring::PIECE_BYTES) : step);
+    const unsigned src = TILED && C >= NDA ? ln.srcb : ln.src;
     const unsigned m0 = dst + C * post_ring::WAVES * post_ring::PIECE_BYTES;
     asm volatile("s_mov_b32 m0, %0\n\ts_nop 0\n\tglobal_load_lds_dwordx4 %1, %2" ::"s"(m0), "v"(src), "s"(g) : "memory");
   }
@@ -347,17 +352,22 @@
   }
   static constexpr bool is_dma(int x) { return dma_before(x + 1) > dma_before(x); }
 
+  static __device__ __forceinline__ int64_t ks_advance(int kb) {
+    if constexpr (TILED) return (int64_t)kb * ks_tile::BLOCK_BYTES;
+    return (int64_t)(kb * BK) * 8;
+  }
+
   template <int FIRST, int NEXT_FIRST, bool ZERO, int POS>
   static __device__ __forceinline__ void stage(Set &s0, Set &s1, const Lane &ln,
                                                const char *__restrict__ pa, const char *__restrict__ pb, int64_t lda, Cursor &ld) {
     constexpr int CUR = POS % NBUF, NXT = (POS + 1) % NBUF, DST = (POS + 2) % NBUF;
     const int64_t step = 32 * lda * 8;
-    const char *ga = pa + (((int64_t)ld.t * BMT) * lda + ld.kb * BK) * 8, *gb = pb + (int64_t)(ld.kb * BK) * 8;
+    const char *ga = pa + (((int64_t)ld.t * BMT) * lda + ld.kb * BK) * 8, *gb = pb + ks_advance(ld.kb);
     ld.advance();
     auto sides = [&](auto ks_, Set &into, auto x_) {
       constexpr int ks = decltype(ks_)::value, x = decltype(x_)::value, r = x - dma_before(x);
       if constexpr (is_dma(x))
-        dma_piece<H * ks + dma_before(x)>(ga, gb, step, ln.src, ln.dst[DST]);
+        dma_piece<H * ks + dma_before(x)>(ga, gb, step, ln, ln.dst[DST]);
       else if constexpr (r < NJ || r - NJ >= FIRST)
         read_one<r, ks + 1, CUR>(into, ln);
     };
@@ -373,12 +383,12 @@
   }
 };
 
-template <int NJ, int NR>
+template <int NJ, int NR, bool TILED = false>
 __global__ void __launch_bounds__(256)
     post_kernel_w4t(const double *__restrict__ Linv, const double *__restrict__ ks, int Npad, int64_t row0, int64_t Mtotal,
                     double base, double sgn, double var_add, int clamp, double var_min, double *__restrict__ var,
                     PostBatch bat) {
-  using T = Tall<NJ, NR>;
+  using T = Tall<NJ, NR, TILED>;
   constexpr int BMT = T::BMT, BN = T::BN, NP = T::NP;
   extern __shared__ __align__(16) double sm[];
   if (bat.base) {
@@ -396,11 +406,14 @@
 #endif
   const int64_t lda = Npad;
   const char *pa = reinterpret_cast<const char *>(Linv + (int64_t)(post_ring::PIECE_ROWS * wave) * lda);
-  const char *pb = reinterpret_cast<const char *>(ks + ((int64_t)blockIdx.x * BN + post_ring::PIECE_ROWS * wave) * lda);
+  const char *pb = TILED ? reinterpret_cast<const char *>(ks) + ks_tile::tile_byte(blockIdx.x, 0, 0, Npad) +
+                               ks_tile::piece_of(wave, 0) * post_ring::PIECE_BYTES
+                         : reinterpret_cast<const char *>(ks + ((int64_t)blockIdx.x * BN + post_ring::PIECE_ROWS * wave) * lda);
   typename T::Lane ln;
   {
     const post_ring::Chunk c = post_ring::dma_src(wave, lane);
     ln.src = (unsigned)(((c.row - post_ring::PIECE_ROWS * wave) * Npad + 2 * c.chunk) * 8);
+    ln.srcb = (unsigned)(ks_tile::dma_src_byte(ks_tile::piece_of(wave, 0), lane) - ks_tile::piece_of(wave, 0) * post_ring::PIECE_BYTES);
   }
   const unsigned lds0 = (unsigned)(uintptr_t)(__attribute__((address_space(3))) void *)sm;
 #pragma unroll
@@ -408,7 +421,11 @@
 #pragma unroll
     for (int s = 0; s < 4; ++s) {
       ln.fa[b][s] = lds0 + b * T::STAGE_BYTES + post_ring::frag_byte(lane & 15, 4 * s + (lane >> 4));
-      ln.fb[b][s] = ln.fa[b][s] + (BMT + wave * 16 * NJ) * post_ring::ROW_BYTES;
+      if constexpr (TILED)
+        ln.fb[b][s] = lds0 + b * T::STAGE_BYTES + BMT * post_ring::ROW_BYTES +
+                      ks_tile::frag_byte(wave * 16 * NJ + (lane & 15), 4 * s + (lane >> 4));
+      else
+        ln.fb[b][s] = ln.fa[b][s] + (BMT + wave * 16 * NJ) * post_ring::ROW_BYTES;
       asm volatile("" : "+v"(ln.fa[b][s]), "+v"(ln.fb[b][s]));
     }
     ln.dst[b] = lds0 + b * T::STAGE_BYTES + wave * post_ring::PIECE_BYTES;
@@ -419,10 +436,10 @@
   typename T::Set s0, s1;
   {
     const int64_t step = 32 * lda * 8;
-    static_for<T::ND>([&](auto c_) { T::template dma_piece<decltype(c_)::value>(pa, pb, step, ln.src, ln.dst[0]); });
+    static_for<T::ND>([&](auto c_) { T::template dma_piece<decltype(c_)::value>(pa, pb, step, ln, ln.dst[0]); });
     ld.advance();
-    const char *ga = pa + (((int64_t)ld.t * BMT) * lda + ld.kb * BK) * 8, *gb = pb + (int64_t)(ld.kb * BK) * 8;
-    static_for<T::ND>([&](auto c_) { T::template dma_piece<decltype(c_)::value>(ga, gb, step, ln.src, ln.dst[1]); });
+    const char *ga = pa + (((int64_t)ld.t * BMT) * lda + ld.kb * BK) * 8, *gb = pb + T::ks_advance(ld.kb);
+    static_for<T::ND>([&](auto c_) { T::template dma_piece<decltype(c_)::value>(ga, gb, step, ln, ln.dst[1]); });
     ld.advance();
   }
   asm volatile("s_waitcnt vmcnt(12)" ::: "memory");
@@ -585,7 +602,8 @@
 #ifndef B7_POST_NO_LAUNCHERS
 namespace {
 struct PostArgs {
-  const double *Linv, *ks;
+  const double *Linv;
+  KsBuf ks;
   double *var;
   double base, sgn, var_add;
   int S;
@@ -597,19 +615,19 @@
   constexpr int lds = w4::lds_bytes<NJ>();
   B7_HIP(c, hipFuncSetAttribute(reinterpret_cast<const void *>(w4::post_kernel_w4<NJ>),
                                 hipFuncAttributeMaxDynamicSharedMemorySize, lds));
-  hipLaunchKernelGGL(w4::post_kernel_w4<NJ>, dim3((unsigned)(rows / (64 * NJ)), a.S), dim3(256), lds, c->stream, a.Linv, a.ks,
+  hipLaunchKernelGGL(w4::post_kernel_w4<NJ>, dim3((unsigned)(rows / (64 * NJ)), a.S), dim3(256), lds, c->stream, a.Linv, (const double *)a.ks.p,
                      c->Npad, row0, Mtotal, a.base, a.sgn, a.var_add, c->opts.var_clamp, c->opts.var_min, a.var, a.pb);
   B7_HIP(c, hipGetLastError());
   return B7_OK;
 }
 
-template <int NJ, int NR>
+template <int NJ, int NR, bool TILED>
 int launch_post_tall(b7_ctx *c, const PostArgs &a, int64_t row0, int64_t rows, int64_t Mtotal) {
-  using T = w4::Tall<NJ, NR>;
-  auto kern = w4::post_kernel_w4t<NJ, NR>;
+  using T = w4::Tall<NJ, NR, TILED>;
+  auto kern = w4::post_kernel_w4t<NJ, NR, TILED>;
   B7_HIP(c, hipFuncSetAttribute(reinterpret_cast<const void *>(kern), hipFuncAttributeMaxDynamicSharedMemorySize,
                                 T::LDS_BYTES));
-  hipLaunchKernelGGL(kern, dim3((unsigned)(rows / T::BN), a.S), dim3(256), T::LDS_BYTES, c->stream, a.Linv, a.ks, c->Npad, row0,
+  hipLaunchKernelGGL(kern, dim3((unsigned)(rows / T::BN), a.S), dim3(256), T::LDS_BYTES, c->stream, a.Linv, (const double *)a.ks.p, c->Npad, row0,
                      Mtotal, a.base, a.sgn, a.var_add, c->opts.var_clamp, c->opts.var_min, a.var, a.pb);
   B7_HIP(c, hipGetLastError());
   return B7_OK;
@@ -622,7 +640,7 @@
   int gx = (2 * c->cus + S - 1) / S;
   if (gx > ntiles) gx = ntiles;
   if (gx < 1) gx = 1;
-  hipLaunchKernelGGL(small64::post_small_kernel, dim3((unsigned)gx, S), dim3(256), small64::LDS_BYTES, c->stream, a.Linv, a.ks, row0,
+  hipLaunchKernelGGL(small64::post_small_kernel, dim3((unsigned)gx, S), dim3(256), small64::LDS_BYTES, c->stream, a.Linv, (const double *)a.ks.p, row0,
                      Mtotal, ntiles, a.base, a.sgn, a.var_add, c->opts.var_clamp, c->opts.var_min, a.var, a.pb);
   B7_HIP(c, hipGetLastError());
   return B7_OK;
@@ -630,15 +648,21 @@
 
 int dispatch_post(b7_ctx *c, const PostArgs &a, int64_t row0, int64_t rows, int64_t Mtotal) {
   if (rows % B7_MROWS) return b7_fail(c, B7_ERR_INVALID, "post: rows %lld not a multiple of %d", (long long)rows, B7_MROWS);
+  const bool tall = post_takes_tall(c, rows, a.S);
+  if (a.ks.layout == KsLayout::Tiles && !tall) return b7_fail(c, B7_ERR_INVALID, "post: K* in piece order for a launch that is not the tall shape");
   if (c->Npad == 64) return launch_post_small(c, a, row0, rows, Mtotal);
   const bool large = rows / 256 * a.S >= c->cus;
-  if (c->Npad % 256 == 0 && large) return launch_post_tall<2, 16>(c, a, row0, rows, Mtotal);
+  if (tall && a.ks.layout == KsLayout::Tiles) {
+    if (c->profile) c->phases["post.tiles"].launches += 1;
+    return launch_post_tall<2, 16, true>(c, a, row0, rows, Mtotal);
+  }
+  if (tall) return launch_post_tall<2, 16, false>(c, a, row0, rows, Mtotal);
   if (!large) return launch_post_w4<2>(c, a, row0, rows, Mtotal);
   return launch_post_w4<4>(c, a, row0, rows, Mtotal);
 }
 }
 
-int launch_post(b7_ctx *c, const FitSet &f, const double *ks, int64_t row0, int64_t rows, int64_t Mtotal, double *var) {
+int launch_post(b7_ctx *c, const FitSet &f, const KsBuf &ks, int64_t row0, int64_t rows, int64_t Mtotal, double *var) {
   PhaseScope ps(c, "post");
   const bool blr = c->model_kind == 1;
   PostArgs a{f.Linv, ks, var, blr ? 0.0 : f.amp, blr ? 1.0 : -1.0, blr ? f.noise : (c->opts.var_with_noise ? f.noise : 0.0), 1,
@@ -646,7 +670,7 @@
   return dispatch_post(c, a, row0, rows, Mtotal);
 }
 
-int launch_post_batch(b7_ctx *c, const FitSet &f, const double *ks, int64_t sks, int64_t rows, int64_t Mtotal, double *var,
+int launch_post_batch(b7_ctx *c, const FitSet &f, const KsBuf &ks, int64_t sks, int64_t rows, int64_t Mtotal, double *var,
                       int64_t svar) {
   PhaseScope ps(c, "post");
   PostArgs a{f.Linv, ks, var, 0.0, -1.0, 0.0, f.S, PostBatch{}};
@@ -661,7 +685,7 @@
 int launch_post_heads(b7_ctx *c, int S, const double *Linv, const double *feat, int64_t rows, int64_t Mtotal, double *var, int64_t svar,
                       const double *zero_dev, const double *invbeta_dev) {
   PhaseScope ps(c, "post");
-  PostArgs a{Linv, feat, var, 0.0, 1.0, 0.0, S, PostBatch{}};
+  PostArgs a{Linv, ks_row_major(feat), var, 0.0, 1.0, 0.0, S, PostBatch{}};
   a.pb.sLinv = FitSet::s_Linv(c->Npad, c->dpad);
   a.pb.sks = 0;
   a.pb.svar = svar;
diff --git a/bot7_amd/csrc/rff.hip b/bot7_amd/csrc/rff.hip
--- a/bot7_amd/csrc/rff.hip
+++ b/bot7_amd/csrc/rff.hip
@@ -268,7 +268,7 @@
   const double *grid = (const double *)c->grid[c->grid_cur].p;
   for (int64_t row0 = 0; row0 < M; row0 += chunk) {
     const int64_t rows = Mpad - row0 < chunk ? Mpad - row0 : chunk;
-    B7_TRY(launch_ksx(c, ctx_fit(c), grid, row0, rows, M, c->dfit, (double *)c->ks.p, (double *)c->mu.p, c->ycols));
+    B7_TRY(launch_ksx(c, ctx_fit(c), grid, row0, rows, M, c->dfit, ks_row_major(c->ks.p), (double *)c->mu.p, c->ycols));
     if (c->ycols > 1) B7_TRY(launch_mean_multi(c, ctx_fit(c), (const double *)c->ks.p, row0, rows, M, (double *)c->mu.p));
   }
   return B7_OK;
```

Result: no change. 16.62 million (median of 6 runs) (+0.9%).
